# Seanforfun/Distributed-Tensorflow-Framework

Measured on AMD Instinct MI355X. Metric: images/sec (whole node) ResNet-50 sync-SGD at 1/2/4/8 MI355X; scaling efficiency, higher is better.
Workload: dtype bf16; 1 GPU; model=resnet50_v1.5, global_batch=256, per_gpu_batch=256, image_size=224, parallelism=dp1, grad_sync=allreduce, comm_dtype=fp32, optimizer=momentum-sgd (fused), kernels=native, hip_graph=True

## Files before the change

### mdtf/csrc/bn.hip

```cpp
#include "mdtf_common.h"

using namespace mdtf;

namespace {

constexpr int kThreads = 256;

struct Geo {
  int tpr;
  int rg;
  int gy;
  int gx;
};

Geo make_geo(long long M, int C) {
  Geo g;
  int cv = C / 8;
  int t = 1;
  while (t * 2 <= cv && t * 2 <= kThreads) t *= 2;
  g.tpr = t;
  g.rg = kThreads / t;
  g.gy = static_cast<int>(ceil_div(cv, t));
  long long gx = ceil_div(M, (long long)g.rg * 16);
  long long cap = 1024 / g.gy;
// ... 258 lines not shown
    const char* e = getenv("MDTF_BN_NT");
    return !(e && e[0] == '0');
  }();
  return on;
}

template <bool HAS_RES, bool RELU, bool NT = false>
__device__ __forceinline__ void apply8(const uint4& xr, const uint4& rr, const float (&sc)[8], const float (&sh)[8],
                                       bf16_t* __restrict__ y, uint8_t* __restrict__ mask, long long i) {
  float v[8], r[8];
  unpack8(xr, v);
  if (HAS_RES) unpack8(rr, r);
  uint32_t bits = 0;
#pragma unroll
  for (int k = 0; k < 8; ++k) {
    float o = v[k] * sc[k] + sh[k];
    if (HAS_RES) o += r[k];
    if (RELU) {
      o = fmaxf(o, 0.f);
      bits |= (o > 0.f ? 1u : 0u) << k;
    }
    v[k] = o;
  }
  st_bf8<NT>(y + i * 8, v);
  if (RELU && mask) mask[i] = static_cast<uint8_t>(bits);
}

constexpr int kVpt = 4;

template <bool HAS_RES, bool RELU, bool NT = false>
__global__ void __launch_bounds__(kThreads)
    bn_apply_kernel(const bf16_t* __restrict__ x, const bf16_t* __restrict__ res, bf16_t* __restrict__ y,
                    uint8_t* __restrict__ mask, long long n8, int C, const float* __restrict__ scale,
                    const float* __restrict__ shift) {
  const long long base = (long long)blockIdx.x * (kThreads * kVpt) + threadIdx.x;
  const uint4 z4 = make_uint4(0, 0, 0, 0);
  uint4 xr[kVpt], rr[kVpt];
#pragma unroll
  for (int u = 0; u < kVpt; ++u) {
    const long long i = base + u * kThreads;
    xr[u] = i < n8 ? ld16<NT>(x + i * 8) : z4;
    rr[u] = (HAS_RES && i < n8) ? ld16<NT>(res + i * 8) : z4;
  }
  const bool fixed = (kThreads * 8) % C == 0;
  float sc[8], sh[8];
  load_coef8(scale, static_cast<int>((base * 8) % C), sc);
  load_coef8(shift, static_cast<int>((base * 8) % C), sh);
#pragma unroll
  for (int u = 0; u < kVpt; ++u) {
    const long long i = base + u * kThreads;
    if (i >= n8) break;
    if (!fixed) {
      load_coef8(scale, static_cast<int>((i * 8) % C), sc);
      load_coef8(shift, static_cast<int>((i * 8) % C), sh);
    }
    apply8<HAS_RES, RELU, NT>(xr[u], rr[u], sc, sh, y, mask, i);
  }
}

template <bool NT>
__global__ void __launch_bounds__(kThreads)
    bn_apply_dual_kernel(const bf16_t* __restrict__ x, const bf16_t* __restrict__ r, bf16_t* __restrict__ y,
                         uint8_t* __restrict__ mask, long long n8, int C, const float* __restrict__ scale,
                         const float* __restrict__ shift, const float* __restrict__ scale2,
                         const float* __restrict__ shift2) {
  const long long base = (long long)blockIdx.x * (kThreads * kVpt) + threadIdx.x;
  const uint4 z4 = make_uint4(0, 0, 0, 0);
  uint4 xr[kVpt], rr[kVpt];
#pragma unroll
  for (int u = 0; u < kVpt; ++u) {
    const long long i = base + u * kThreads;
    xr[u] = i < n8 ? ld16<NT>(x + i * 8) : z4;
    rr[u] = i < n8 ? ld16<NT>(r + i * 8) : z4;
  }
  const bool fixed = (kThreads * 8) % C == 0;
  float sc[8], sh[8], sc2[8], sh2[8];
  int c0 = static_cast<int>((base * 8) % C);
  load_coef8(scale, c0, sc);
  load_coef8(shift, c0, sh);
  load_coef8(scale2, c0, sc2);
  load_coef8(shift2, c0, sh2);
#pragma unroll
  for (int u = 0; u < kVpt; ++u) {
    const long long i = base + u * kThreads;
    if (i >= n8) break;
    if (!fixed) {
      c0 = static_cast<int>((i * 8) % C);
      load_coef8(scale, c0, sc);
      load_coef8(shift, c0, sh);
      load_coef8(scale2, c0, sc2);
      load_coef8(shift2, c0, sh2);
    }
    float v[8], rv[8];
    unpack8(xr[u], v);
    unpack8(rr[u], rv);
    uint32_t bits = 0;
#pragma unroll
    for (int k = 0; k < 8; ++k) {
      const float o = fmaxf(v[k] * sc[k] + sh[k] + (rv[k] * sc2[k] + sh2[k]), 0.f);
      bits |= (o > 0.f ? 1u : 0u) << k;
      v[k] = o;
    }
    st_bf8<NT>(y + i * 8, v);
    mask[i] = static_cast<uint8_t>(bits);
  }
}

struct FinBwd {
  const float* p0;
  const float* p1;
  int gx;
  const float* gamma;
  const float* mean;
  const float* invstd;
  float* dgamma;
  float* dbeta;
  float* k1;
  float* k2;
  float* k3;
  int zero_after;
};

__device__ __forceinline__ void finalize_bwd(const FinBwd& a, long long M, int C) {
  const int c = blockIdx.x * kFinCh + threadIdx.x % kFinCh;
  const bool own = threadIdx.x < kFinCh && c < C;
  const float mu = own ? a.mean[c] : 0.f, inv = own ? a.invstd[c] : 0.f;
  const float g = own && a.gamma ? a.gamma[c] : 1.f;
  const bool ow = (a.zero_after & 2) != 0;
  const float dg0 = own && a.dgamma && !ow ? a.dgamma[c] : 0.f;
  const float db0 = own && a.dbeta && !ow ? a.dbeta[c] : 0.f;
  double sdz, sdzx;
  if (!sum_partials(a.p0, a.p1, a.gx, C, sdz, sdzx, (a.zero_after & 1) != 0)) return;
  float db = (float)sdz;
  float dg = (float)((sdzx - (double)mu * sdz) * inv);
  if (a.dgamma) a.dgamma[c] = dg0 + dg;
  if (a.dbeta) a.dbeta[c] = db0 + db;
  float ak = g * inv;
  float invM = 1.f / (float)M;
  a.k1[c] = ak;
  a.k2[c] = -ak * inv * dg * invM;
  a.k3[c] = ak * (-db * invM + mu * inv * dg * invM);
}

__global__ void __launch_bounds__(1024)
    bn_finalize_bwd(const float* __restrict__ p0, const float* __restrict__ p1, int gx, long long M, int C,
                    const float* __restrict__ gamma, const float* __restrict__ mean, const float* __restrict__ invstd,
                    float* __restrict__ dgamma, float* __restrict__ dbeta, float* __restrict__ k1,
                    float* __restrict__ k2, float* __restrict__ k3, int zero_after) {
  finalize_bwd(FinBwd{p0, p1, gx, gamma, mean, invstd, dgamma, dbeta, k1, k2, k3, zero_after}, M, C);
}

__global__ void __launch_bounds__(1024) bn_finalize_bwd2(FinBwd a0, FinBwd a1, long long M, int C) {
  finalize_bwd(blockIdx.y ? a1 : a0, M, C);
}

template <bool RELU, bool WRITE_DRES, bool NT = false>
__device__ __forceinline__ void dx8(const uint4& gr, const uint4& xr, uint32_t m8, const uint4& orr,
                                    const float (&A)[8], const float (&B)[8], const float (&E)[8],
                                    bf16_t* __restrict__ dx, bf16_t* __restrict__ dres, long long i, int accum_dres) {
  float g[8], xv[8];
  unpack8(gr, g);
  unpack8(xr, xv);
  if (RELU) {
#pragma unroll
    for (int k = 0; k < 8; ++k) g[k] = ((m8 >> k) & 1u) ? g[k] : 0.f;
  }
  if (WRITE_DRES) {
    if (accum_dres) {
      float o[8];
      unpack8(orr, o);
#pragma unroll
      for (int k = 0; k < 8; ++k) o[k] += g[k];
      st_bf8<NT>(dres + i * 8, o);
    } else {
      st_bf8<NT>(dres + i * 8, g);
    }
  }
  float o[8];
#pragma unroll
  for (int k = 0; k < 8; ++k) o[k] = A[k] * g[k] + B[k] * xv[k] + E[k];
  st_bf8<NT>(dx + i * 8, o);
}

template <bool RELU, bool WRITE_DRES, bool NT = false>
__global__ void __launch_bounds__(kThreads)
    bn_dx_kernel(const bf16_t* __restrict__ dy, const bf16_t* __restrict__ x, const uint8_t* __restrict__ mk,
                 bf16_t* __restrict__ dx, bf16_t* __restrict__ dres, long long n8, int C, const float* __restrict__ k1,
                 const float* __restrict__ k2, const float* __restrict__ k3, int accum_dres,
                 const float* __restrict__ fin_dgdb, float* __restrict__ dgamma, float* __restrict__ dbeta) {
  if (fin_dgdb && blockIdx.x == 0) {
    for (int c = threadIdx.x; c < C; c += kThreads) {
      if (dgamma) dgamma[c] += fin_dgdb[c];
      if (dbeta) dbeta[c] += fin_dgdb[C + c];
    }
  }
  const long long base = (long long)blockIdx.x * (kThreads * kVpt) + threadIdx.x;
  const uint4 z4 = make_uint4(0, 0, 0, 0);
  const bool acc = WRITE_DRES && accum_dres;
  uint4 gr[kVpt], xr[kVpt], orr[kVpt];
  uint32_t m8[kVpt];
#pragma unroll
  for (int u = 0; u < kVpt; ++u) {
    const long long i = base + u * kThreads;
    const bool ok = i < n8;
    gr[u] = ok ? ld16<NT>(dy + i * 8) : z4;
    xr[u] = ok ? ld16<NT>(x + i * 8) : z4;
    m8[u] = (RELU && ok) ? mk[i] : 0xffu;
    orr[u] = (acc && ok) ? ld16<NT>(dres + i * 8) : z4;
  }
  const bool fixed = (kThreads * 8) % C == 0;
  float A[8], B[8], E[8];
  const int c0 = static_cast<int>((base * 8) % C);
  load_coef8(k1, c0, A);
  load_coef8(k2, c0, B);
  load_coef8(k3, c0, E);
#pragma unroll
  for (int u = 0; u < kVpt; ++u) {
    const long long i = base + u * kThreads;
    if (i >= n8) break;
    if (!fixed) {
      const int c = static_cast<int>((i * 8) % C);
      load_coef8(k1, c, A);
      load_coef8(k2, c, B);
      load_coef8(k3, c, E);
    }
    dx8<RELU, WRITE_DRES, NT>(gr[u], xr[u], m8[u], orr[u], A, B, E, dx, dres, i, accum_dres);
  }
}

inline int ew_grid(long long n8);
void launch_dx(const void* dy, const void* x, const void* mask, void* dx, void* dres, long long M, int C,
               const float* k1, const float* k2, const float* k3, int relu, int accum_dres, hipStream_t st,
               const float* fin_dgdb = nullptr, float* dgamma = nullptr, float* dbeta = nullptr);

void launch_apply(const void* x, const void* res, void* y, uint8_t* mask, long long n8, int C, const float* scale,
                  const float* shift, int relu, hipStream_t st) {
  const bf16_t* r = (const bf16_t*)res;
  const bf16_t* xx = (const bf16_t*)x;
  bf16_t* yy = (bf16_t*)y;
  const bool nt = bn_nt();
#define APPLY(R_, L_)                                                                                               \
  hipLaunchKernelGGL((nt ? bn_apply_kernel<R_, L_, true> : bn_apply_kernel<R_, L_, false>), dim3(ew_grid(n8)),     \
                     dim3(kThreads), 0, st, xx, R_ ? r : nullptr, yy, L_ ? mask : nullptr, n8, C, scale, shift)
  if (r && relu)
    APPLY(true, true);
  else if (r)
    APPLY(true, false);
  else if (relu)
    APPLY(false, true);
  else
    APPLY(false, false);
#undef APPLY
}

inline int ew_grid(long long n8) {
  long long b = ceil_div(n8, (long long)kThreads * kVpt);
  return static_cast<int>(b > 0 ? b : 1);
}

}

MDTF_EXPORT long long mdtf_bn_workspace_floats(long long M, int C) {
  Geo g = make_geo(M, C);
  return 2LL * g.gx * C + 4LL * C;
}

MDTF_EXPORT int mdtf_bn_fwd_train(const void* x, const void* res, void* y, uint8_t* mask, long long M, int C,
                                  const float* gamma, const float* beta, float* mmean, float* mvar, float decay,
                                  float eps, int relu, float* mean, float* invstd, float* ws, hipStream_t st) {
  if (C % 8) return MDTF_EINVAL;
  Geo g = make_geo(M, C);
  float* p0 = ws;
  float* p1 = ws + (long long)g.gx * C;
  float* scale = p1 + (long long)g.gx * C;
  float* shift = scale + C;
  size_t lds = 2 * sizeof(float) * g.rg * g.tpr * 8;
  hipLaunchKernelGGL((bn_reduce_kernel<false, false>), dim3(g.gx, g.gy), dim3(kThreads), lds, st,
                     (const bf16_t*)x, nullptr, nullptr, M, C, g.tpr, g.rg, p0, p1);
  hipLaunchKernelGGL(bn_finalize_fwd, dim3(ceil_div(C, kFinCh)), dim3(kFinCh * kFinGroups), 0, st, p0, p1, g.gx, M, C, gamma, beta,
                     mmean, mvar, decay, eps, mean, invstd, scale, shift, 0);
  long long n8 = M * C / 8;
  launch_apply(x, res, y, mask, n8, C, scale, shift, relu, st);
  MDTF_LAUNCH_CHECK();
  return 0;
}

MDTF_EXPORT int mdtf_bn_fwd_stats(const void* x, const void* res, void* y, uint8_t* mask, long long M, int C,
                                  const float* gamma, const float* beta, float* mmean, float* mvar, float decay,
                                  float eps, int relu, float* mean, float* invstd, const float* psum, const float* psq,
                                  int P, float* ws, hipStream_t st) {
  if (C % 8) return MDTF_EINVAL;
  float* scale = ws;
  float* shift = ws + C;
  hipLaunchKernelGGL(bn_finalize_fwd, dim3(ceil_div(C, kFinCh)), dim3(kFinCh * kFinGroups), 0, st, psum, psq, P, M,
                     C, gamma, beta, mmean, mvar, decay, eps, mean, invstd, scale, shift, 1);
  long long n8 = M * C / 8;
  launch_apply(x, res, y, mask, n8, C, scale, shift, relu, st);
  MDTF_LAUNCH_CHECK();
  return 0;
}

MDTF_EXPORT int mdtf_bn_fwd_coeffs(long long M, int C, const float* gamma, const float* beta, float* mmean,
                                   float* mvar, float decay, float eps, float* mean, float* invstd, const float* psum,
                                   const float* psq, int P, float* ws, hipStream_t st) {
  if (C % 8) return MDTF_EINVAL;
  hipLaunchKernelGGL(bn_finalize_fwd, dim3(ceil_div(C, kFinCh)), dim3(kFinCh * kFinGroups), 0, st, psum, psq, P, M,
// ... 630 lines not shown
bool pool_geo_ok(const PoolG& g) {
  return g.C % 8 == 0 && g.KH * g.KW <= 255 && (long long)g.N * g.H * g.W * g.C < (1LL << 31) &&
         g.OH > 0 && g.OW > 0;
}

}

MDTF_EXPORT int mdtf_bn_relu_maxpool_fwd(const void* x, void* y, uint8_t* arg, int N, int H, int W, int C, int OH,
                                         int OW, int KH, int KW, int SH, int SW, int PT, int PL, const float* gamma,
                                         const float* beta, float* mmean, float* mvar, float decay, float eps,
                                         float* mean, float* invstd, const float* psum, const float* psq, int P,
                                         float* ss, hipStream_t st) {
  PoolG g{N, H, W, C, OH, OW, KH, KW, SH, SW, PT, PL};
  if (!pool_geo_ok(g)) return MDTF_EUNSUPPORTED;
  const long long M = (long long)N * H * W;
  hipLaunchKernelGGL(bn_finalize_fwd, dim3(ceil_div(C, kFinCh)), dim3(kFinCh * kFinGroups), 0, st, psum, psq, P, M,
                     C, gamma, beta, mmean, mvar, decay, eps, mean, invstd, ss, ss + C, 1);
  const int total = N * OH * OW * (C / 8);
  hipLaunchKernelGGL(bn_relu_maxpool_fwd, dim3(ceil_div(total, kThreads)), dim3(kThreads), 0, st, (const bf16_t*)x,
                     ss, ss + C, (bf16_t*)y, arg, g, total);
  MDTF_LAUNCH_CHECK();
  return 0;
}

namespace {
int pool_dx_pairs = -1;
}

MDTF_EXPORT void mdtf_bn_pool_dx_pairs(int on) { pool_dx_pairs = on ? 1 : 0; }

MDTF_EXPORT int mdtf_maxpool_bn_bwd(const void* dy, const uint8_t* arg, const void* x, void* dx, int N, int H, int W,
                                    int C, int OH, int OW, int KH, int KW, int SH, int SW, int PT, int PL,
                                    const float* gamma, const float* mean, const float* invstd, float* dgamma,
                                    float* dbeta, const float* ss, float* ws, const void* y, hipStream_t st) {
  PoolG g{N, H, W, C, OH, OW, KH, KW, SH, SW, PT, PL};
  if (!pool_geo_ok(g)) return MDTF_EUNSUPPORTED;
  const long long M = (long long)N * H * W;
  Geo ge = make_geo(M, C);
  float* p0 = ws;
  float* p1 = ws + (long long)ge.gx * C;
  float* k1 = p1 + (long long)ge.gx * C;
  float* k2 = k1 + C;
  float* k3 = k2 + C;
  const int cv = C / 8;
  const bool rows_path = (cv & (cv - 1)) == 0 && cv <= kThreads;
  int parts = ge.gx;
  if (y) {
    const Geo gp = make_geo((long long)N * OH * OW, C);
    parts = gp.gx;
    const size_t lds = 2 * sizeof(float) * gp.rg * gp.tpr * 8;
    hipLaunchKernelGGL(maxpool_bn_bwd_reduce_pooled, dim3(gp.gx, gp.gy), dim3(kThreads), lds, st, (const bf16_t*)dy,
                       (const bf16_t*)y, arg, (const bf16_t*)x, ss, ss + C, invstd, g, gp.tpr, gp.rg, p0, p1);
  } else if (rows_path) {
    int cvs = 0;
    while ((1 << cvs) < cv) ++cvs;
    const int nrows = N * H;
    int gx = ge.gx < nrows ? ge.gx : nrows;
    const int rpb = (nrows + gx - 1) / gx;
    gx = (nrows + rpb - 1) / rpb;
    parts = gx;
    hipLaunchKernelGGL(maxpool_bn_bwd_reduce_rows, dim3(gx), dim3(kThreads), 0, st, (const bf16_t*)dy, arg,
                       (const bf16_t*)x, ss, ss + C, g, cvs, rpb, p0, p1);
  } else {
    const size_t lds = 2 * sizeof(float) * ge.rg * ge.tpr * 8;
    hipLaunchKernelGGL(maxpool_bn_bwd_reduce, dim3(ge.gx, ge.gy), dim3(kThreads), lds, st, (const bf16_t*)dy, arg,
                       (const bf16_t*)x, ss, ss + C, g, ge.tpr, ge.rg, p0, p1);
  }
  hipLaunchKernelGGL(bn_finalize_bwd, dim3(ceil_div(C, kFinCh)), dim3(kFinCh * kFinGroups), 0, st, p0, p1, parts, M,
                     C, gamma, mean, invstd, dgamma, dbeta, k1, k2, k3, 0);
  if (pool_dx_pairs < 0) {
    const char* e = getenv("MDTF_POOL_DX_PAIRS");
    pool_dx_pairs = (e && e[0] == '0') ? 0 : 1;
  }
  const bool pairs_on = pool_dx_pairs != 0;
  const size_t pair_lds = (size_t)2 * OW * cv * (sizeof(uint4) + sizeof(uint2));
  if (rows_path && pairs_on && SH == 2 && SW == 2 && KH <= 4 && KW <= 4 && PT >= 0 && PL >= 0 &&
      2 * W * cv <= kThreads * kPairVec && pair_lds <= 64 * 1024) {
    int cvs = 0;
    while ((1 << cvs) < cv) ++cvs;
    const int kmin = PT >> 1, nk = ((H - 1 + PT) >> 1) - kmin + 1;
    hipLaunchKernelGGL(maxpool_bn_dx_pairs, dim3(N * nk), dim3(kThreads), pair_lds, st, (const bf16_t*)dy, arg,
                       (const bf16_t*)x, ss, ss + C, k1, k2, k3, (bf16_t*)dx, g, cvs, kmin, nk);
  } else if (rows_path) {
    int cvs = 0;
    while ((1 << cvs) < cv) ++cvs;
    hipLaunchKernelGGL(maxpool_bn_dx_rows, dim3(N * H), dim3(kThreads), 0, st, (const bf16_t*)dy, arg,
                       (const bf16_t*)x, ss, ss + C, k1, k2, k3, (bf16_t*)dx, g, cvs);
  } else {
    const int total = (int)(M * cv);
    hipLaunchKernelGGL(maxpool_bn_dx, dim3(ceil_div(total, kThreads)), dim3(kThreads), 0, st, (const bf16_t*)dy, arg,
                       (const bf16_t*)x, ss, ss + C, k1, k2, k3, (bf16_t*)dx, g, total);
  }
  MDTF_LAUNCH_CHECK();
  return 0;
}

namespace {
template <bool NT>
__global__ void __launch_bounds__(kThreads)
    bn_dx_dual_kernel(const bf16_t* __restrict__ dy, const bf16_t* __restrict__ x, const bf16_t* __restrict__ r,
                      const uint8_t* __restrict__ mk, bf16_t* __restrict__ dx, bf16_t* __restrict__ dr, long long n8,
                      int C, const float* __restrict__ k, const float* __restrict__ k2) {
  const long long base = (long long)blockIdx.x * (kThreads * kVpt) + threadIdx.x;
  const uint4 z4 = make_uint4(0, 0, 0, 0);
  uint4 gr[kVpt], xr[kVpt], rr[kVpt];
  uint32_t m8[kVpt];
#pragma unroll
  for (int u = 0; u < kVpt; ++u) {
    const long long i = base + u * kThreads;
    const bool ok = i < n8;
    gr[u] = ok ? ld16<NT>(dy + i * 8) : z4;
    xr[u] = ok ? ld16<NT>(x + i * 8) : z4;
    rr[u] = ok ? ld16<NT>(r + i * 8) : z4;
    m8[u] = ok ? mk[i] : 0u;
  }
  const bool fixed = (kThreads * 8) % C == 0;
  float A[8], B[8], E[8], A2[8], B2[8], E2[8];
  int c0 = static_cast<int>((base * 8) % C);
  load_coef8(k, c0, A);
  load_coef8(k + C, c0, B);
  load_coef8(k + 2 * C, c0, E);
  load_coef8(k2, c0, A2);
  load_coef8(k2 + C, c0, B2);
  load_coef8(k2 + 2 * C, c0, E2);
#pragma unroll
  for (int u = 0; u < kVpt; ++u) {
    const long long i = base + u * kThreads;
    if (i >= n8) break;
    if (!fixed) {
      c0 = static_cast<int>((i * 8) % C);
      load_coef8(k, c0, A);
      load_coef8(k + C, c0, B);
      load_coef8(k + 2 * C, c0, E);
      load_coef8(k2, c0, A2);
      load_coef8(k2 + C, c0, B2);
      load_coef8(k2 + 2 * C, c0, E2);
    }
    float g[8], xv[8], rv[8], o[8], o2[8];
    unpack8(gr[u], g);
    unpack8(xr[u], xv);
    unpack8(rr[u], rv);
#pragma unroll
    for (int e = 0; e < 8; ++e) {
      const float gm = ((m8[u] >> e) & 1u) ? g[e] : 0.f;
      o[e] = A[e] * gm + B[e] * xv[e] + E[e];
      o2[e] = A2[e] * gm + B2[e] * rv[e] + E2[e];
    }
    st_bf8<NT>(dx + i * 8, o);
    st_bf8<NT>(dr + i * 8, o2);
  }
}
}

MDTF_EXPORT int mdtf_bn_bwd_dual(const void* dy, const void* x, const void* r, const uint8_t* mask, void* dx, void* dr,
                                 long long M, int C, const float* gamma, const float* mean, const float* invstd,
                                 float* dgamma, float* dbeta, float* psum, float* psq, int P, const float* gamma2,
                                 const float* mean2, const float* invstd2, float* dgamma2, float* dbeta2, float* ws,
                                 hipStream_t st) {
  if (C % 8 || !mask) return MDTF_EINVAL;
  Geo g = make_geo(M, C);
  const long long half = 2LL * g.gx * C + 4LL * C;
  float* q0 = ws;
  float* q1 = q0 + (long long)g.gx * C;
  float* kk2 = q1 + (long long)g.gx * C;
  float* w2 = ws + half;
  float* p0 = w2;
  float* p1 = p0 + (long long)g.gx * C;
  float* kk = p1 + (long long)g.gx * C;
  const size_t lds = 2 * sizeof(float) * g.rg * g.tpr * 8;
  if (P <= 0) {
    hipLaunchKernelGGL((bn_reduce_kernel<true, true>), dim3(g.gx, g.gy), dim3(kThreads), lds, st, (const bf16_t*)dy,
                       (const bf16_t*)x, mask, M, C, g.tpr, g.rg, p0, p1);
    hipLaunchKernelGGL(bn_finalize_bwd, dim3(ceil_div(C, kFinCh)), dim3(kFinCh * kFinGroups), 0, st, p0, p1, g.gx, M,
                       C, gamma, mean, invstd, dgamma, dbeta, kk, kk + C, kk + 2 * C, 0);
  }
  hipLaunchKernelGGL((bn_reduce_kernel<true, true>), dim3(g.gx, g.gy), dim3(kThreads), lds, st, (const bf16_t*)dy,
                     (const bf16_t*)r, mask, M, C, g.tpr, g.rg, q0, q1);
  const FinBwd sc{q0, q1, g.gx, gamma2, mean2, invstd2, dgamma2, dbeta2, kk2, kk2 + C, kk2 + 2 * C, 0};
  if (P > 0)
    hipLaunchKernelGGL(bn_finalize_bwd2, dim3(ceil_div(C, kFinCh), 2), dim3(kFinCh * kFinGroups), 0, st,
                       FinBwd{psum, psq, P, gamma, mean, invstd, dgamma, dbeta, kk, kk + C, kk + 2 * C, 1}, sc, M, C);
  else
    hipLaunchKernelGGL(bn_finalize_bwd2, dim3(ceil_div(C, kFinCh), 1), dim3(kFinCh * kFinGroups), 0, st, sc, sc, M,
                       C);
  const long long n8 = M * C / 8;
  hipLaunchKernelGGL((bn_nt() ? bn_dx_dual_kernel<true> : bn_dx_dual_kernel<false>), dim3(ew_grid(n8)),
                     dim3(kThreads), 0, st, (const bf16_t*)dy,
                     (const bf16_t*)x, (const bf16_t*)r, mask, (bf16_t*)dx, (bf16_t*)dr, n8, C, kk, kk2);
  MDTF_LAUNCH_CHECK();
  return 0;
}
```

### mdtf/csrc/conv_igemm.hip

```cpp
#include "mdtf_common.h"

#ifndef FD_PF16
#define FD_PF16 1
#endif

using namespace mdtf;

namespace {

typedef __bf16 bf16x8_t __attribute__((ext_vector_type(8)));
typedef short v4s __attribute__((ext_vector_type(4)));
typedef __attribute__((address_space(3))) v4s lds_v4s;

constexpr int BK = 32;
constexpr int PADK = 8;
constexpr int PADN = 16;
constexpr int NT = 256;
constexpr int kStatSlots = 64;

struct ConvArgs {
  const bf16_t* src;
  const bf16_t* wgt;
  const bf16_t* dy;
  bf16_t* out;
  float* dw;
  float* stat_sum;
  float* stat_sq;
  int N, H, W, Cin;
  int OH, OW, Cout;
  int KH, KW, SH, SW, PH, PW, DH, DW;
  long long M;
  int Ncol;
  int K;
  int mtiles, ntiles;
  int ksplit_steps;
  int stat_slots;
  int ld_dy, ld_dw;
  int accumulate;
  const bf16_t* acc_src;
  const uint8_t* acc_mask;
  int cls_h0, cls_w0, cls_q0h, cls_q0w, cls_kh0, cls_kw0, cls_Hc, cls_Wc, cls_th, cls_tw;
  const bf16_t* bx;
  const uint8_t* bmask;
  float* bsum;
  float* bsq;
  int bslots;
  float* dbias;
  float* slab;
  int slab_cap;
  int slab_nt;
  int* cnt;
  int wg_xcd;
  const bf16_t* wseg[4];
  int seg_cols, ld_b;
  const bf16_t* bias;
  bf16_t* pre_out;
  int act;
  unsigned mg_rw, mg_rh;
  int sh_rw, sh_rh;
  long long m_base;
  int fin_blocks, fin_first;
  int co_remap;
  const float* fin_psum;
  const float* fin_psq;
  int fin_P, fin_C;
  long long fin_M;
  const float* fin_gamma;
  const float* fin_mean;
  const float* fin_invstd;
  float* fin_ws;
};

__device__ __noinline__ void fin_bwd_block(float* psum, float* psq, int P, int C, long long M, const float* gamma,
                                           const float* meanp, const float* invstdp, float* ws, int blk, char* smem) {
  const int G = blockDim.x / 32;
  const int lc = threadIdx.x & 31, grp = threadIdx.x >> 5;
  const int c = blk * 32 + lc;
  const bool own = grp == 0 && c < C;
  const float mu = own ? meanp[c] : 0.f, inv = own ? invstdp[c] : 0.f;
  const float gm = own && gamma ? gamma[c] : 1.f;
  float s[4] = {0.f, 0.f, 0.f, 0.f}, q[4] = {0.f, 0.f, 0.f, 0.f};
  if (c < C) {
    int r = grp;
    for (; r + 3 * G < P; r += 4 * G) {
#pragma unroll
      for (int u = 0; u < 4; ++u) {
        s[u] += psum[(long long)(r + u * G) * C + c];
        q[u] += psq[(long long)(r + u * G) * C + c];
      }
    }
    for (; r < P; r += G) {
      s[0] += psum[(long long)r * C + c];
      q[0] += psq[(long long)r * C + c];
    }
    for (r = grp; r < P; r += G) {
      psum[(long long)r * C + c] = 0.f;
      psq[(long long)r * C + c] = 0.f;
    }
  }
  double* L0 = reinterpret_cast<double*>(smem);
  double* L1 = L0 + G * 32;
  L0[grp * 32 + lc] = (double)s[0] + (double)s[1] + (double)s[2] + (double)s[3];
  L1[grp * 32 + lc] = (double)q[0] + (double)q[1] + (double)q[2] + (double)q[3];
  __syncthreads();
  if (!own) return;
  double sdz = 0.0, sdzx = 0.0;
  for (int g = 0; g < G; ++g) {
    sdz += L0[g * 32 + lc];
    sdzx += L1[g * 32 + lc];
  }
  const float db = (float)sdz;
  const float dg = (float)((sdzx - (double)mu * sdz) * inv);
  ws[3 * C + c] = dg;
  ws[4 * C + c] = db;
  const float ak = gm * inv, invM = 1.f / (float)M;
  ws[c] = ak;
  ws[C + c] = -ak * inv * dg * invM;
  ws[2 * C + c] = ak * (-db * invM + mu * inv * dg * invM);
}

inline void magic31(unsigned d, unsigned* m, int* sh) {
  int l = 0;
  while ((1ull << l) < d) ++l;
  *m = static_cast<unsigned>(((1ull << (31 + l)) + d - 1) / d);
  *sh = 31 + l;
}

__device__ __forceinline__ unsigned fdiv31(unsigned n, unsigned m, int sh) {
  return static_cast<unsigned>((static_cast<unsigned long long>(n) * m) >> sh);
}

__device__ __forceinline__ uint4 mask_bf8(const uint4& v, uint32_t m8) {
  const uint32_t w[4] = {v.x, v.y, v.z, v.w};
  uint32_t o[4];
#pragma unroll
  for (int k = 0; k < 4; ++k)
    o[k] = (w[k] & (((m8 >> (2 * k)) & 1u) ? 0x0000ffffu : 0u)) | (w[k] & (((m8 >> (2 * k + 1)) & 1u) ? 0xffff0000u : 0u));
  return make_uint4(o[0], o[1], o[2], o[3]);
}

typedef unsigned v4u __attribute__((ext_vector_type(4)));

__device__ __forceinline__ void unpack8(const uint4& raw, float (&f)[8]) {
  const uint32_t w[4] = {raw.x, raw.y, raw.z, raw.w};
#pragma unroll
  for (int k = 0; k < 4; ++k) {
    f[2 * k] = __uint_as_float(w[k] << 16);
    f[2 * k + 1] = __uint_as_float(w[k] & 0xffff0000u);
  }
}

__device__ __forceinline__ uint4 ld16(const bf16_t* p, bool ok) {
  return ok ? *reinterpret_cast<const uint4*>(p) : make_uint4(0, 0, 0, 0);
}

__device__ __forceinline__ void st16(bf16_t* lds, const uint4& v) { *reinterpret_cast<uint4*>(lds) = v; }

__device__ __forceinline__ bf16x8_t frag_kcontig(const bf16_t* tile, int row0, int lane) {
  const bf16_t* p = tile + (row0 + (lane & 15)) * (BK + PADK) + 8 * (lane >> 4);
  uint4 v = *reinterpret_cast<const uint4*>(p);
  return __builtin_bit_cast(bf16x8_t, v);
}

__device__ __forceinline__ bf16x8_t frag_ncontig(const bf16_t* tile, int ld, int col0, int lane) {
  const int g = lane >> 4, i = lane & 15, q = i >> 2, p = i & 3;
  const int odd = g & 1;
  const int rfirst = 8 * g + (odd ? 4 : 0) + q;
  const int rsecond = 8 * g + (odd ? 0 : 4) + q;
  const bf16_t* a1 = tile + rfirst * ld + col0 + 4 * p;
  const bf16_t* a2 = tile + rsecond * ld + col0 + 4 * p;
  v4s r1 = __builtin_amdgcn_ds_read_tr16_b64_v4i16((lds_v4s*)a1);
  v4s r2 = __builtin_amdgcn_ds_read_tr16_b64_v4i16((lds_v4s*)a2);
  v4s lo = odd ? r2 : r1;
  v4s hi = odd ? r1 : r2;
  short8 f = {lo[0], lo[1], lo[2], lo[3], hi[0], hi[1], hi[2], hi[3]};
  return __builtin_bit_cast(bf16x8_t, f);
}

__device__ __forceinline__ float dense_act(float v, int act) {
  if (act == 1) return fmaxf(v, 0.f);
  if (act == 2) {
    const float u2 = 1.5957691216f * (v + 0.044715f * v * v * v);
    return v * __builtin_amdgcn_rcpf(1.f + __expf(-u2));
  }
  return v;
}

__device__ __forceinline__ float dense_act_grad(float x, int act) {
  if (act == 1) return x > 0.f ? 1.f : 0.f;
  if (act == 2) {
    const float s = __builtin_amdgcn_rcpf(1.f + __expf(-1.5957691216f * (x + 0.044715f * x * x * x)));
    return s + 2.f * x * s * (1.f - s) * 0.7978845608f * (1.f + 0.134145f * x * x);
  }
  return 1.f;
}

__device__ __forceinline__ int trswz(int k) { return 2 * (((k >> 1) & 1) | (((k >> 3) & 1) << 1)); }

__device__ __forceinline__ bf16x8_t frag_tr(const char* img, int col0, int kbase, int lane) {
  const int g = lane >> 4, i = lane & 15, q = i >> 2, p = i & 3;
  const int c = col0 + 4 * p;
  const int k1 = kbase + 8 * g + q, k2 = k1 + 4;
  const char* a1 = img + k1 * 128 + (((c >> 3) ^ trswz(k1)) << 4) + (c & 7) * 2;
  const char* a2 = img + k2 * 128 + (((c >> 3) ^ trswz(k2)) << 4) + (c & 7) * 2;
  v4s lo = __builtin_amdgcn_ds_read_tr16_b64_v4i16((lds_v4s*)a1);
  v4s hi = __builtin_amdgcn_ds_read_tr16_b64_v4i16((lds_v4s*)a2);
  short8 f = {lo[0], lo[1], lo[2], lo[3], hi[0], hi[1], hi[2], hi[3]};
  return __builtin_bit_cast(bf16x8_t, f);
}

__device__ __forceinline__ float4v mfma(const bf16x8_t& a, const bf16x8_t& b, const float4v& c) {
  return __builtin_amdgcn_mfma_f32_16x16x32_bf16(a, b, c, 0, 0, 0);
}

__device__ __forceinline__ int xcd_remap(int bid, int nwg) {
// ... 251 lines not shown
    const int cidx = tid + i * NT;
    a_mrow[i] = cidx / (BM / 8);
    a_rc[i] = cidx % (BM / 8);
    const int r = r0 + a_rc[i] * 8;
    a_rok[i] = r < R;
    const int rr = a_rok[i] ? r : 0;
    a_c[i] = rr % a.Cin;
    const int t = rr / a.Cin;
    a_kw[i] = t % a.KW;
    a_kh[i] = t / a.KW;
  }
  const long long Mpix = a.M;
  const int KT_total = static_cast<int>((Mpix + BK - 1) / BK);
  const int kt_begin = split * a.ksplit_steps;
  const int kt_end = min(KT_total, kt_begin + a.ksplit_steps);
  if (kt_begin >= kt_end) return;

  int p_ow[A_CHUNKS], p_oh[A_CHUNKS], p_n[A_CHUNKS];
#pragma unroll
  for (int i = 0; i < A_CHUNKS; ++i) {
    const long long m = (long long)kt_begin * BK + a_mrow[i];
    p_ow[i] = static_cast<int>(m % a.OW);
    const long long t = m / a.OW;
    p_oh[i] = static_cast<int>(t % a.OH);
    p_n[i] = static_cast<int>(t / a.OH);
  }
  uint4 ra[A_CHUNKS], rb[B_CHUNKS];
  auto load_tiles = [&](int kt) {
#pragma unroll
    for (int i = 0; i < A_CHUNKS; ++i) {
      const long long m = (long long)kt * BK + a_mrow[i];
      const int iy = p_oh[i] * a.SH - a.PH + a_kh[i] * a.DH, ix = p_ow[i] * a.SW - a.PW + a_kw[i] * a.DW;
      const bool ok = a_rok[i] && m < Mpix && iy >= 0 && iy < a.H && ix >= 0 && ix < a.W;
      ra[i] = ld16(a.src + (((long long)p_n[i] * a.H + (ok ? iy : 0)) * a.W + (ok ? ix : 0)) * a.Cin + a_c[i], ok);
      p_ow[i] += BK;
      while (p_ow[i] >= a.OW) { p_ow[i] -= a.OW; if (++p_oh[i] == a.OH) { p_oh[i] = 0; ++p_n[i]; } }
    }
#pragma unroll
    for (int i = 0; i < B_CHUNKS; ++i) {
      const int cidx = tid + i * NT;
      const int mrow = cidx / (BN / 8), c8 = cidx % (BN / 8);
      const long long m = (long long)kt * BK + mrow;
      const int n = n0 + c8 * 8;
      const bool ok = m < Mpix && n < a.Cout;
      rb[i] = ld16(a.dy + (ok ? m : 0) * a.Cout + (ok ? n : 0), ok);
    }
  };
  auto store_tiles = [&](int buf) {
#pragma unroll
    for (int i = 0; i < A_CHUNKS; ++i) st16(As[buf] + a_mrow[i] * LDA + a_rc[i] * 8, ra[i]);
#pragma unroll
    for (int i = 0; i < B_CHUNKS; ++i) {
      const int cidx = tid + i * NT;
      st16(Bs[buf] + (cidx / (BN / 8)) * LDB + (cidx % (BN / 8)) * 8, rb[i]);
    }
  };

  float4v acc[TM][TN];
#pragma unroll
  for (int i = 0; i < TM; ++i)
#pragma unroll
    for (int j = 0; j < TN; ++j) acc[i][j] = float4v{0.f, 0.f, 0.f, 0.f};

  load_tiles(kt_begin);
  store_tiles(0);
  __syncthreads();
  int cur = 0;
  for (int kt = kt_begin; kt < kt_end; ++kt) {
    if (kt + 1 < kt_end) load_tiles(kt + 1);
    bf16x8_t fa[TM], fb[TN];
#pragma unroll
    for (int i = 0; i < TM; ++i) fa[i] = frag_ncontig(As[cur], LDA, wm * (TM * 16) + i * 16, lane);
#pragma unroll
    for (int j = 0; j < TN; ++j) fb[j] = frag_ncontig(Bs[cur], LDB, wn * (TN * 16) + j * 16, lane);
#pragma unroll
    for (int i = 0; i < TM; ++i)
#pragma unroll
      for (int j = 0; j < TN; ++j) acc[i][j] = mfma(fa[i], fb[j], acc[i][j]);
    if (kt + 1 < kt_end) store_tiles(cur ^ 1);
    __syncthreads();
    cur ^= 1;
  }
  const int g = lane >> 4, li = lane & 15;
#pragma unroll
  for (int i = 0; i < TM; ++i)
#pragma unroll
    for (int j = 0; j < TN; ++j) {
      const int co = n0 + wn * (TN * 16) + j * 16 + li;
      if (co >= a.Cout) continue;
#pragma unroll
      for (int rr = 0; rr < 4; ++rr) {
        const int r = r0 + wm * (TM * 16) + i * 16 + 4 * g + rr;
        if (r < R) atomicAdd(a.dw + (long long)r * a.Cout + co, acc[i][j][rr]);
      }
    }
}

template <int BN>
__device__ __forceinline__ void copyout_rc(int idx, int& row, int& c8, bool remap) {
  if (BN == 128 && remap) {
    const int l = idx & 31, hh = (idx >> 5) & 1;
    const bool ga = l < 4 || (l >= 12 && l < 16) || (l >= 20 && l < 28);
    c8 = ga ? (l < 4 ? l : (l < 16 ? l - 8 : l - 12)) : (l < 12 ? l - 4 : (l < 20 ? l - 8 : l - 16));
    row = ((idx >> 6) << 2) + 2 * hh + (ga ? 0 : 1);
  } else {
    row = idx / (BN / 8);
    c8 = idx - row * (BN / 8);
  }
}

template <int BM, int BN, int MODE, bool STATS, int STAGES, int NW>
__global__ void __launch_bounds__(64 * NW) conv_fd_v2(ConvArgs a) {
  constexpr int NT = 64 * NW;
  constexpr int WM = NW == 4 ? 2 : (BM > BN ? 4 : 2), WN = NW / WM;
  constexpr int TM = BM / WM / 16, TN = BN / WN / 16;
  constexpr int RA = BM / (8 * NW), RB = BN / (8 * NW);
  constexpr int ROWB = 128;
  constexpr int STAGE = (BM + BN) * ROWB;
  constexpr int PER_STAGE = RA + RB;
  constexpr unsigned OOB = 0x80000000u;
  constexpr bool SPLIT = STAGES >= 10;
  constexpr int SA = SPLIT ? STAGES / 10 : STAGES, SB = SPLIT ? STAGES % 10 : STAGES;
  static_assert(RA >= 1 && RB >= 1, "tile too small");
  static_assert(STAGES >= 1 && (STAGES < 2 || SPLIT || (STAGES - 2) * PER_STAGE < 64), "pipeline depth");
  static_assert(!SPLIT || (SA > SB && SB >= 2 && (SA - 1) * PER_STAGE < 64), "split ring");
  extern __shared__ __attribute__((aligned(16))) char smem_raw[];

  const int tid = threadIdx.x, lane = tid & 63;
  const int wave = __builtin_amdgcn_readfirstlane(tid >> 6);
  const int wm = wave / WN, wn = wave % WN;
  const int tile = xcd_remap(blockIdx.x, gridDim.x);
  const int mt = tile / a.ntiles, nt = tile % a.ntiles;
  const long long m0 = a.m_base + (long long)mt * BM;
  const int n0 = nt * BN;

  constexpr int AM = MODE == 3 ? 0 : MODE == 4 ? 1 : MODE;
  const int GH = AM == 0 ? a.H : a.OH;
  const int GW = AM == 0 ? a.W : a.OW;
  const int GC = AM == 0 ? a.Cin : a.Cout;
  const int RH = AM == 0 ? a.OH : AM == 1 ? a.H : a.cls_Hc;
  const int RW = AM == 0 ? a.OW : AM == 1 ? a.W : a.cls_Wc;
  const int lrow = lane >> 3;
  const int TKW = MODE == 2 ? a.cls_tw : a.KW;
  const int ntaps = MODE == 2 ? a.cls_th * a.cls_tw : a.KH * a.KW;
  const int DHe = MODE == 2 ? 1 : a.DH, DWe = MODE == 2 ? 1 : a.DW;

  const int bytes_a = (int)((long long)a.N * GH * GW * GC * 2);
  const int bytes_b = MODE == 3 ? (int)((long long)a.K * a.ld_b * 2)
                                : (int)((long long)(MODE == 2 ? a.KH * a.KW * a.Cout : a.K) * a.Ncol * 2);
  const int seg = MODE == 3 ? n0 / a.seg_cols : 0;
  const bf16_t* wbase = MODE == 3 ? a.wseg[seg] : a.wgt;
  const int nl0 = MODE == 3 ? n0 - seg * a.seg_cols : n0;

  unsigned a_off[RA], a_mask[RA];
#pragma unroll
  for (int i = 0; i < RA; ++i) {
    const int row = 8 * (wave + NW * i) + lrow;
    const long long m = m0 + row;
    const bool ok = m < a.M;
    const unsigned mm = ok ? static_cast<unsigned>(m) : 0u;
    const unsigned t = fdiv31(mm, a.mg_rw, a.sh_rw);
    const int ow = static_cast<int>(mm - t * static_cast<unsigned>(RW));
    const unsigned nq = fdiv31(t, a.mg_rh, a.sh_rh);
    const int oh = static_cast<int>(t - nq * static_cast<unsigned>(RH));
    const int n = static_cast<int>(nq);
    const int y0 = AM == 0 ? oh * a.SH - a.PH : AM == 1 ? oh + a.PH : a.cls_q0h + oh;
    const int x0 = AM == 0 ? ow * a.SW - a.PW : AM == 1 ? ow + a.PW : a.cls_q0w + ow;
    const int ch = 8 * ((lane & 7) ^ ((row >> 1) & 7));
    a_off[i] = static_cast<unsigned>(((n * GH + y0) * GW + x0) * GC + ch);
    unsigned mask = 0;
    if (ok) {
      for (int tt = 0; tt < ntaps; ++tt) {
        const int kh = tt / TKW, kw = tt - kh * TKW;
        const int iy = AM == 0 ? y0 + kh * DHe : y0 - kh * DHe;
        const int ix = AM == 0 ? x0 + kw * DWe : x0 - kw * DWe;
        if (iy >= 0 && iy < GH && ix >= 0 && ix < GW) mask |= 1u << tt;
      }
    }
    a_mask[i] = mask;
  }
  unsigned b_off[RB];
#pragma unroll
  for (int i = 0; i < RB; ++i) {
    if (MODE == 3) {
      const int blk = wave + NW * i;
      const int krow = 8 * (blk & 7) + lrow;
      const int col = nl0 + 64 * (blk >> 3) + 8 * ((lane & 7) ^ trswz(krow));
      b_off[i] = (unsigned)(((long long)krow * a.ld_b + col) * 2);
      continue;
    }
    const int row = 8 * (wave + NW * i) + lrow;
    const int n = n0 + row;
    const int ch = 8 * ((lane & 7) ^ ((row >> 1) & 7));
    const long long e = MODE == 0 ? (long long)n * a.K + ch : (long long)n * a.Cout + ch;
    b_off[i] = n < a.Ncol ? (unsigned)(e * 2) : OOB;
  }

  int s_t = 0, s_kh = 0, s_kw = 0, s_c0 = 0, s_k0 = 0;
  auto stage = [&](int buf) {
    const int tap_e = (AM == 0 ? (s_kh * DHe * GW + s_kw * DWe) : -(s_kh * DHe * GW + s_kw * DWe)) * GC + s_c0;
    char* lds = smem_raw + buf * STAGE;
#pragma unroll
    for (int i = 0; i < RA; ++i) {
      const bool ok = (a_mask[i] >> s_t) & 1u;
      const unsigned voff = ok ? (a_off[i] + (unsigned)tap_e) * 2u : OOB;
      dma16(a.src, bytes_a, lds + (wave + NW * i) * 1024, voff, 0);
    }
    char* ldsb = lds + BM * ROWB;
    const int wtap = MODE == 2 ? (a.cls_kh0 + a.SH * s_kh) * a.KW + a.cls_kw0 + a.SW * s_kw : s_t;
    const int sb = MODE == 3 ? s_k0 * a.ld_b * 2 : MODE == 0 ? s_k0 * 2 : (wtap * a.Cin * a.Cout + s_c0) * 2;
#pragma unroll
    for (int i = 0; i < RB; ++i)
      dma16(wbase, bytes_b, ldsb + (wave + NW * i) * 1024, b_off[i], sb);
    s_k0 += 64;
    s_c0 += 64;
    const int wrap = s_c0 == GC ? 1 : 0;
    s_c0 = wrap ? 0 : s_c0;
    s_t += wrap;
    s_kw += wrap;
    const int wrap2 = s_kw == TKW ? 1 : 0;
    s_kw = wrap2 ? 0 : s_kw;
    s_kh += wrap2;
  };

  float4v acc[TM][TN];
#pragma unroll
  for (int i = 0; i < TM; ++i)
#pragma unroll
    for (int j = 0; j < TN; ++j) acc[i][j] = float4v{0.f, 0.f, 0.f, 0.f};

  constexpr int PITER = MODE == 4 ? BM * (BN / 8) / (64 * NW) : 1;
  uint4 prepf[PITER];
  if constexpr (MODE == 4) {
#pragma unroll
    for (int it = 0; it < PITER; ++it) {
      const int idx = tid + it * 64 * NW;
      int row, c8;
      copyout_rc<BN>(idx, row, c8, a.co_remap != 0);
      const long long m = m0 + row;
      const int n = n0 + c8 * 8;
      prepf[it] = (m < a.M && n < a.Ncol) ? *reinterpret_cast<const uint4*>(a.pre_out + m * a.Ncol + n)
                                          : make_uint4(0, 0, 0, 0);
    }
  }

  const int KT = a.K / 64;
  const int fr = lane & 15, fq = lane >> 4;
  if constexpr (SPLIT) {
    struct Walk { int t, kh, kw, c0, k0; };
    Walk wa{0, 0, 0, 0, 0}, wb{0, 0, 0, 0, 0};
    auto advance = [&](Walk& w) {
      w.k0 += 64;
      w.c0 += 64;
      const int wrap = w.c0 == GC ? 1 : 0;
      w.c0 = wrap ? 0 : w.c0;
      w.t += wrap;
      w.kw += wrap;
      const int wrap2 = w.kw == TKW ? 1 : 0;
      w.kw = wrap2 ? 0 : w.kw;
      w.kh += wrap2;
    };
    char* const ringB = smem_raw + SA * BM * ROWB;
    auto stage_a = [&](int buf) {
      const int tap_e = (AM == 0 ? (wa.kh * DHe * GW + wa.kw * DWe) : -(wa.kh * DHe * GW + wa.kw * DWe)) * GC + wa.c0;
      char* lds = smem_raw + buf * (BM * ROWB);
#pragma unroll
      for (int i = 0; i < RA; ++i) {
        const bool ok = (a_mask[i] >> wa.t) & 1u;
        const unsigned voff = ok ? (a_off[i] + (unsigned)tap_e) * 2u : OOB;
        dma16(a.src, bytes_a, lds + (wave + NW * i) * 1024, voff, 0);
      }
      advance(wa);
    };
    auto stage_b = [&](int buf) {
      char* ldsb = ringB + buf * (BN * ROWB);
      const int wtap = MODE == 2 ? (a.cls_kh0 + a.SH * wb.kh) * a.KW + a.cls_kw0 + a.SW * wb.kw : wb.t;
      const int sb = MODE == 3 ? wb.k0 * a.ld_b * 2 : MODE == 0 ? wb.k0 * 2 : (wtap * a.Cin * a.Cout + wb.c0) * 2;
#pragma unroll
      for (int i = 0; i < RB; ++i)
        dma16(wbase, bytes_b, ldsb + (wave + NW * i) * 1024, b_off[i], sb);
      advance(wb);
    };
    auto nb_of = [&](int j) { return (j + SB - 1 < KT ? RB : 0); };
    auto na_of = [&](int j) { return (j + SA - 1 < KT ? RA : 0); };
#pragma unroll
    for (int s = 0; s < SA - 1; ++s) {
      if (s <= SB - 2 && s < KT) stage_b(s);
      if (s < KT) stage_a(s);
    }
    int ca = 0, cb = 0;
    for (int kt = 0; kt < KT; ++kt) {
      int younger = 0;
      if (kt <= SB - 2) {
        for (int s = kt + 1; s <= SA - 2; ++s) younger += (s <= SB - 2 && s < KT ? RB : 0) + (s < KT ? RA : 0);
        for (int j = 0; j < kt; ++j) younger += nb_of(j) + na_of(j);
      } else {
        const int g0 = kt - SB + 1;
        younger = na_of(g0);
        for (int j = g0 + 1; j < kt; ++j) younger += nb_of(j) + na_of(j);
      }
      wait_vmcnt_le<(SA - 1) * PER_STAGE>(younger);
      __builtin_amdgcn_s_barrier();
      if (kt + SB - 1 < KT) stage_b(cb == 0 ? SB - 1 : cb - 1);
      if (kt + SA - 1 < KT) stage_a(ca == 0 ? SA - 1 : ca - 1);
      const char* As = smem_raw + ca * (BM * ROWB);
      const char* Bs = ringB + cb * (BN * ROWB);
      ca = ca + 1 == SA ? 0 : ca + 1;
      cb = cb + 1 == SB ? 0 : cb + 1;
      bf16x8_t fa[2][TM], fb[2][TN];
#pragma unroll
      for (int h = 0; h < 2; ++h) {
#pragma unroll
        for (int i = 0; i < TM; ++i) {
          const int row = wm * (TM * 16) + i * 16 + fr;
          const int pc = (h * 4 + fq) ^ ((row >> 1) & 7);
          fa[h][i] = __builtin_bit_cast(bf16x8_t, *reinterpret_cast<const uint4*>(As + row * ROWB + pc * 16));
        }
#pragma unroll
        for (int j = 0; j < TN; ++j) {
          if (MODE == 3) {
            const int col = wn * (TN * 16) + j * 16;
            fb[h][j] = frag_tr(Bs + (col >> 6) * 8192, col & 63, 32 * h, lane);
            continue;
          }
          const int row = wn * (TN * 16) + j * 16 + fr;
          const int pc = (h * 4 + fq) ^ ((row >> 1) & 7);
          fb[h][j] = __builtin_bit_cast(bf16x8_t, *reinterpret_cast<const uint4*>(Bs + row * ROWB + pc * 16));
        }
      }
#pragma unroll
      for (int h = 0; h < 2; ++h)
#pragma unroll
        for (int i = 0; i < TM; ++i)
#pragma unroll
          for (int j = 0; j < TN; ++j) acc[i][j] = mfma(fb[h][j], fa[h][i], acc[i][j]);
      {
        constexpr int R = TM + TN, MF = TM * TN, PER = MF / R > 0 ? MF / R : 1;
        __builtin_amdgcn_sched_group_barrier(0x100, R, 0);
#pragma unroll
        for (int i = 0; i < R; ++i) {
          __builtin_amdgcn_sched_group_barrier(0x008, PER, 0);
          __builtin_amdgcn_sched_group_barrier(0x100, 1, 0);
        }
        __builtin_amdgcn_sched_group_barrier(0x008, 2 * MF, 0);
      }
    }
  } else {
#pragma unroll
  for (int s = 0; s < (STAGES > 1 ? STAGES - 1 : 1); ++s)
    if (s < KT) stage(s);
  int cur = 0;
  for (int kt = 0; kt < KT; ++kt) {
    if (STAGES >= 2 && kt + STAGES - 2 < KT)
      wait_vmcnt<(STAGES >= 2 ? (STAGES - 2) * PER_STAGE : 0)>();
    else
      wait_vmcnt<0>();
    __builtin_amdgcn_s_barrier();
    if (STAGES >= 2) {
      const int nk = kt + STAGES - 1;
      if (nk < KT) stage(nk % STAGES);
    }
    const char* As = smem_raw + cur * STAGE;
    cur = cur + 1 == STAGES ? 0 : cur + 1;
    const char* Bs = As + BM * ROWB;
    bf16x8_t fa[2][TM], fb[2][TN];
#pragma unroll
    for (int h = 0; h < 2; ++h) {
#pragma unroll
      for (int i = 0; i < TM; ++i) {
        const int row = wm * (TM * 16) + i * 16 + fr;
        const int pc = (h * 4 + fq) ^ ((row >> 1) & 7);
        fa[h][i] = __builtin_bit_cast(bf16x8_t, *reinterpret_cast<const uint4*>(As + row * ROWB + pc * 16));
      }
#pragma unroll
      for (int j = 0; j < TN; ++j) {
        if (MODE == 3) {
          const int col = wn * (TN * 16) + j * 16;
          fb[h][j] = frag_tr(Bs + (col >> 6) * 8192, col & 63, 32 * h, lane);
          continue;
        }
        const int row = wn * (TN * 16) + j * 16 + fr;
        const int pc = (h * 4 + fq) ^ ((row >> 1) & 7);
        fb[h][j] = __builtin_bit_cast(bf16x8_t, *reinterpret_cast<const uint4*>(Bs + row * ROWB + pc * 16));
      }
    }
#pragma unroll
    for (int h = 0; h < 2; ++h)
#pragma unroll
      for (int i = 0; i < TM; ++i)
#pragma unroll
        for (int j = 0; j < TN; ++j) acc[i][j] = mfma(fb[h][j], fa[h][i], acc[i][j]);
    {
      constexpr int R = TM + TN, MF = TM * TN, PER = MF / R > 0 ? MF / R : 1;
      __builtin_amdgcn_sched_group_barrier(0x100, R, 0);
#pragma unroll
      for (int i = 0; i < R; ++i) {
        __builtin_amdgcn_sched_group_barrier(0x008, PER, 0);
        __builtin_amdgcn_sched_group_barrier(0x100, 1, 0);
      }
      __builtin_amdgcn_sched_group_barrier(0x008, 2 * MF, 0);
    }
  }
  }

  constexpr int LDC = BN * 2 + 16;
  const int g = lane >> 4, li = lane & 15;
  __syncthreads();
#pragma unroll
  for (int i = 0; i < TM; ++i) {
    const int pl = wm * (TM * 16) + i * 16 + li;
#pragma unroll
    for (int j = 0; j < TN; ++j) {
      const int cl = wn * (TN * 16) + j * 16 + 4 * g;
      float4v v = acc[i][j];
      if (MODE == 3 && a.bias) {
        const uint2 b4 = *reinterpret_cast<const uint2*>(a.bias + n0 + cl);
        v[0] += __uint_as_float(b4.x << 16);
        v[1] += __uint_as_float(b4.x & 0xffff0000u);
        v[2] += __uint_as_float(b4.y << 16);
        v[3] += __uint_as_float(b4.y & 0xffff0000u);
      }
      uint32_t lo = (uint32_t)f2bf(v[0]) | ((uint32_t)f2bf(v[1]) << 16);
      uint32_t hi = (uint32_t)f2bf(v[2]) | ((uint32_t)f2bf(v[3]) << 16);
      *reinterpret_cast<uint2*>(smem_raw + pl * LDC + ((cl * 2) ^ (((pl >> 3) & 1) << 3))) = make_uint2(lo, hi);
    }
  }
  __syncthreads();
  const bool bstat = (MODE == 1 || MODE == 2) && a.bsum != nullptr;
  float bs0[8], bs1[8];
#pragma unroll
  for (int k = 0; k < 8; ++k) bs0[k] = bs1[k] = 0.f;
  constexpr int ITER = BM * (BN / 8) / NT;
  static_assert(ITER * NT == BM * (BN / 8), "copy-out rows per thread");
  constexpr int PF = (FD_PF16 && (MODE == 1 || MODE == 2) && ITER <= 16) ? ITER
                                                                        : (ITER < 4 ? ITER : (ITER % 4 == 0 ? 4 : 2));
  static_assert(ITER % PF == 0, "prefetch groups");
#pragma unroll
  for (int g0 = 0; g0 < ITER; g0 += PF) {
  long long off[PF];
  uint4 old4[PF], x4[PF];
  uint32_t mb[PF];
#pragma unroll
  for (int it = 0; it < PF; ++it) {
    const int idx = tid + (g0 + it) * NT;
    int row, c8;
    copyout_rc<BN>(idx, row, c8, a.co_remap != 0);
    const long long m = m0 + row;
    const int n = n0 + c8 * 8;
    off[it] = -1;
    if (m < a.M && n < a.Ncol) {
      long long pix = m;
      if (MODE == 2) {
        const unsigned mu = static_cast<unsigned>(m);
        const unsigned t = fdiv31(mu, a.mg_rw, a.sh_rw);
        const int j = static_cast<int>(mu - t * static_cast<unsigned>(a.cls_Wc));
        const unsigned nb = fdiv31(t, a.mg_rh, a.sh_rh);
        const int i = static_cast<int>(t - nb * static_cast<unsigned>(a.cls_Hc));
        pix = (static_cast<long long>(nb) * a.H + a.cls_h0 + a.SH * i) * a.W + a.cls_w0 + a.SW * j;
      }
      off[it] = pix * a.Ncol + n;
      if (a.accumulate) {
        old4[it] = *reinterpret_cast<const uint4*>((a.acc_src ? a.acc_src : a.out) + off[it]);
        if (a.acc_mask) old4[it] = mask_bf8(old4[it], a.acc_mask[off[it] >> 3]);
      }
      if (bstat) {
        x4[it] = *reinterpret_cast<const uint4*>(a.bx + off[it]);
        mb[it] = a.bmask ? a.bmask[off[it] >> 3] : 0xffu;
      }
    }
  }
#pragma unroll
  for (int it = 0; it < PF; ++it) {
    if (off[it] < 0) continue;
    const int idx = tid + (g0 + it) * NT;
    int row, c8;
    copyout_rc<BN>(idx, row, c8, a.co_remap != 0);
    uint4 v = *reinterpret_cast<const uint4*>(smem_raw + row * LDC + c8 * 16);
    if ((row >> 3) & 1) v = make_uint4(v.z, v.w, v.x, v.y);
    bf16_t* dst = a.out + off[it];
    if (MODE == 3 && a.act) {
      if (a.pre_out) *reinterpret_cast<uint4*>(a.pre_out + off[it]) = v;
      float c[8];
      const uint32_t w4[4] = {v.x, v.y, v.z, v.w};
#pragma unroll
      for (int k = 0; k < 4; ++k) {
        c[2 * k] = dense_act(__uint_as_float(w4[k] << 16), a.act);
        c[2 * k + 1] = dense_act(__uint_as_float(w4[k] & 0xffff0000u), a.act);
      }
      store_bf8(dst, c);
    } else if (MODE == 4) {
      float c[8];
      const uint32_t w4[4] = {v.x, v.y, v.z, v.w};
      const uint4 pv = prepf[(g0 + it) % PITER];
      const uint32_t p4[4] = {pv.x, pv.y, pv.z, pv.w};
#pragma unroll
      for (int k = 0; k < 4; ++k) {
        c[2 * k] = __uint_as_float(w4[k] << 16) * dense_act_grad(__uint_as_float(p4[k] << 16), a.act);
        c[2 * k + 1] = __uint_as_float(w4[k] & 0xffff0000u) * dense_act_grad(__uint_as_float(p4[k] & 0xffff0000u), a.act);
      }
      store_bf8(dst, c);
    } else if (a.accumulate || bstat) {
      float c[8];
      const uint32_t w4[4] = {v.x, v.y, v.z, v.w};
#pragma unroll
      for (int k = 0; k < 4; ++k) {
        c[2 * k] = __uint_as_float(w4[k] << 16);
        c[2 * k + 1] = __uint_as_float(w4[k] & 0xffff0000u);
      }
      if (a.accumulate) {
        const uint32_t o4[4] = {old4[it].x, old4[it].y, old4[it].z, old4[it].w};
#pragma unroll
        for (int k = 0; k < 4; ++k) {
          const float lo = __uint_as_float(o4[k] << 16) + c[2 * k];
          const float hi = __uint_as_float(o4[k] & 0xffff0000u) + c[2 * k + 1];
          c[2 * k] = __uint_as_float((uint32_t)f2bf(lo) << 16);
          c[2 * k + 1] = __uint_as_float((uint32_t)f2bf(hi) << 16);
        }
        store_bf8(dst, c);
      } else {
        *reinterpret_cast<uint4*>(dst) = v;
      }
      if (bstat) {
        const uint32_t xw[4] = {x4[it].x, x4[it].y, x4[it].z, x4[it].w};
#pragma unroll
        for (int k = 0; k < 8; ++k) {
          const float xk = (k & 1) ? __uint_as_float(xw[k >> 1] & 0xffff0000u) : __uint_as_float(xw[k >> 1] << 16);
          const float gk = ((mb[it] >> k) & 1u) ? c[k] : 0.f;
          bs0[k] += gk;
          bs1[k] += gk * xk;
        }
      }
    } else {
      *reinterpret_cast<uint4*>(dst) = v;
    }
  }
  }
  if (bstat) {
    static_assert(NT % (BN / 8) == 0, "one channel chunk per thread");
    __syncthreads();
    constexpr int LDR = NT + 4;
    float* red = reinterpret_cast<float*>(smem_raw);
    int slot = tid;
    if (BN == 128 && a.co_remap) {
      int r0_, c0_;
      copyout_rc<BN>(tid, r0_, c0_, true);
      slot = (tid & ~63) | ((r0_ & 3) << 4) | c0_;
    }
#pragma unroll
    for (int k = 0; k < 8; ++k) {
      red[k * LDR + slot] = bs0[k];
      red[(8 + k) * LDR + slot] = bs1[k];
    }
    __syncthreads();
    for (int nl = tid; nl < BN; nl += NT) {
      const int n = n0 + nl, c8 = nl >> 3, k = nl & 7;
      if (n < a.Ncol) {
        float sv = 0.f, q = 0.f;
        for (int t2 = c8; t2 < NT; t2 += BN / 8) {
          sv += red[k * LDR + t2];
          q += red[(8 + k) * LDR + t2];
        }
        const long long slot = (long long)(mt % a.bslots) * a.Ncol + n;
        atomicAdd(a.bsum + slot, sv);
        atomicAdd(a.bsq + slot, q);
      }
    }
  }
  if (STATS) {
    float ssum[TN][4], ssq[TN][4];
#pragma unroll
    for (int j = 0; j < TN; ++j)
#pragma unroll
      for (int r = 0; r < 4; ++r) ssum[j][r] = ssq[j][r] = 0.f;
#pragma unroll
    for (int i = 0; i < TM; ++i) {
      const bool mok = m0 + wm * (TM * 16) + i * 16 + li < a.M;
#pragma unroll
      for (int j = 0; j < TN; ++j)
        if (mok) {
#pragma unroll
          for (int r = 0; r < 4; ++r) {
            ssum[j][r] += acc[i][j][r];
            ssq[j][r] += acc[i][j][r] * acc[i][j][r];
          }
        }
    }
#pragma unroll
    for (int j = 0; j < TN; ++j)
#pragma unroll
      for (int r = 0; r < 4; ++r) {
#pragma unroll
        for (int o = 1; o < 16; o <<= 1) {
          ssum[j][r] += __shfl_xor(ssum[j][r], o, 64);
          ssq[j][r] += __shfl_xor(ssq[j][r], o, 64);
        }
      }
    __syncthreads();
    float* red = reinterpret_cast<float*>(smem_raw);
    if (li == 0) {
#pragma unroll
      for (int j = 0; j < TN; ++j)
#pragma unroll
        for (int r = 0; r < 4; ++r) {
          const int nl = wn * (TN * 16) + j * 16 + 4 * g + r;
          red[wm * BN + nl] = ssum[j][r];
          red[WM * BN + wm * BN + nl] = ssq[j][r];
        }
    }
    __syncthreads();
    for (int nl = tid; nl < BN; nl += NT) {
      const int n = n0 + nl;
      if (n < a.Ncol) {
        float sv = 0.f, q = 0.f;
#pragma unroll
        for (int w = 0; w < WM; ++w) {
          sv += red[w * BN + nl];
          q += red[WM * BN + w * BN + nl];
        }
        const long long slot = (long long)(mt % a.stat_slots) * a.Ncol + n;
        atomicAdd(a.stat_sum + slot, sv);
        atomicAdd(a.stat_sq + slot, q);
      }
    }
  }
}

template <int BM, int BN, int MODE, bool STATS, int STAGES, int NW, bool HEAVY>
__global__ void __launch_bounds__(64 * NW) conv_fd_p(ConvArgs a) {
  constexpr int NT = 64 * NW;
  constexpr int WM = NW == 4 ? 2 : (BM > BN ? 4 : 2), WN = NW / WM;
  constexpr int TM = BM / WM / 16, TN = BN / WN / 16;
  constexpr int RA = BM / (8 * NW), RB = BN / (8 * NW);
  constexpr int ROWB = 128;
  constexpr int PER_STAGE = RA + RB;
  constexpr unsigned OOB = 0x80000000u;
  constexpr bool SPLIT = STAGES >= 10;
  constexpr int SA = SPLIT ? STAGES / 10 : STAGES, SB = SPLIT ? STAGES % 10 : STAGES;
  constexpr int RING = (SA * BM + SB * BN) * ROWB;
  static_assert(MODE <= 2 && TN % 2 == 0 && RA >= 1 && RB >= 1, "persistent tile");
  constexpr int EMAX = TM * (TN / 2);
  static_assert(SA >= SB && SB >= 2 && (SA - 1) * PER_STAGE + EMAX < 64, "persistent ring");
  extern __shared__ __attribute__((aligned(16))) char smem_raw[];
  float* red = reinterpret_cast<float*>(smem_raw + RING);

  const int tid = threadIdx.x, lane = tid & 63;
  const int wave = __builtin_amdgcn_readfirstlane(tid >> 6);
  const int wm = wave / WN, wn = wave % WN;
  const int total = a.mtiles * a.ntiles;
  const int GH = MODE == 0 ? a.H : a.OH;
  const int GW = MODE == 0 ? a.W : a.OW;
  const int GC = MODE == 0 ? a.Cin : a.Cout;
  const int RH = MODE == 0 ? a.OH : MODE == 1 ? a.H : a.cls_Hc;
  const int RW = MODE == 0 ? a.OW : MODE == 1 ? a.W : a.cls_Wc;
  const int lrow = lane >> 3;
  const int TKW = MODE == 2 ? a.cls_tw : a.KW;
  const int ntaps = MODE == 2 ? a.cls_th * a.cls_tw : a.KH * a.KW;
  const int DHe = MODE == 2 ? 1 : a.DH, DWe = MODE == 2 ? 1 : a.DW;
  const int bytes_a = (int)((long long)a.N * GH * GW * GC * 2);
  const int bytes_b = (int)((long long)(MODE == 2 ? a.KH * a.KW * a.Cout : a.K) * a.Ncol * 2);
  const int bytes_o = (int)((long long)a.N * (MODE == 0 ? a.OH * a.OW : a.H * a.W) * a.Ncol * 2);
  const __amdgpu_buffer_rsrc_t rs_out = __builtin_amdgcn_make_buffer_rsrc(a.out, (short)0, bytes_o, 0x00020000);
  constexpr bool heavy = HEAVY && (MODE == 1 || MODE == 2);
  const bool bstat = heavy && a.bsum != nullptr;
  const int KT = a.K / 64;

  int mt = 0, nt = 0;
  long long m0 = 0;
  int n0 = 0;
  unsigned a_off[RA], a_mask[RA], b_off[RB];
  auto setup = [&](int w) {
    const int tile = xcd_remap(w, total);
    mt = tile / a.ntiles;
    nt = tile - mt * a.ntiles;
    m0 = a.m_base + (long long)mt * BM;
    n0 = nt * BN;
#pragma unroll
    for (int i = 0; i < RA; ++i) {
      const int row = 8 * (wave + NW * i) + lrow;
      const long long m = m0 + row;
      const bool ok = m < a.M;
      const unsigned mm = ok ? static_cast<unsigned>(m) : 0u;
      const unsigned t = fdiv31(mm, a.mg_rw, a.sh_rw);
      const int ow = static_cast<int>(mm - t * static_cast<unsigned>(RW));
      const unsigned nq = fdiv31(t, a.mg_rh, a.sh_rh);
      const int oh = static_cast<int>(t - nq * static_cast<unsigned>(RH));
      const int n = static_cast<int>(nq);
      const int y0 = MODE == 0 ? oh * a.SH - a.PH : MODE == 1 ? oh + a.PH : a.cls_q0h + oh;
      const int x0 = MODE == 0 ? ow * a.SW - a.PW : MODE == 1 ? ow + a.PW : a.cls_q0w + ow;
      const int ch = 8 * ((lane & 7) ^ ((row >> 1) & 7));
      a_off[i] = static_cast<unsigned>(((n * GH + y0) * GW + x0) * GC + ch);
      unsigned mask = 0;
      if (ok) {
        for (int tt = 0; tt < ntaps; ++tt) {
          const int kh = tt / TKW, kw = tt - kh * TKW;
          const int iy = MODE == 0 ? y0 + kh * DHe : y0 - kh * DHe;
          const int ix = MODE == 0 ? x0 + kw * DWe : x0 - kw * DWe;
          if (iy >= 0 && iy < GH && ix >= 0 && ix < GW) mask |= 1u << tt;
        }
      }
      a_mask[i] = mask;
    }
#pragma unroll
    for (int i = 0; i < RB; ++i) {
      const int row = 8 * (wave + NW * i) + lrow;
      const int n = n0 + row;
      const int ch = 8 * ((lane & 7) ^ ((row >> 1) & 7));
      const int e = MODE == 0 ? n * a.K + ch : n * a.Cout + ch;
      b_off[i] = n < a.Ncol ? static_cast<unsigned>(e * 2) : OOB;
    }
  };

  struct Walk { int t, kh, kw, c0, k0; };
  Walk wa{0, 0, 0, 0, 0}, wb{0, 0, 0, 0, 0};
  auto advance = [&](Walk& w) {
    w.k0 += 64;
    w.c0 += 64;
    const int wrap = w.c0 == GC ? 1 : 0;
// ... 236 lines not shown
#pragma unroll
        for (int r = 0; r < 4; ++r)
#pragma unroll
          for (int o2 = 1; o2 < 16; o2 <<= 1) {
            ssum[j][r] += __shfl_xor(ssum[j][r], o2, 64);
            ssq[j][r] += __shfl_xor(ssq[j][r], o2, 64);
          }
      if (li == 0) {
#pragma unroll
        for (int j = 0; j < TN; ++j)
#pragma unroll
          for (int r = 0; r < 4; ++r) {
            const int nl = wn * (TN * 16) + j * 16 + 4 * g + r;
            red[wm * BN + nl] = ssum[j][r];
            red[WM * BN + wm * BN + nl] = ssq[j][r];
          }
      }
      __syncthreads();
      for (int nl = tid; nl < BN; nl += NT) {
        const int n = cur_n0 + nl;
        if (n < a.Ncol) {
          float sv = 0.f, q = 0.f;
#pragma unroll
          for (int w2 = 0; w2 < WM; ++w2) {
            sv += red[w2 * BN + nl];
            q += red[WM * BN + w2 * BN + nl];
          }
          const long long slot = (long long)(cur_mt % a.stat_slots) * a.Ncol + n;
          atomicAdd(a.stat_sum + slot, sv);
          atomicAdd(a.stat_sq + slot, q);
        }
      }
    }
    if (!more) break;
    if (heavy) {
      __syncthreads();
      setup(w_next);
      prologue();
      E = 0;
    } else {
      E = issued;
    }
    w = w_next;
  }
}

int conv_persist_mode() {
  static const int m = [] {
    const char* e = getenv("MDTF_CONV_PERSIST");
    return e ? atoi(e) : 0;
  }();
  return m;
}

int num_cus() {
  static const int n = [] {
    int dev = 0, v = 0;
    if (hipGetDevice(&dev) != hipSuccess ||
        hipDeviceGetAttribute(&v, hipDeviceAttributeMultiprocessorCount, dev) != hipSuccess || v <= 0)
      return 256;
    return v;
  }();
  return n;
}

template <int BM, int BN, int MODE, bool STATS, int STAGES, int NW>
int launch_fd_p(ConvArgs& a, hipStream_t st) {
  constexpr int NT = 64 * NW;
  constexpr int WM = NW == 4 ? 2 : (BM > BN ? 4 : 2), WN = NW / WM;
  constexpr int TM = BM / WM / 16, TN = BN / WN / 16;
  constexpr int SA = STAGES >= 10 ? STAGES / 10 : STAGES, SB = STAGES >= 10 ? STAGES % 10 : STAGES;
  const bool heavy = (MODE == 1 || MODE == 2) && (a.accumulate || a.bsum != nullptr);
  if (conv_persist_mode() == 2 && !(MODE == 0 && NW == 8 && BM == 256 && BN == 256)) return MDTF_EUNSUPPORTED;
  if constexpr (MODE > 2 || TN % 2 != 0 || SB < 2) {
    return MDTF_EUNSUPPORTED;
  } else {
    if (heavy && TM > 4) return MDTF_EUNSUPPORTED;
    const size_t ring = ((size_t)SA * BM + (size_t)SB * BN) * 128;
    const size_t lds = ring + (STATS ? (size_t)2 * WM * BN * sizeof(float) : 0);
    if (lds > 160 * 1024) return MDTF_EUNSUPPORTED;
    auto kern = heavy ? conv_fd_p<BM, BN, MODE, STATS, STAGES, NW, (MODE != 0 && TM <= 4)>
                      : conv_fd_p<BM, BN, MODE, STATS, STAGES, NW, false>;
    static int occ[2] = {0, 0};
    if (occ[heavy] == 0) {
      int o = 0;
      if (hipOccupancyMaxActiveBlocksPerMultiprocessor(&o, kern, NT, lds) != hipSuccess || o < 1) o = 1;
      occ[heavy] = o;
    }
    const long long total = (long long)a.mtiles * a.ntiles;
    const long long cap = (long long)num_cus() * occ[heavy];
    const unsigned grid = (unsigned)(total < cap ? total : cap);
    hipLaunchKernelGGL(kern, dim3(grid), dim3(NT), lds, st, a);
    MDTF_LAUNCH_CHECK();
    return 0;
  }
}

int conv_tail_mode() {
  static const int m = [] {
    const char* e = getenv("MDTF_CONV_TAIL");
    return e ? atoi(e) : 0;
  }();
  return m;
}

extern "C" int mdtf_get_deterministic();

template <int BM, int BN, int MODE, bool STATS, int STAGES, int NW = 4>
int launch_fd_v2(ConvArgs& a, hipStream_t st);

template <int BM, int BN, int MODE, bool STATS, int STAGES, int NW>
int launch_fd_tail_split(ConvArgs& a, hipStream_t st, int* rc) {
  if constexpr (NW == 8 && BM == 256 && (MODE == 0 || MODE == 1)) {
    if (!conv_tail_mode() || a.m_base != 0 || mdtf_get_deterministic()) return 0;
    const long long mtiles = ceil_div(a.M, BM), ntiles = ceil_div(a.Ncol, BN);
    const long long cus = num_cus(), total = mtiles * ntiles;
    const long long rounds = total / cus, rem = total - rounds * cus;
    if (rounds < 1 || rem == 0 || (conv_tail_mode() == 1 && rem * 4 > cus) || (rounds * cus) % ntiles) return 0;
    const long long m1 = rounds * cus / ntiles * BM;
    if (m1 >= a.M) return 0;
    const long long M = a.M;
    ConvArgs tail = a;
    tail.m_base = m1;
    a.M = m1;
    *rc = launch_fd_v2<BM, BN, MODE, STATS, STAGES, NW>(a, st);
    a.M = M;
    if (*rc == 0) *rc = launch_fd_v2<128, 128, MODE, STATS, 2, 4>(tail, st);
    a.mtiles = static_cast<int>(mtiles);
    a.ntiles = static_cast<int>(ntiles);
    return 1;
  } else {
    (void)a;
    (void)st;
    (void)rc;
    return 0;
  }
}

template <int BM, int BN, int MODE, bool STATS, int STAGES, int NW>
int launch_fd_v2(ConvArgs& a, hipStream_t st) {
  constexpr int NT = 64 * NW;
  {
    int rc = 0;
    if (launch_fd_tail_split<BM, BN, MODE, STATS, STAGES, NW>(a, st, &rc)) return rc;
  }
  a.mtiles = static_cast<int>(ceil_div(a.M - a.m_base, BM));
  a.ntiles = static_cast<int>(ceil_div(a.Ncol, BN));
  const long long nblk = (long long)a.mtiles * a.ntiles;
  if (nblk > 0x7fffffff) return MDTF_EUNSUPPORTED;
  const size_t stage_bytes = STAGES >= 10 ? ((size_t)(STAGES / 10) * BM + (size_t)(STAGES % 10) * BN) * 128
                                          : STAGES * (size_t)(BM + BN) * 128;
  const size_t ctile = (size_t)BM * (BN * 2 + 16);
  size_t lds = stage_bytes > ctile ? stage_bytes : ctile;
  if (lds < (size_t)(NT + 8) * 16 * sizeof(float)) lds = (size_t)(NT + 8) * 16 * sizeof(float);
  if (STAGES == 1 && a.K > 64) return MDTF_EINVAL;
  if (lds > 160 * 1024) return MDTF_EUNSUPPORTED;
  if (a.M >= (1LL << 31)) return MDTF_EUNSUPPORTED;
  {
    constexpr int AM = MODE == 3 ? 0 : MODE == 4 ? 1 : MODE;
    const int RH = AM == 0 ? a.OH : AM == 1 ? a.H : a.cls_Hc;
    const int RW = AM == 0 ? a.OW : AM == 1 ? a.W : a.cls_Wc;
    if (RH < 1 || RW < 1) return MDTF_EINVAL;
    magic31(static_cast<unsigned>(RW), &a.mg_rw, &a.sh_rw);
    magic31(static_cast<unsigned>(RH), &a.mg_rh, &a.sh_rh);
  }
  if (MODE <= 2 && STAGES >= 2 && conv_persist_mode() && a.K >= 64) {
    const int rc = launch_fd_p<BM, BN, MODE, STATS, STAGES, NW>(a, st);
    if (rc != MDTF_EUNSUPPORTED) return rc;
  }
  {
    static const int remap = [] {
      const char* e = getenv("MDTF_FD_COREMAP");
      return (e && e[0] == '1') ? 1 : 0;
    }();
    a.co_remap = remap;
  }
  hipLaunchKernelGGL((conv_fd_v2<BM, BN, MODE, STATS, STAGES, NW>), dim3((unsigned)nblk), dim3(NT), lds, st, a);
  MDTF_LAUNCH_CHECK();
  return 0;
}

template <int MODE, bool STATS, int STAGES>
int dispatch_fd_v2s(ConvArgs& a, int bm, int bn, hipStream_t st) {
  if (bm == 128 && bn == 128) return launch_fd_v2<128, 128, MODE, STATS, STAGES>(a, st);
  if (bm == 128 && bn == 64) return launch_fd_v2<128, 64, MODE, STATS, STAGES>(a, st);
  if (bm == 256 && bn == 128) return launch_fd_v2<256, 128, MODE, STATS, STAGES>(a, st);
  if (bm == 256 && bn == 64) return launch_fd_v2<256, 64, MODE, STATS, STAGES>(a, st);
  if (bm == 64 && bn == 128) return launch_fd_v2<64, 128, MODE, STATS, STAGES>(a, st);
  if (bm == 64 && bn == 64) return launch_fd_v2<64, 64, MODE, STATS, STAGES>(a, st);
  return MDTF_EUNSUPPORTED;
}

template <int MODE, bool STATS>
int dispatch_fd_v2w8(ConvArgs& a, int bm, int bn, int stages, hipStream_t st) {
#define FD8(BM_, BN_, S_) \
  if (bm == BM_ && bn == BN_ && stages == S_) return launch_fd_v2<BM_, BN_, MODE, STATS, S_, 8>(a, st);
  FD8(256, 256, 1) FD8(256, 256, 2) FD8(256, 128, 1) FD8(256, 128, 2) FD8(256, 128, 3) FD8(256, 64, 2)
  FD8(256, 64, 3) FD8(256, 64, 4) FD8(128, 256, 2) FD8(128, 256, 3)
  FD8(256, 256, 32) FD8(256, 128, 32) FD8(256, 128, 42) FD8(128, 256, 32) FD8(128, 256, 42)
  if constexpr (MODE != 4) {
    FD8(448, 128, 1) FD8(448, 128, 2)
  }
#undef FD8
  return MDTF_EUNSUPPORTED;
}

template <int MODE, bool STATS>
int dispatch_fd_v2(ConvArgs& a, int bm, int bn, int stages, hipStream_t st) {
  if (bm >= 10000) return dispatch_fd_v2w8<MODE, STATS>(a, bm % 10000, bn, stages, st);
  if (stages == 32) {
    if (bm == 128 && bn == 128) return launch_fd_v2<128, 128, MODE, STATS, 32>(a, st);
    if (bm == 64 && bn == 128) return launch_fd_v2<64, 128, MODE, STATS, 32>(a, st);
    return MDTF_EUNSUPPORTED;
  }
  if (stages == 42) {
    if (bm == 64 && bn == 128) return launch_fd_v2<64, 128, MODE, STATS, 42>(a, st);
    return MDTF_EUNSUPPORTED;
  }
  if (stages == 1) return dispatch_fd_v2s<MODE, STATS, 1>(a, bm, bn, st);
  if (stages == 2) return dispatch_fd_v2s<MODE, STATS, 2>(a, bm, bn, st);
  if (stages == 3) return dispatch_fd_v2s<MODE, STATS, 3>(a, bm, bn, st);
  if (stages == 4) return dispatch_fd_v2s<MODE, STATS, 4>(a, bm, bn, st);
  return MDTF_EUNSUPPORTED;
}


template <int BM, int BN, int STAGES, int NW>
constexpr int wgrad_min_waves() {
  constexpr int blocks = (160 * 1024) / (STAGES * (BM + BN) * 128);
  constexpr int w = blocks * NW / 4;
  return w < 1 ? 1 : (w > 8 ? 8 : w);
}

template <int BM, int BN, int STAGES, int NW, bool PIPE>
__global__ void __launch_bounds__(64 * NW, (wgrad_min_waves<BM, BN, STAGES, NW>()))
    conv_wgrad_v2(ConvArgs a) {
  constexpr int WM = NW == 4 ? 2 : (BM > BN ? 4 : 2), WN = NW / WM;
  constexpr int U = 8 / NW;
  constexpr int TM = BM / WM / 16, TN = BN / WN / 16;
  constexpr int HA = BM / 64, HB = BN / 64;
  constexpr int IA = HA * U, IB = HB * U;
  constexpr int STAGE = (BM + BN) * 128;
  constexpr int PER_STAGE = IA + IB;
  constexpr unsigned OOB = 0x80000000u;
  static_assert(HA >= 1 && HB >= 1, "tile too small");
  static_assert(STAGES >= 2 && (STAGES - 2) * PER_STAGE < 64, "pipeline depth");
  extern __shared__ __attribute__((aligned(16))) char smem_raw[];

  const int tid = threadIdx.x, lane = tid & 63;
  const int wave = __builtin_amdgcn_readfirstlane(tid >> 6);
  const int wm = wave / WN, wn = wave % WN;
  const int tiles_mn = a.mtiles * a.ntiles;
  const int nwg = static_cast<int>(gridDim.x) - a.fin_blocks;
  const int fb = a.fin_first ? static_cast<int>(blockIdx.x) : static_cast<int>(blockIdx.x) - nwg;
  if (fb >= 0 && fb < a.fin_blocks) {
    fin_bwd_block(const_cast<float*>(a.fin_psum), const_cast<float*>(a.fin_psq), a.fin_P, a.fin_C, a.fin_M,
                  a.fin_gamma, a.fin_mean, a.fin_invstd, a.fin_ws, fb, smem_raw);
    return;
  }
  const int gb = a.fin_first ? static_cast<int>(blockIdx.x) - a.fin_blocks : static_cast<int>(blockIdx.x);
  const int lb = a.wg_xcd ? xcd_remap(gb, nwg) : gb;
  const int tile = lb % tiles_mn;
  const int split = lb / tiles_mn;
  const int mt = tile / a.ntiles, nt = tile % a.ntiles;
  const int r0 = mt * BM, n0 = nt * BN;
  const int R = a.KH * a.KW * a.Cin;
  const long long Mpix = a.M;
  const int KT_total = static_cast<int>((Mpix + 63) / 64);
  const int kt_begin = split * a.ksplit_steps;
  const int kt_end = min(KT_total, kt_begin + a.ksplit_steps);
  if (kt_begin >= kt_end) return;

  const int bytes_x = (int)((long long)a.N * a.H * a.W * a.Cin * 2);
  const int bytes_dy = (int)((Mpix - 1) * a.ld_dy * 2 + a.Cout * 2);
  const i32x4_t rsrc_x = buffer_rsrc(a.src, bytes_x), rsrc_dy = buffer_rsrc(a.dy, bytes_dy);

  int h_dy[HA], h_dx[HA], h_c[HA];
  bool h_ok[HA];
#pragma unroll
  for (int h = 0; h < HA; ++h) {
    const int r = r0 + 64 * h;
    h_ok[h] = r < R;
    const int rr = h_ok[h] ? r : 0;
    const int t = rr / a.Cin;
    h_c[h] = rr - t * a.Cin;
    const int kh = t / a.KW, kw = t - kh * a.KW;
    h_dy[h] = kh * a.DH - a.PH;
    h_dx[h] = kw * a.DW - a.PW;
  }
  const int krow0 = 8 * wave + (lane >> 3);
  int gch[U];
#pragma unroll
  for (int u = 0; u < U; ++u) gch[u] = ((lane & 7) ^ trswz(krow0 + 8 * NW * u)) * 8;
  int p_ow[U], p_oh[U], p_n[U];
  long long p_m[U];
#pragma unroll
  for (int u = 0; u < U; ++u) {
    const long long m = (long long)kt_begin * 64 + krow0 + 8 * NW * u;
    p_m[u] = m;
    p_ow[u] = static_cast<int>(m % a.OW);
    const long long t = m / a.OW;
    p_oh[u] = static_cast<int>(t % a.OH);
    p_n[u] = static_cast<int>(t / a.OH);
  }
  const int d_ow = 64 % a.OW, d_oh = (64 / a.OW) % a.OH, d_n = 64 / (a.OW * a.OH);

  auto stage = [&](int buf) {
    char* lds = smem_raw + buf * STAGE;
#pragma unroll
    for (int u = 0; u < U; ++u) {
      const bool mok = p_m[u] < Mpix;
      const int iy0 = p_oh[u] * a.SH, ix0 = p_ow[u] * a.SW;
#pragma unroll
      for (int h = 0; h < HA; ++h) {
        const int iy = iy0 + h_dy[h], ix = ix0 + h_dx[h];
        const bool ok = mok && h_ok[h] && iy >= 0 && iy < a.H && ix >= 0 && ix < a.W;
        const unsigned voff =
            ok ? (unsigned)((((p_n[u] * a.H + iy) * a.W + ix) * a.Cin + h_c[h] + gch[u]) * 2) : OOB;
        if constexpr (PIPE)
          dma16_asm(rsrc_x, lds + h * 8192 + (wave + NW * u) * 1024, voff);
        else
          dma16(a.src, bytes_x, lds + h * 8192 + (wave + NW * u) * 1024, voff, 0);
      }
      char* ldsb = lds + BM * 128;
#pragma unroll
      for (int h = 0; h < HB; ++h) {
        const int co = n0 + 64 * h;
        const unsigned voff = (mok && co < a.Cout) ? (unsigned)((p_m[u] * a.ld_dy + co + gch[u]) * 2) : OOB;
// ... 390 lines not shown
  if (a.slab && (splits < 2 || splits > a.slab_cap || (a.ld_dw % 4) || (a.Cout % 4))) b.slab = nullptr;
  b.cnt = nullptr;
  if (b.slab && g_wg_cnt && g_wg_cnt_n >= (long long)a.mtiles * a.ntiles && 256 % BM == 0 && 256 % BN == 0 &&
      (long long)splits * BM * BN * a.mtiles * a.ntiles * 4 < (1ll << 31) &&
      (long long)a.mtiles * BM <= ceil_div(R, 256) * 256 && (long long)a.ntiles * BN <= ceil_div(a.Cout, 256) * 256)
    b.cnt = g_wg_cnt;
  {
    static const int nt = [] {
      const char* e = getenv("MDTF_SLAB_NT");
      return (e && e[0] == '0') ? 0 : 1;
    }();
    b.slab_nt = nt;
  }
  const int store = g_wg_store;
  if (g_wg_fin.C > 0) {
    b.fin_blocks = static_cast<int>(ceil_div(g_wg_fin.C, 32));
    b.fin_psum = g_wg_fin.psum;
    b.fin_psq = g_wg_fin.psq;
    b.fin_P = g_wg_fin.P;
    b.fin_C = g_wg_fin.C;
    b.fin_M = g_wg_fin.M;
    b.fin_gamma = g_wg_fin.gamma;
    b.fin_mean = g_wg_fin.mean;
    b.fin_invstd = g_wg_fin.invstd;
    b.fin_ws = g_wg_fin.ws;
    static const int first = [] {
      const char* e = getenv("MDTF_BN_WG_FIN_FIRST");
      return (e && e[0] == '1') ? 1 : 0;
    }();
    b.fin_first = first;
    g_wg_fin = FinReq{};
  } else {
    b.fin_blocks = 0;
    b.fin_first = 0;
  }
  if (store && !(b.slab && !b.cnt)) {
    if (hipMemset2DAsync(a.dw, (size_t)a.ld_dw * 4, 0, (size_t)a.Cout * 4, (size_t)R, st) != hipSuccess)
      return MDTF_EUNSUPPORTED;
  }
  hipLaunchKernelGGL((conv_wgrad_v2<BM, BN, STAGES, NW, PIPE>), dim3(a.mtiles * a.ntiles * splits + b.fin_blocks),
                     dim3(64 * NW), lds, st, b);
  MDTF_LAUNCH_CHECK();
  if (b.slab && !b.cnt) {
    if (g_slab_stream && g_slab_stream != st) {
      hipEvent_t ev = slab_event();
      if (!ev || hipEventRecord(ev, st) != hipSuccess || hipStreamWaitEvent(g_slab_stream, ev, 0) != hipSuccess)
        return MDTF_EUNSUPPORTED;
      st = g_slab_stream;
    }
    const long long RC = (long long)R * a.Cout;
    static const int gmax = [] {
      const char* e = getenv("MDTF_SLAB_G");
      return e ? atoi(e) : 16;
    }();
    const long long q4 = RC / 4;
    int G = 1;
    while (G < gmax && G < 16 && q4 * G < 256LL * 256 && splits >= 8 * G) G *= 4;
    if (G == 16)
      hipLaunchKernelGGL((b.slab_nt ? wgrad_slab_reduce_g<true, 16> : wgrad_slab_reduce_g<false, 16>),
                         dim3((unsigned)ceil_div(q4, 16)), dim3(256), 0, st, b.slab, splits, RC, a.Cout,
                         (long long)a.ld_dw, a.dw, store);
    else if (G == 4)
      hipLaunchKernelGGL((b.slab_nt ? wgrad_slab_reduce_g<true, 4> : wgrad_slab_reduce_g<false, 4>),
                         dim3((unsigned)ceil_div(q4, 64)), dim3(256), 0, st, b.slab, splits, RC, a.Cout,
                         (long long)a.ld_dw, a.dw, store);
    else
      hipLaunchKernelGGL((b.slab_nt ? wgrad_slab_reduce<true> : wgrad_slab_reduce<false>),
                         dim3((unsigned)ceil_div(RC / 4, 256)), dim3(256), 0, st, b.slab, splits, RC, a.Cout,
                         (long long)a.ld_dw, a.dw, store);
    MDTF_LAUNCH_CHECK();
  }
  return 0;
}

template <int BM, int BN, int MODE, bool STATS>
size_t fd_lds() {
  const size_t a = (size_t)BM * (BK + PADK);
  const size_t b = MODE == 0 ? (size_t)BK * (BN + PADN) : (size_t)BN * (BK + PADK);
  size_t bytes = 2 * (a + b) * sizeof(bf16_t);
  const size_t red = 2 * 2 * BN * sizeof(float);
  return bytes > red ? bytes : red;
}

template <int BM, int BN, int MODE, bool STATS>
int launch_fd(ConvArgs& a, hipStream_t st) {
  a.mtiles = static_cast<int>(ceil_div(a.M, BM));
  a.ntiles = static_cast<int>(ceil_div(a.Ncol, BN));
  const long long nblk = (long long)a.mtiles * a.ntiles;
  if (nblk > 0x7fffffff) return MDTF_EUNSUPPORTED;
  const size_t lds = fd_lds<BM, BN, MODE, STATS>();
  hipLaunchKernelGGL((conv_fd_kernel<BM, BN, MODE, STATS>), dim3((unsigned)nblk), dim3(NT), lds, st, a);
  MDTF_LAUNCH_CHECK();
  return 0;
}

template <int MODE, bool STATS>
int dispatch_fd(ConvArgs& a, int bm, int bn, hipStream_t st) {
  if (bm == 128 && bn == 128) return launch_fd<128, 128, MODE, STATS>(a, st);
  if (bm == 128 && bn == 64) return launch_fd<128, 64, MODE, STATS>(a, st);
  if (bm == 64 && bn == 64) return launch_fd<64, 64, MODE, STATS>(a, st);
  if (bm == 256 && bn == 64) return launch_fd<256, 64, MODE, STATS>(a, st);
  return MDTF_EUNSUPPORTED;
}

template <int BM, int BN>
int launch_wgrad(ConvArgs& a, int splits, hipStream_t st) {
  const int R = a.KH * a.KW * a.Cin;
  a.mtiles = static_cast<int>(ceil_div(R, BM));
  a.ntiles = static_cast<int>(ceil_div(a.Cout, BN));
  const int kt_total = static_cast<int>(ceil_div(a.M, BK));
  if (splits < 1) {
    const int tiles = a.mtiles * a.ntiles;
    splits = (1024 + tiles - 1) / tiles;
  }
  if (splits > kt_total) splits = kt_total;
  a.ksplit_steps = (kt_total + splits - 1) / splits;
  splits = (kt_total + a.ksplit_steps - 1) / a.ksplit_steps;
  const size_t lds = 2 * ((size_t)BK * (BM + PADN) + (size_t)BK * (BN + PADN)) * sizeof(bf16_t);
  hipLaunchKernelGGL((conv_wgrad_kernel<BM, BN>), dim3(a.mtiles * a.ntiles * splits), dim3(NT), lds, st, a);
  MDTF_LAUNCH_CHECK();
  return 0;
}

int dispatch_wgrad_v2(ConvArgs& a, int bm, int bn, int stages, int w8, int splits, hipStream_t st) {
  static const bool pipe = [] {
    const char* e = getenv("MDTF_WGRAD_PIPE");
    return !(e && e[0] == '0');
  }();
  static const int xcd = [] {
    const char* e = getenv("MDTF_WGRAD_XCD");
    return (e && e[0] == '0') ? 0 : 1;
  }();
  a.wg_xcd = xcd;
#define WG2(BM_, BN_, S_, NW_) \
  if (bm == BM_ && bn == BN_ && stages == S_ && (NW_ == 8) == (w8 != 0)) \
    return pipe ? launch_wgrad_v2<BM_, BN_, S_, NW_, true>(a, splits, st) \
                : launch_wgrad_v2<BM_, BN_, S_, NW_, false>(a, splits, st);
  WG2(128, 128, 2, 4) WG2(128, 128, 3, 4) WG2(128, 64, 2, 4) WG2(128, 64, 3, 4) WG2(64, 128, 2, 4)
  WG2(64, 128, 3, 4) WG2(64, 64, 2, 4) WG2(64, 64, 3, 4) WG2(64, 64, 4, 4)
  WG2(256, 256, 2, 8) WG2(256, 128, 2, 8) WG2(256, 128, 3, 8) WG2(128, 256, 2, 8) WG2(128, 256, 3, 8)
  WG2(128, 128, 2, 8) WG2(128, 128, 3, 8) WG2(128, 128, 4, 8)
  WG2(128, 128, 5, 8) WG2(128, 128, 4, 4) WG2(128, 128, 5, 4) WG2(64, 128, 4, 4) WG2(64, 128, 6, 4)
  WG2(64, 256, 3, 8) WG2(64, 256, 4, 8) WG2(256, 64, 3, 8) WG2(256, 64, 4, 8)
#undef WG2
  return MDTF_EUNSUPPORTED;
}

template <bool BSTAT>
__global__ void __launch_bounds__(256) dgrad_zero_classes(ConvArgs a, int C8) {
  const int tid = threadIdx.x;
  const int ppb = 256 / C8;
  const int c8 = tid % C8, pl = tid / C8;
  const unsigned P = (unsigned)a.N * a.H * a.W;
  float s0[8], s1[8];
#pragma unroll
  for (int k = 0; k < 8; ++k) s0[k] = s1[k] = 0.f;
  for (unsigned p = blockIdx.x * (unsigned)ppb + pl; p < P; p += gridDim.x * (unsigned)ppb) {
    const unsigned q = fdiv31(p, a.mg_rw, a.sh_rw);
    const int w = static_cast<int>(p - q * (unsigned)a.W);
    const int h = static_cast<int>(q - fdiv31(q, a.mg_rh, a.sh_rh) * (unsigned)a.H);
    const int rh = (h + a.PH) % a.SH, rw = (w + a.PW) % a.SW;
    if (rh < a.KH && rw < a.KW) continue;
    const long long off = (long long)p * a.Ncol + c8 * 8;
    uint4 v = make_uint4(0, 0, 0, 0);
    if (a.accumulate) {
      v = *reinterpret_cast<const uint4*>((a.acc_src ? a.acc_src : a.out) + off);
      if (a.acc_mask) v = mask_bf8(v, a.acc_mask[off >> 3]);
    }
    if (a.acc_src || !a.accumulate) *reinterpret_cast<uint4*>(a.out + off) = v;
    if constexpr (BSTAT) {
      const uint4 x4 = *reinterpret_cast<const uint4*>(a.bx + off);
      const uint32_t mb = a.bmask ? a.bmask[off >> 3] : 0xffu;
      const uint32_t vw[4] = {v.x, v.y, v.z, v.w}, xw[4] = {x4.x, x4.y, x4.z, x4.w};
#pragma unroll
      for (int k = 0; k < 8; ++k) {
        const float g = (k & 1) ? __uint_as_float(vw[k >> 1] & 0xffff0000u) : __uint_as_float(vw[k >> 1] << 16);
        const float xk = (k & 1) ? __uint_as_float(xw[k >> 1] & 0xffff0000u) : __uint_as_float(xw[k >> 1] << 16);
        const float gm = ((mb >> k) & 1u) ? g : 0.f;
        s0[k] += gm;
        s1[k] += gm * xk;
      }
    }
  }
  if constexpr (BSTAT) {
    __shared__ float red[2][8][260];
#pragma unroll
    for (int k = 0; k < 8; ++k) {
      red[0][k][tid] = s0[k];
      red[1][k][tid] = s1[k];
    }
    __syncthreads();
    const long long slot = (long long)(blockIdx.x % a.bslots) * a.Ncol;
    for (int ch = tid; ch < a.Ncol; ch += 256) {
      const int cc = ch >> 3, k = ch & 7;
      float sv = 0.f, q = 0.f;
      for (int t = cc; t < 256; t += C8) {
        sv += red[0][k][t];
        q += red[1][k][t];
      }
      atomicAdd(a.bsum + slot + ch, sv);
      atomicAdd(a.bsq + slot + ch, q);
    }
  }
}

bool zero_class_gemm() {
  static const bool g = [] {
    const char* e = getenv("MDTF_ZERO_CLASS");
    return e && e[0] == 'g';
  }();
  return g;
}

void decode_tile(int* bm, int* stages) {
  const int c = *bm;
  if (c >= 100000) {
    *stages = (c % 100000) / 1000;
    *bm = (c / 100000 - 1) * 10000 + c % 1000;
    return;
  }
  *stages = (c % 10000) / 1000 ? (c % 10000) / 1000 : 2;
  *bm = (c / 10000) * 10000 + c % 1000;
}

ConvArgs make_args(int N, int H, int W, int Cin, int OH, int OW, int Cout, int KH, int KW, int SH, int SW, int PH,
                   int PW, int DH, int DW) {
  ConvArgs a{};
  a.N = N;
  a.H = H;
  a.W = W;
  a.Cin = Cin;
  a.OH = OH;
  a.OW = OW;
  a.Cout = Cout;
  a.KH = KH;
  a.KW = KW;
  a.SH = SH;
  a.SW = SW;
  a.PH = PH;
  a.PW = PW;
  a.DH = DH;
  a.DW = DW;
  return a;
}

}

MDTF_EXPORT int mdtf_conv_fwd(const void* x, const void* w, void* y, float* stat_sum, float* stat_sq, int stat_slots,
                              int N, int H, int W, int Cin, int OH, int OW, int Cout, int KH, int KW, int SH, int SW,
                              int PH, int PW, int DH, int DW, int bm, int bn, int* mtiles_out, hipStream_t st) {
  if (Cin % 8 || Cout % 8) return MDTF_EINVAL;
  ConvArgs a = make_args(N, H, W, Cin, OH, OW, Cout, KH, KW, SH, SW, PH, PW, DH, DW);
  a.src = (const bf16_t*)x;
  a.wgt = (const bf16_t*)w;
  a.out = (bf16_t*)y;
  a.stat_sum = stat_sum;
  a.stat_sq = stat_sq;
  a.stat_slots = stat_slots > 0 ? stat_slots : kStatSlots;
  a.M = (long long)N * OH * OW;
  a.Ncol = Cout;
  a.K = KH * KW * Cin;
  int rc = stat_sum ? dispatch_fd<0, true>(a, bm, bn, st) : dispatch_fd<0, false>(a, bm, bn, st);
  if (mtiles_out) *mtiles_out = a.mtiles;
  return rc;
}

MDTF_EXPORT int mdtf_conv_dgrad(const void* dy, const void* w, void* dx, int N, int H, int W, int Cin, int OH, int OW,
                                int Cout, int KH, int KW, int SH, int SW, int PH, int PW, int DH, int DW, int bm, int bn,
                                hipStream_t st) {
  if (Cin % 8 || Cout % 8) return MDTF_EINVAL;
  ConvArgs a = make_args(N, H, W, Cin, OH, OW, Cout, KH, KW, SH, SW, PH, PW, DH, DW);
  a.src = (const bf16_t*)dy;
  a.wgt = (const bf16_t*)w;
  a.out = (bf16_t*)dx;
  a.M = (long long)N * H * W;
  a.Ncol = Cin;
  a.K = KH * KW * Cout;
  return dispatch_fd<1, false>(a, bm, bn, st);
}

MDTF_EXPORT int mdtf_conv_wgrad(const void* x, const void* dy, float* dw, int N, int H, int W, int Cin, int OH, int OW,
                                int Cout, int KH, int KW, int SH, int SW, int PH, int PW, int DH, int DW, int bm, int bn,
                                int splits, hipStream_t st) {
  if (Cin % 8 || Cout % 8) return MDTF_EINVAL;
  ConvArgs a = make_args(N, H, W, Cin, OH, OW, Cout, KH, KW, SH, SW, PH, PW, DH, DW);
  a.src = (const bf16_t*)x;
  a.dy = (const bf16_t*)dy;
  a.dw = dw;
  a.M = (long long)N * OH * OW;
  a.Ncol = Cout;
  if (bm == 128 && bn == 128) return launch_wgrad<128, 128>(a, splits, st);
  if (bm == 64 && bn == 64) return launch_wgrad<64, 64>(a, splits, st);
  if (bm == 128 && bn == 64) return launch_wgrad<128, 64>(a, splits, st);
  if (bm == 64 && bn == 128) return launch_wgrad<64, 128>(a, splits, st);
  return MDTF_EUNSUPPORTED;
}

MDTF_EXPORT int mdtf_conv_fwd_v2(const void* x, const void* wt, void* y, float* stat_sum, float* stat_sq,
                                 int stat_slots, int N, int H, int W, int Cin, int OH, int OW, int Cout, int KH, int KW,
                                 int SH, int SW, int PH, int PW, int DH, int DW, int bm, int bn, int* mtiles_out,
                                 hipStream_t st) {
  if (Cin % 64 || Cout % 8) return MDTF_EINVAL;
  if (KH * KW > 32 || (long long)N * H * W * Cin * 2 > 0x7fffffffLL) return MDTF_EUNSUPPORTED;
  ConvArgs a = make_args(N, H, W, Cin, OH, OW, Cout, KH, KW, SH, SW, PH, PW, DH, DW);
  a.src = (const bf16_t*)x;
  a.wgt = (const bf16_t*)wt;
  a.out = (bf16_t*)y;
  a.stat_sum = stat_sum;
  a.stat_sq = stat_sq;
  a.stat_slots = stat_slots > 0 ? stat_slots : kStatSlots;
  a.M = (long long)N * OH * OW;
  a.Ncol = Cout;
  a.K = KH * KW * Cin;
  int stages;
  decode_tile(&bm, &stages);
  int rc = stat_sum ? dispatch_fd_v2<0, true>(a, bm, bn, stages, st) : dispatch_fd_v2<0, false>(a, bm, bn, stages, st);
  if (mtiles_out) *mtiles_out = a.mtiles;
  return rc;
}

MDTF_EXPORT int mdtf_conv_dgrad_v2(const void* dy, const void* w, void* dx, int N, int H, int W, int Cin, int OH,
                                   int OW, int Cout, int KH, int KW, int SH, int SW, int PH, int PW, int DH, int DW,
                                   int bm, int bn, int accumulate, const void* bx, const void* bmask,
                                   float* bsum, float* bsq, int bslots, const void* acc_src, const void* acc_mask,
                                   hipStream_t st) {
  if (Cout % 64 || Cin % 8) return MDTF_EINVAL;
  if ((acc_src || acc_mask) && !accumulate) return MDTF_EINVAL;
  if ((long long)N * OH * OW * Cout * 2 > 0x7fffffffLL) return MDTF_EUNSUPPORTED;
  if ((SH != 1 || SW != 1) && (DH != 1 || DW != 1)) return MDTF_EUNSUPPORTED;
  if (ceil_div(KH, SH) * ceil_div(KW, SW) > 32) return MDTF_EUNSUPPORTED;
  ConvArgs a = make_args(N, H, W, Cin, OH, OW, Cout, KH, KW, SH, SW, PH, PW, DH, DW);
  a.src = (const bf16_t*)dy;
  a.wgt = (const bf16_t*)w;
  a.out = (bf16_t*)dx;
  a.accumulate = accumulate;
  a.acc_src = (const bf16_t*)acc_src;
  a.acc_mask = (const uint8_t*)acc_mask;
  a.bx = (const bf16_t*)bx;
  a.bmask = (const uint8_t*)bmask;
  a.bsum = bsum;
  a.bsq = bsq;
  a.bslots = bslots > 0 ? bslots : 1;
  a.Ncol = Cin;
  int stages;
  decode_tile(&bm, &stages);
  if (SH == 1 && SW == 1) {
    a.M = (long long)N * H * W;
    a.K = KH * KW * Cout;
    return dispatch_fd_v2<1, false>(a, bm, bn, stages, st);
  }
  const int C8 = Cin / 8;
  const bool zero_stream = C8 <= 256 && 256 % C8 == 0 && !zero_class_gemm();
  bool zero_pending = false;
  for (int rh = 0; rh < SH; ++rh)
    for (int rw = 0; rw < SW; ++rw) {
      ConvArgs c = a;
      c.cls_h0 = ((rh - PH) % SH + SH) % SH;
      c.cls_w0 = ((rw - PW) % SW + SW) % SW;
      c.cls_Hc = c.cls_h0 < H ? (H - c.cls_h0 + SH - 1) / SH : 0;
      c.cls_Wc = c.cls_w0 < W ? (W - c.cls_w0 + SW - 1) / SW : 0;
      c.cls_kh0 = rh;
      c.cls_kw0 = rw;
      c.cls_th = rh < KH ? (KH - rh + SH - 1) / SH : 0;
      c.cls_tw = rw < KW ? (KW - rw + SW - 1) / SW : 0;
      c.cls_q0h = (c.cls_h0 + PH - rh) / SH;
      c.cls_q0w = (c.cls_w0 + PW - rw) / SW;
      c.M = (long long)N * c.cls_Hc * c.cls_Wc;
      c.K = c.cls_th * c.cls_tw * Cout;
      if (c.M == 0 || (c.K == 0 && accumulate && !bsum && !acc_src)) continue;
      if (c.K == 0 && zero_stream) {
        zero_pending = true;
        continue;
      }
      const int cs = c.K > 64 && stages == 1 ? 2 : stages;
      const int rc = dispatch_fd_v2<2, false>(c, bm, bn, cs, st);
      if (rc) return rc;
    }
  if (zero_pending) {
    if ((long long)N * H * W >= (1LL << 31)) return MDTF_EUNSUPPORTED;
    magic31(static_cast<unsigned>(W), &a.mg_rw, &a.sh_rw);
    magic31(static_cast<unsigned>(H), &a.mg_rh, &a.sh_rh);
    const long long chunks = (long long)N * H * W * C8;
    const int blocks = static_cast<int>(ceil_div(chunks, 256) < 4096 ? ceil_div(chunks, 256) : 4096);
    if (bsum)
      hipLaunchKernelGGL(dgrad_zero_classes<true>, dim3(blocks), dim3(256), 0, st, a, C8);
    else
      hipLaunchKernelGGL(dgrad_zero_classes<false>, dim3(blocks), dim3(256), 0, st, a, C8);
    MDTF_LAUNCH_CHECK();
  }
  return 0;
}

MDTF_EXPORT int mdtf_set_wgrad_fin(const float* psum, const float* psq, int P, const float* gamma, const float* mean,
                                   const float* invstd, float* ws, long long M, int C) {
  if (C < 0 || (C > 0 && (!psum || !psq || !mean || !invstd || !ws || P <= 0 || M <= 0))) return MDTF_EINVAL;
  g_wg_fin = FinReq{psum, psq, gamma, mean, invstd, ws, P, C, M};
  return 0;
}

MDTF_EXPORT int mdtf_set_wgrad_store(int on) {
  g_wg_store = on ? 1 : 0;
  return 0;
}

MDTF_EXPORT int mdtf_set_wgrad_tickets(int* cnt, long long n) {
  g_wg_cnt = cnt;
  g_wg_cnt_n = cnt ? n : 0;
  return 0;
}

MDTF_EXPORT int mdtf_set_slab_stream(hipStream_t s) {
  g_slab_stream = s;
  return 0;
}

MDTF_EXPORT int mdtf_conv_wgrad_v2(const void* x, const void* dy, float* dw, int N, int H, int W, int Cin, int OH,
                                   int OW, int Cout, int KH, int KW, int SH, int SW, int PH, int PW, int DH, int DW,
                                   int bm, int bn, int splits, float* slab, int slab_cap, hipStream_t st) {
  if (Cin % 64 || Cout % 64) return MDTF_EINVAL;
  if ((long long)N * H * W * Cin * 2 > 0x7fffffffLL || (long long)N * OH * OW * Cout * 2 > 0x7fffffffLL)
    return MDTF_EUNSUPPORTED;
  ConvArgs a = make_args(N, H, W, Cin, OH, OW, Cout, KH, KW, SH, SW, PH, PW, DH, DW);
  a.src = (const bf16_t*)x;
  a.dy = (const bf16_t*)dy;
  a.dw = dw;
  a.ld_dy = a.ld_dw = Cout;
  a.M = (long long)N * OH * OW;
  a.Ncol = Cout;
  a.slab = slab;
  a.slab_cap = slab_cap;
  const int w8 = bm / 10000, stages = (bm % 10000) / 1000 ? (bm % 10000) / 1000 : 2;
  bm %= 1000;
  return dispatch_wgrad_v2(a, bm, bn, stages, w8, splits, st);
}

MDTF_EXPORT int mdtf_gemm_wgrad(const void* x, const void* dy, float* dw, long long M, int K, int N, int ld_dy,
                                int ld_dw, int bm, int bn, int stages, int splits, float* slab, int slab_cap,
                                float* dbias, hipStream_t st) {
  if (dbias && bm >= 10000) return MDTF_EUNSUPPORTED;
  if (K % 64 || N % 64 || ld_dy % 8 || M > 0x7fffffff) return MDTF_EINVAL;
  if (M * K * 2 > 0x7fffffffLL || M * (long long)ld_dy * 2 > 0x7fffffffLL) return MDTF_EUNSUPPORTED;
  ConvArgs a = make_args((int)M, 1, 1, K, 1, 1, N, 1, 1, 1, 1, 0, 0, 1, 1);
  a.src = (const bf16_t*)x;
  a.dy = (const bf16_t*)dy;
  a.dw = dw;
  a.ld_dy = ld_dy;
  a.ld_dw = ld_dw;
  a.M = M;
  a.Ncol = N;
  a.slab = slab;
  a.slab_cap = slab_cap;
  a.dbias = dbias;
  return dispatch_wgrad_v2(a, bm % 10000, bn, stages, bm / 10000, splits, st);
}

MDTF_EXPORT int mdtf_gemm_fwd(const void* x, const void* w0, const void* w1, const void* w2, const void* w3, int nseg,
                              int seg_cols, const void* bias, void* y, void* pre, int act, long long M, int K, int bm,
                              int bn, hipStream_t st) {
  if (nseg < 1 || nseg > 4 || K % 64 || bn <= 0 || seg_cols % bn || seg_cols % 64 || M <= 0 || act < 0 || act > 2)
    return MDTF_EINVAL;
  if (M > 0x7fffffff || M * K * 2 > 0x7fffffffLL || (long long)K * seg_cols * 2 > 0x7fffffffLL)
    return MDTF_EUNSUPPORTED;
  ConvArgs a = make_args((int)M, 1, 1, K, 1, 1, nseg * seg_cols, 1, 1, 1, 1, 0, 0, 1, 1);
  a.src = (const bf16_t*)x;
  const void* ws[4] = {w0, w1, w2, w3};
  for (int s = 0; s < 4; ++s) {
    if (s < nseg && !ws[s]) return MDTF_EINVAL;
    a.wseg[s] = (const bf16_t*)(s < nseg ? ws[s] : w0);
  }
  a.seg_cols = seg_cols;
  a.ld_b = seg_cols;
  a.bias = (const bf16_t*)bias;
  a.pre_out = (bf16_t*)pre;
  a.act = act;
  a.out = (bf16_t*)y;
  a.M = M;
  a.Ncol = nseg * seg_cols;
  a.K = K;
  const int w8 = bm / 10000, stages = (bm % 10000) / 1000 ? (bm % 10000) / 1000 : 2;
  bm = w8 * 10000 + bm % 1000;
  return dispatch_fd_v2<3, false>(a, bm, bn, stages, st);
}

MDTF_EXPORT int mdtf_gemm_dgrad_act(const void* dy, const void* w, void* dx, const void* pre, int act, long long M,
                                    int K, int N, int bm, int bn, hipStream_t st) {
  if (N % 64 || K % 8 || M <= 0 || !pre || act < 1 || act > 2) return MDTF_EINVAL;
  if (M > 0x7fffffff || M * N * 2 > 0x7fffffffLL || M * K * 2 > 0x7fffffffLL) return MDTF_EUNSUPPORTED;
  ConvArgs a = make_args((int)M, 1, 1, K, 1, 1, N, 1, 1, 1, 1, 0, 0, 1, 1);
  a.src = (const bf16_t*)dy;
  a.wgt = (const bf16_t*)w;
  a.out = (bf16_t*)dx;
  a.pre_out = (bf16_t*)pre;
  a.act = act;
  a.Ncol = K;
  a.M = M;
  a.K = N;
  const int w8 = bm / 10000, stages = (bm % 10000) / 1000 ? (bm % 10000) / 1000 : 2;
  bm = w8 * 10000 + bm % 1000;
  return dispatch_fd_v2<4, false>(a, bm, bn, stages, st);
}
```

### mdtf/ops/bn.py

```python
import os

import torch

from . import _native as N
from ..train import variables as V

N.register("mdtf_bn_workspace_floats", [N.L, N.I], N.L)
N.register("mdtf_bn_fwd_train", [N.P, N.P, N.P, N.P, N.L, N.I, N.P, N.P, N.P, N.P, N.F, N.F, N.I, N.P, N.P, N.P, N.P])
N.register("mdtf_bn_fwd_eval", [N.P, N.P, N.P, N.L, N.I, N.P, N.P, N.P, N.P, N.F, N.I, N.P, N.P])
N.register("mdtf_bn_bwd", [N.P, N.P, N.P, N.P, N.P, N.L, N.I, N.P, N.P, N.P, N.P, N.P, N.I, N.P, N.I, N.P])
N.register("mdtf_bn_bwd_stats", [N.P, N.P, N.P, N.P, N.P, N.L, N.I, N.P, N.P, N.P, N.P, N.P, N.I, N.P, N.P, N.I,
                                 N.P, N.I, N.P])
N.register("mdtf_bn_fwd_dual", [N.P, N.P, N.P, N.P, N.L, N.I] + [N.P] * 6 + [N.I, N.P, N.P] + [N.P] * 6 + [N.I, N.P, N.P]
           + [N.F, N.F, N.P, N.P])
N.register("mdtf_bn_fwd_stats", [N.P, N.P, N.P, N.P, N.L, N.I, N.P, N.P, N.P, N.P, N.F, N.F, N.I, N.P, N.P, N.P, N.P,
                                 N.I, N.P, N.P])
N.register("mdtf_bn_relu_maxpool_fwd", [N.P, N.P, N.P] + [N.I] * 12 + [N.P] * 4 + [N.F, N.F] + [N.P] * 4 + [N.I]
           + [N.P, N.P])
N.register("mdtf_maxpool_bn_bwd", [N.P] * 4 + [N.I] * 12 + [N.P] * 8 + [N.P])
N.register("mdtf_bn_bwd_dual", [N.P] * 6 + [N.L, N.I] + [N.P] * 7 + [N.I] + [N.P] * 6 + [N.P])
N.register("mdtf_bn_bwd_finalize_ws", [N.L, N.I, N.P, N.P, N.P, N.P, N.P, N.I, N.P, N.P])
N.register("mdtf_bn_dx_ws", [N.P, N.P, N.P, N.P, N.P, N.L, N.I, N.P, N.P, N.P, N.I, N.I, N.P])
N.register("mdtf_bn_fwd_coeffs", [N.L, N.I, N.P, N.P, N.P, N.P, N.F, N.F, N.P, N.P, N.P, N.P, N.I, N.P, N.P])
N.register("mdtf_bn_apply_ss", [N.P, N.P, N.P, N.L, N.I, N.P, N.I, N.P])


FUSED_BWD = [0]
EARLY_FIN = os.environ.get("MDTF_BN_EARLY_FIN", "0") == "1"
WG_FIN = os.environ.get("MDTF_BN_WG_FIN", "1") == "1"
WG_FIN_USED = [0]
EARLY_USED = [0]
_FIN_SIDE = {}


def _early_finalize(sbuf, g, mean, invstd, M, C):
    dev = sbuf.device
    main = torch.cuda.current_stream(dev)
    side = _FIN_SIDE.get(dev)
    if side is None:
        side = _FIN_SIDE[dev] = torch.cuda.Stream(device=dev)
    side.wait_stream(main)
    with torch.cuda.stream(side):
        ws = torch.empty(5 * C, dtype=torch.float32, device=dev)
        N.check(N.fn("mdtf_bn_bwd_finalize_ws")(M, C, N.ptr(g), N.ptr(mean), N.ptr(invstd), N.ptr(sbuf[0]),
                                                N.ptr(sbuf[1]), int(sbuf.shape[1]), N.ptr(ws), N.stream_ptr()),
                "bn_bwd_finalize_ws")
        ev = torch.cuda.Event()
        ev.record(side)
    ws.record_stream(main)
    for t in (sbuf, g, mean, invstd):
        if t is not None:
            t.record_stream(side)
    return ws, ev
DEFER_SHORTCUT = os.environ.get("MDTF_DEFER_SHORTCUT_BN", "1") != "0"
ON_CONSUMER = os.environ.get("MDTF_BN_ON_CONSUMER", "0") == "1"
_PENDING = {}
ON_CONSUMER_USED = [0]


def take_pending(y):
    if not _PENDING:
        return None
    ent = _PENDING.get(y.data_ptr())
    if ent is None or ent[0].shape != y.shape or ent[0].dtype != y.dtype:
        return None
    del _PENDING[y.data_ptr()]
    return ent


def apply_pending(ent):
    y, x, ss, mask = ent
    C = x.shape[-1]
    N.check(N.fn("mdtf_bn_apply_ss")(N.ptr(x), N.ptr(y), N.ptr(mask), x.numel() // C, C, N.ptr(ss), 1,
                                     N.stream_ptr()), "bn_apply_ss")


def materialize(y):
    ent = take_pending(y)
    if ent is not None:
        apply_pending(ent)
    return y


def _check(x):
    if x.dtype != torch.bfloat16:
        raise TypeError("mdtf BN kernel expects bf16 NHWC activations, got %s" % x.dtype)
    if x.shape[-1] % 8:
        raise ValueError("mdtf BN kernel needs C % 8 == 0 (C=%d)" % x.shape[-1])


def _f32(t):
    return None if t is None else t.detach().float().contiguous()


BWD_TRACE = [] if os.environ.get("MDTF_BN_TRACE") == "1" else None
DUAL_DZ = os.environ.get("MDTF_DUAL_DZ", "0") == "1"
DUAL_FUSED = os.environ.get("MDTF_DUAL_BWD_FUSED", "1") != "0"
DUAL_BWD = [0]


class _BNTrain(torch.autograd.Function):
    @staticmethod
    def forward(ctx, x, gamma, beta, residual, mm, mv, decay, eps, relu, stats, on_consumer=False):
        from . import actsink
        ctx.set_materialize_grads(False)
        ctx.res_sink = actsink.sink_of(residual)
        if ctx.res_sink is not None:
            ctx.res_sink.register()
        x = x.contiguous()
        C = x.shape[-1]
        M = x.numel() // C
        y = torch.empty_like(x)
        mean = torch.empty(C, dtype=torch.float32, device=x.device)
        invstd = torch.empty_like(mean)
        mask = torch.empty(M * C // 8, dtype=torch.uint8, device=x.device) if relu else None
        g, b = _f32(gamma), _f32(beta)
        res = residual.contiguous() if residual is not None else None
        if stats is not None and on_consumer and relu and res is None:
            psum, psq, P = stats
            ws = torch.empty(2 * C, dtype=torch.float32, device=x.device)
            N.check(N.fn("mdtf_bn_fwd_coeffs")(M, C, N.ptr(g), N.ptr(b), N.ptr(mm), N.ptr(mv), float(decay),
                                               float(eps), N.ptr(mean), N.ptr(invstd), N.ptr(psum), N.ptr(psq),
                                               int(P), N.ptr(ws), N.stream_ptr()), "bn_fwd_coeffs")
            from . import conv as _conv
            _conv.stats_consumed(x.device)
            _PENDING[y.data_ptr()] = (y, x, ws, mask)
        elif stats is not None:
            psum, psq, P = stats
            ws = torch.empty(2 * C, dtype=torch.float32, device=x.device)
            N.check(N.fn("mdtf_bn_fwd_stats")(N.ptr(x), N.ptr(res), N.ptr(y), N.ptr(mask), M, C, N.ptr(g), N.ptr(b),
                                              N.ptr(mm), N.ptr(mv), float(decay), float(eps), int(relu), N.ptr(mean),
                                              N.ptr(invstd), N.ptr(psum), N.ptr(psq), int(P), N.ptr(ws),
                                              N.stream_ptr()), "bn_fwd_stats")
            from . import conv as _conv
            _conv.stats_consumed(x.device)
        else:
            ws = torch.empty(int(N.fn("mdtf_bn_workspace_floats")(M, C)), dtype=torch.float32, device=x.device)
            N.check(N.fn("mdtf_bn_fwd_train")(N.ptr(x), N.ptr(res), N.ptr(y), N.ptr(mask), M, C, N.ptr(g), N.ptr(b),
                                              N.ptr(mm), N.ptr(mv), float(decay), float(eps), int(relu), N.ptr(mean),
                                              N.ptr(invstd), N.ptr(ws), N.stream_ptr()), "bn_fwd_train")
        ctx.save_for_backward(x, mask if mask is not None else y.new_empty(0), g, mean, invstd)
        ctx.has_res = residual is not None
        ctx.relu = relu
        ctx.has_gamma = gamma is not None
        ctx.has_beta = beta is not None
        ctx.sinks = (V.grad_sink(gamma) if gamma is not None else None,
                     V.grad_sink(beta) if beta is not None else None)
        ctx.like = (gamma, beta)
        ctx.out_sink = actsink.attach(y)
        if ctx.out_sink is not None:
            fin = None
            if EARLY_FIN and x.is_cuda and not N.deterministic():
                def fin(sbuf, g=g, mean=mean, invstd=invstd, M=M, C=C):
                    return _early_finalize(sbuf, g, mean, invstd, M, C)
            wgf = (g, mean, invstd, M, C) if (WG_FIN and x.is_cuda and not N.deterministic()) else None
            ctx.out_sink.stat_req = (x, mask, fin, wgf)
        return y

    @staticmethod
    def backward(ctx, dy):
        x, mask, g, mean, invstd = ctx.saved_tensors
        pstats = None
        early = None
        why = "no_sink"
        if ctx.out_sink is not None:
            pstats = ctx.out_sink.take_stats()
            early = ctx.out_sink.take_early()
            why = "no_epilogue_stats" if pstats is None else "fused"
            if early is not None and (pstats is None or dy is not None):
                if early[1] is not None:
                    torch.cuda.current_stream(x.device).wait_event(early[1])
                early = None
            if pstats is not None and dy is not None:
                from . import conv as _conv
                _conv.bwd_stats_release(pstats, False)
                pstats = None
                why = "autograd_part"
            dy = ctx.out_sink.take(dy)
            ctx.out_sink.stat_req = None
        if BWD_TRACE is not None:
            BWD_TRACE.append((tuple(x.shape), ctx.has_res, why))
        if dy is None:
            if early is not None and early[1] is not None:
                torch.cuda.current_stream(x.device).wait_event(early[1])
            return (None,) * 11
        dy = dy.contiguous()
        C = x.shape[-1]
        M = x.numel() // C
        dx = torch.empty_like(x)
        dres, accum = None, 0
        rs = ctx.res_sink if ctx.needs_input_grad[3] else None
        pending = False
        if ctx.has_res:
            from . import actsink
            if (rs is not None and ctx.relu and actsink.MASKED_RESIDUAL and rs.idle()
                    and not rs.completing()):
                pending = True
            else:
                if rs is not None:
                    dres, acc = rs.target()
                    accum = int(acc)
                if dres is None:
                    dres = torch.empty_like(x)
        sg, sb = ctx.sinks
        dgamma = sg.grad if sg is not None else torch.zeros(C, dtype=torch.float32, device=x.device)
        dbeta = sb.grad if sb is not None else torch.zeros(C, dtype=torch.float32, device=x.device)
        if pstats is not None and early is not None:
            from . import conv as _conv
            ws, ev = early
            if ev is not None:
                torch.cuda.current_stream(x.device).wait_event(ev)
                EARLY_USED[0] += 1
            else:
                WG_FIN_USED[0] += 1
            N.check(N.fn("mdtf_bn_dx_ws")(N.ptr(dy), N.ptr(x), N.ptr(mask if ctx.relu else None), N.ptr(dx),
                                          N.ptr(dres), M, C, N.ptr(ws), N.ptr(dgamma), N.ptr(dbeta), int(ctx.relu),
                                          accum, N.stream_ptr()), "bn_dx_ws")
            _conv.bwd_stats_release(pstats, True)
            FUSED_BWD[0] += 1
        elif pstats is not None:
            from . import conv as _conv
            ws = torch.empty(3 * C, dtype=torch.float32, device=x.device)
            N.check(N.fn("mdtf_bn_bwd_stats")(N.ptr(dy), N.ptr(x), N.ptr(mask if ctx.relu else None), N.ptr(dx),
                                              N.ptr(dres), M, C, N.ptr(g), N.ptr(mean), N.ptr(invstd), N.ptr(dgamma),
                                              N.ptr(dbeta), int(ctx.relu), N.ptr(pstats[0]), N.ptr(pstats[1]),
                                              int(pstats.shape[1]), N.ptr(ws), accum, N.stream_ptr()), "bn_bwd_stats")
            _conv.bwd_stats_release(pstats, True)
            FUSED_BWD[0] += 1
        else:
            ws = torch.empty(int(N.fn("mdtf_bn_workspace_floats")(M, C)), dtype=torch.float32, device=x.device)
            N.check(N.fn("mdtf_bn_bwd")(N.ptr(dy), N.ptr(x), N.ptr(mask if ctx.relu else None), N.ptr(dx), N.ptr(dres), M,
                                        C, N.ptr(g),
                                        N.ptr(mean), N.ptr(invstd), N.ptr(dgamma), N.ptr(dbeta), int(ctx.relu),
                                        N.ptr(ws), accum, N.stream_ptr()), "bn_bwd")
        if pending:
            rs.defer_masked(dy, mask)
        elif rs is not None and dres is not None:
            rs.written(dres)
            dres = None
        gamma, beta = ctx.like
        rg = (V.grad_marker(gamma) if sg is not None else dgamma) if ctx.has_gamma else None
        rb = (V.grad_marker(beta) if sb is not None else dbeta) if ctx.has_beta else None
        return (dx, rg, rb, dres, None, None, None, None, None, None, None)


class DeferredBN(object):

    def __init__(self, x, gamma, beta, moving_mean, moving_var, decay, epsilon, stats):
        self.x, self.gamma, self.beta = x, gamma, beta
        self.moving_mean, self.moving_var = moving_mean, moving_var
        self.decay, self.epsilon, self.stats = decay, epsilon, stats
        self.shape = x.shape
        self.dtype = x.dtype

    def materialize(self):
        return _BNTrain.apply(self.x, self.gamma, self.beta, None, self.moving_mean, self.moving_var, self.decay,
                              self.epsilon, False, self.stats)


class _BNTrainDual(torch.autograd.Function):

    @staticmethod
    def forward(ctx, x, gamma, beta, mm, mv, r, gamma2, beta2, mm2, mv2, decay, eps, stats, stats2):
        from . import actsink
        ctx.set_materialize_grads(False)
        x = x.contiguous()
        r = r.contiguous()
        C = x.shape[-1]
        M = x.numel() // C
        y = torch.empty_like(x)
        mean, invstd = (torch.empty(C, dtype=torch.float32, device=x.device) for _ in range(2))
        mean2, invstd2 = (torch.empty(C, dtype=torch.float32, device=x.device) for _ in range(2))
        mask = torch.empty(M * C // 8, dtype=torch.uint8, device=x.device)
        g, b, g2, b2 = _f32(gamma), _f32(beta), _f32(gamma2), _f32(beta2)
        ws = torch.empty(4 * C, dtype=torch.float32, device=x.device)
        (ps, pq, P), (ps2, pq2, P2) = stats, stats2
        N.check(N.fn("mdtf_bn_fwd_dual")(N.ptr(x), N.ptr(r), N.ptr(y), N.ptr(mask), M, C, N.ptr(g), N.ptr(b),
                                         N.ptr(mm), N.ptr(mv), N.ptr(ps), N.ptr(pq), int(P), N.ptr(mean),
                                         N.ptr(invstd), N.ptr(g2), N.ptr(b2), N.ptr(mm2), N.ptr(mv2), N.ptr(ps2),
                                         N.ptr(pq2), int(P2), N.ptr(mean2), N.ptr(invstd2), float(decay), float(eps),
                                         N.ptr(ws), N.stream_ptr()), "bn_fwd_dual")
        from . import conv as _conv
        _conv.stats_consumed(x.device)
        ctx.save_for_backward(x, mask, g, mean, invstd, r, g2, mean2, invstd2)
        ctx.sinks = tuple(V.grad_sink(t) for t in (gamma, beta, gamma2, beta2))
        ctx.like = (gamma, beta, gamma2, beta2)
        ctx.out_sink = actsink.attach(y)
        if ctx.out_sink is not None:
            ctx.out_sink.stat_req = (x, mask)
        return y

    @staticmethod
    def backward(ctx, dy):
        x, mask, g, mean, invstd, r, g2, mean2, invstd2 = ctx.saved_tensors
        pstats = None
        if ctx.out_sink is not None:
            pstats = ctx.out_sink.take_stats()
            if pstats is not None and dy is not None:
                from . import conv as _conv
                _conv.bwd_stats_release(pstats, False)
                pstats = None
            dy = ctx.out_sink.take(dy)
            ctx.out_sink.stat_req = None
        if dy is None:
            return (None,) * 14
        dy = dy.contiguous()
        C = x.shape[-1]
        M = x.numel() // C
        dx = torch.empty_like(x)
        if DUAL_FUSED and not DUAL_DZ:
            grads = [sk.grad if sk is not None else torch.zeros(C, dtype=torch.float32, device=x.device)
                     for sk in ctx.sinks]
            dr = torch.empty_like(r)
            ws = torch.empty(2 * int(N.fn("mdtf_bn_workspace_floats")(M, C)), dtype=torch.float32, device=x.device)
            ps, pq, P = (pstats[0], pstats[1], int(pstats.shape[1])) if pstats is not None else (None, None, 0)
            N.check(N.fn("mdtf_bn_bwd_dual")(N.ptr(dy), N.ptr(x), N.ptr(r), N.ptr(mask), N.ptr(dx), N.ptr(dr), M, C,
                                             N.ptr(g), N.ptr(mean), N.ptr(invstd), N.ptr(grads[0]), N.ptr(grads[1]),
                                             N.ptr(ps), N.ptr(pq), P, N.ptr(g2), N.ptr(mean2), N.ptr(invstd2),
                                             N.ptr(grads[2]), N.ptr(grads[3]), N.ptr(ws), N.stream_ptr()),
                    "bn_bwd_dual")
            DUAL_BWD[0] += 1
            if pstats is not None:
                from . import conv as _conv
                _conv.bwd_stats_release(pstats, True)
                FUSED_BWD[0] += 1
            out = [V.grad_marker(t) if sk is not None else gr for t, sk, gr in zip(ctx.like, ctx.sinks, grads)]
            return (dx, out[0], out[1], None, None, dr, out[2], out[3], None, None, None, None, None, None)
        dz = torch.empty_like(x) if DUAL_DZ else None
        grads = [sk.grad if sk is not None else torch.zeros(C, dtype=torch.float32, device=x.device)
                 for sk in ctx.sinks]
        if pstats is not None:
            from . import conv as _conv
            ws = torch.empty(3 * C, dtype=torch.float32, device=x.device)
            N.check(N.fn("mdtf_bn_bwd_stats")(N.ptr(dy), N.ptr(x), N.ptr(mask), N.ptr(dx), N.ptr(dz), M, C, N.ptr(g),
                                              N.ptr(mean), N.ptr(invstd), N.ptr(grads[0]), N.ptr(grads[1]), 1,
                                              N.ptr(pstats[0]), N.ptr(pstats[1]), int(pstats.shape[1]), N.ptr(ws), 0,
                                              N.stream_ptr()), "bn_bwd_stats")
            _conv.bwd_stats_release(pstats, True)
            FUSED_BWD[0] += 1
        else:
            ws = torch.empty(int(N.fn("mdtf_bn_workspace_floats")(M, C)), dtype=torch.float32, device=x.device)
            N.check(N.fn("mdtf_bn_bwd")(N.ptr(dy), N.ptr(x), N.ptr(mask), N.ptr(dx), N.ptr(dz), M, C, N.ptr(g),
                                        N.ptr(mean), N.ptr(invstd), N.ptr(grads[0]), N.ptr(grads[1]), 1, N.ptr(ws), 0,
                                        N.stream_ptr()), "bn_bwd")
        dr = torch.empty_like(r)
        ws2 = torch.empty(int(N.fn("mdtf_bn_workspace_floats")(M, C)), dtype=torch.float32, device=x.device)
        N.check(N.fn("mdtf_bn_bwd")(N.ptr(dz if dz is not None else dy), N.ptr(r),
                                    N.ptr(mask) if dz is None else None, N.ptr(dr), None, M, C, N.ptr(g2),
                                    N.ptr(mean2), N.ptr(invstd2), N.ptr(grads[2]), N.ptr(grads[3]), int(dz is None),
                                    N.ptr(ws2), 0, N.stream_ptr()), "bn_bwd")
        out = []
        for t, sk, gr in zip(ctx.like, ctx.sinks, grads):
            out.append(V.grad_marker(t) if sk is not None else gr)
        return (dx, out[0], out[1], None, None, dr, out[2], out[3], None, None, None, None, None, None)


FUSED_STEM = os.environ.get("MDTF_FUSED_STEM", "1") != "0"
STEM_POOLED_STATS = os.environ.get("MDTF_STEM_POOLED_STATS", "1") != "0"


class _BNReluMaxPool(torch.autograd.Function):

    @staticmethod
    def forward(ctx, x, gamma, beta, mm, mv, decay, eps, stats, geo):
        from . import actsink
        ctx.set_materialize_grads(False)
        x = x.contiguous()
        n, h, w, c = x.shape
        oh, ow, kh, kw, sh, sw, pt, pl = geo
        y = torch.empty((n, oh, ow, c), dtype=x.dtype, device=x.device)
        arg = torch.empty((n, oh, ow, c), dtype=torch.uint8, device=x.device)
        mean, invstd = (torch.empty(c, dtype=torch.float32, device=x.device) for _ in range(2))
        ss = torch.empty(2 * c, dtype=torch.float32, device=x.device)
        psum, psq, P = stats
        g, b = _f32(gamma), _f32(beta)
        N.check(N.fn("mdtf_bn_relu_maxpool_fwd")(N.ptr(x), N.ptr(y), N.ptr(arg), n, h, w, c, oh, ow, kh, kw, sh, sw,
                                                 pt, pl, N.ptr(g), N.ptr(b), N.ptr(mm), N.ptr(mv), float(decay),
                                                 float(eps), N.ptr(mean), N.ptr(invstd), N.ptr(psum), N.ptr(psq),
                                                 int(P), N.ptr(ss), N.stream_ptr()), "bn_relu_maxpool_fwd")
        from . import conv as _conv
        _conv.stats_consumed(x.device)
        ctx.save_for_backward(x, arg, g, mean, invstd, ss, y if STEM_POOLED_STATS else None)
        ctx.geo = geo
        ctx.sinks = (V.grad_sink(gamma) if gamma is not None else None,
                     V.grad_sink(beta) if beta is not None else None)
        ctx.like = (gamma, beta)
        ctx.out_sink = actsink.attach(y)
        return y

    @staticmethod
    def backward(ctx, dy):
        if ctx.out_sink is not None:
            dy = ctx.out_sink.take(dy)
        if dy is None:
            return (None,) * 9
        x, arg, g, mean, invstd, ss, yp = ctx.saved_tensors
        dy = dy.contiguous()
        n, h, w, c = x.shape
        oh, ow, kh, kw, sh, sw, pt, pl = ctx.geo
        dx = torch.empty_like(x)
        sg, sb = ctx.sinks
        dgamma = sg.grad if sg is not None else torch.zeros(c, dtype=torch.float32, device=x.device)
        dbeta = sb.grad if sb is not None else torch.zeros(c, dtype=torch.float32, device=x.device)
        ws = torch.empty(int(N.fn("mdtf_bn_workspace_floats")(n * h * w, c)), dtype=torch.float32, device=x.device)
        N.check(N.fn("mdtf_maxpool_bn_bwd")(N.ptr(dy), N.ptr(arg), N.ptr(x), N.ptr(dx), n, h, w, c, oh, ow, kh, kw,
                                            sh, sw, pt, pl, N.ptr(g), N.ptr(mean), N.ptr(invstd), N.ptr(dgamma),
                                            N.ptr(dbeta), N.ptr(ss), N.ptr(ws), N.ptr(yp), N.stream_ptr()),
                "maxpool_bn_bwd")
        gamma, beta = ctx.like
        rg = (V.grad_marker(gamma) if sg is not None else dgamma) if gamma is not None else None
        rb = (V.grad_marker(beta) if sb is not None else dbeta) if beta is not None else None
        return (dx, rg, rb, None, None, None, None, None, None)


def bn_relu_maxpool_nhwc(x, gamma, beta, moving_mean, moving_var, decay, epsilon, stats, geo):
    _check(x)
    return _BNReluMaxPool.apply(x, gamma, beta, moving_mean, moving_var, decay, epsilon, stats, geo)


def batch_norm_nhwc(x, gamma, beta, moving_mean, moving_var, training, decay, epsilon, relu, residual, stats=None,
                    on_consumer=False):
    _check(x)
    if isinstance(residual, DeferredBN):
        d = residual
        if training and relu and stats is not None and d.stats is not None and d.x.shape == x.shape:
            return _BNTrainDual.apply(x, gamma, beta, moving_mean, moving_var, d.x, d.gamma, d.beta, d.moving_mean,
                                      d.moving_var, decay, epsilon, stats, d.stats)
        residual = d.materialize()
    if residual is not None and residual.dtype != x.dtype:
        residual = residual.to(x.dtype)
    if training:
        oc = bool(on_consumer and ON_CONSUMER and relu and residual is None and stats is not None
                  and not N.deterministic())
        return _BNTrain.apply(x, gamma, beta, residual, moving_mean, moving_var, decay, epsilon, bool(relu), stats,
                              oc)
    x = x.contiguous()
    C = x.shape[-1]
    M = x.numel() // C
    y = torch.empty_like(x)
    ws = torch.empty(2 * C, dtype=torch.float32, device=x.device)
    res = residual.contiguous() if residual is not None else None
    N.check(N.fn("mdtf_bn_fwd_eval")(N.ptr(x), N.ptr(res), N.ptr(y), M, C, N.ptr(_f32(gamma)), N.ptr(_f32(beta)),
                                     N.ptr(moving_mean), N.ptr(moving_var), float(epsilon), int(bool(relu)),
                                     N.ptr(ws), N.stream_ptr()), "bn_fwd_eval")
    return y
```

### mdtf/ops/conv.py

```python
import collections
import ctypes
import json
import os

import torch
import torch.nn.functional as F

from . import _native as N
from . import winograd
from ..train import variables as V

N.register("mdtf_conv_fwd", [N.P, N.P, N.P, N.P, N.P] + [N.I] * 18 + [N.P, N.P])
N.register("mdtf_conv_dgrad", [N.P, N.P, N.P] + [N.I] * 17 + [N.P])
N.register("mdtf_conv_wgrad", [N.P, N.P, N.P] + [N.I] * 18 + [N.P])
N.register("mdtf_conv_fwd_v2", [N.P, N.P, N.P, N.P, N.P] + [N.I] * 18 + [N.P, N.P])
N.register("mdtf_conv_dgrad_v2", [N.P, N.P, N.P] + [N.I] * 18 + [N.P, N.P, N.P, N.P, N.I, N.P, N.P, N.P])
N.register("mdtf_conv_wgrad_v2", [N.P, N.P, N.P] + [N.I] * 18 + [N.P, N.I, N.P])
N.register("mdtf_set_slab_stream", [N.P])
N.register("mdtf_set_wgrad_store", [N.I])
N.register("mdtf_set_wgrad_fin", [N.P, N.P, N.I, N.P, N.P, N.P, N.P, N.L, N.I])

_SLAB_MODE = os.environ.get("MDTF_WGRAD_SLAB", "dense")
WGRAD_SLAB = _SLAB_MODE not in ("0", "", "false", "dense")
DENSE_WGRAD_SLAB = _SLAB_MODE not in ("0", "", "false")


def wgrad_splits(M, R, Cout, bm, bn, ver, splits):
    kt_total = -(-M // 64)
    tiles = -(-R // bm) * -(-Cout // bn)
    if splits < 1:
        splits = -(-(512 if ver == 3 else 1024) // tiles)
    splits = max(1, min(splits, kt_total))
    ks = -(-kt_total // splits)
    return -(-kt_total // ks)


def wgrad_slab(M, R, Cout, bm, bn, ver, splits, device, dense=False, force=None):
    on = (DENSE_WGRAD_SLAB if dense else WGRAD_SLAB) if force is None else force
    if not on or N.deterministic():
        return None, 0
    sp = wgrad_splits(M, R, Cout, bm, bn, ver, splits)
    if sp < 2:
        return None, 0
    if WGRAD_INK:
        return torch.empty(sp * (-(-R // 256) * 256) * (-(-Cout // 256) * 256), dtype=torch.float32,
                           device=device), sp
    return torch.empty(sp * R * Cout, dtype=torch.float32, device=device), sp


WGRAD_INK = os.environ.get("MDTF_WGRAD_INK", "0") == "1"
N.register("mdtf_set_wgrad_tickets", [N.P, N.L])


class wgrad_tickets:

    def __init__(self, slab):
        self.on = WGRAD_INK and slab is not None and slab.is_cuda
        self.device = slab.device if self.on else None

    def __enter__(self):
        if self.on:
            from . import mm
            t = mm._tickets(self.device, 4096)
            N.fn("mdtf_set_wgrad_tickets")(N.ptr(t), t.numel())
        return self

    def __exit__(self, *exc):
        if self.on:
            N.fn("mdtf_set_wgrad_tickets")(None, 0)
        return False

_HERE = os.path.dirname(os.path.abspath(__file__))
TUNED_BATCH = 256
TABLE_PATH = os.environ.get("MDTF_CONV_TABLE") or os.path.join(_HERE, "conv_table.json")
_TABLE = None


def table():
    global _TABLE
    if _TABLE is None:
        _TABLE = {}
        if os.path.exists(TABLE_PATH):
            with open(TABLE_PATH) as f:
                _TABLE = json.load(f)
    return _TABLE


def shape_key(pass_, x_shape, w_shape, stride, pads, dil):
    n, h, w, c = x_shape
    kh, kw, ci, co = w_shape
    return "%s:%d,%d,%d,%d:%d,%d,%d:%d,%d:%d,%d,%d,%d:%d,%d" % (
        pass_, n, h, w, c, kh, kw, co, stride[0], stride[1], pads[0], pads[1], pads[2], pads[3], dil[0], dil[1])


def _default_tile(ncol):
    return (128, 128) if ncol % 128 == 0 else (128, 64)


def v2_ok(pass_, c, co, stride=(1, 1), taps=1, dil=(1, 1)):
    if taps > 32:
        return False
    if pass_ == "fwd":
        return c % 64 == 0 and co % 8 == 0
    if pass_ == "dgrad":
        return co % 64 == 0 and c % 8 == 0 and (tuple(stride) == (1, 1) or tuple(dil) == (1, 1))
    if pass_ == "wgrad":
        return c % 64 == 0 and co % 64 == 0
    return False


def _default_wgrad_tile(r, co):
    return (128 if r >= 128 else 64, 128 if co % 128 == 0 else 64)


class Mdtf(collections.namedtuple("Mdtf", "backend bm bn splits ver stages")):
    v2 = sink_aware = property(lambda self: self.ver in (2, 3))
    stat_rows = property(lambda self: self.bm)


class Ws(collections.namedtuple("Ws", "backend tile")):
    stat_rows, sink_aware = None, True


class Pp(collections.namedtuple("Pp", "backend tile")):
    rows = stat_rows = property(lambda self: PP_TILES[self.tile][0])
    sink_aware = True


class Lib(collections.namedtuple("Lib", "backend")):
    stat_rows, sink_aware = None, False


def _mdtf(tile, splits=0, ver=1, stages=2):
    return Mdtf("mdtf", tile[0], tile[1], splits, ver, stages)


def choose(pass_, x_shape, w_shape, stride, pads, dil):
    n, h, w, c = x_shape
    kh, kw, ci, co = w_shape
    forced = os.environ.get("MDTF_CONV", "auto")
    native_ok = c % 8 == 0 and co % 8 == 0
    if pass_ in ("fwd", "wgrad") and not native_ok and stem_ok(x_shape, w_shape, dil):
        if pass_ == "fwd" or (co == 64 and kh <= 8 and not N.deterministic()):
            return Lib("stem")
    if not native_ok or forced == "miopen":
        return Lib("miopen")
    if pass_ in ("fwd", "dgrad") and winograd.enabled() and winograd.eligible(w_shape, stride, pads, dil, c, co):
        return Lib("winograd")
    ent = table().get(shape_key(pass_, x_shape, w_shape, stride, pads, dil))
    if ent is None and n != TUNED_BATCH:
        ent = table().get(shape_key(pass_, (TUNED_BATCH, h, w, c), w_shape, stride, pads, dil))
    if N.deterministic() and pass_ == "wgrad":
        ver = 2 if v2_ok(pass_, c, co, stride, kh * kw, dil) else 1
        return _mdtf(_default_wgrad_tile(kh * kw * ci, co), 1, ver)
    if forced == "auto" and ent is not None:
        if ent["backend"] in ("miopen", "winograd"):
            return Lib(ent["backend"])
        if ent.get("ver") == 5:
            if pp_ok(pass_, c, co, stride, kh, kw, ent["tile"]):
                return Pp("pp", ent["tile"])
            ent = ent.get("prev")
            if ent is None:
                return _mdtf(_default_tile(co if pass_ == "fwd" else ci), 0, 2)
            if ent["backend"] in ("miopen", "winograd"):
                return Lib(ent["backend"])
        if ent.get("ver") == 4:
            if N.deterministic():
                return _mdtf(_default_tile(co if pass_ == "fwd" else c), 0, 2)
            return Ws("ws", tuple(ent["ws"]))
        return Mdtf("mdtf", ent["bm"], ent["bn"], ent.get("splits", 0), ent.get("ver", 1), ent.get("stages", 2))
    ver = 2 if (forced in ("auto", "mdtf2") and v2_ok(pass_, c, co, stride, kh * kw, dil)) else 1
    if pass_ == "wgrad":
        return _mdtf(_default_wgrad_tile(kh * kw * ci, co), 0, ver)
    return _mdtf(_default_tile(co if pass_ == "fwd" else ci), 0, ver, 3 if ver == 2 else 2)


def _nchw(x):
    return x.permute(0, 3, 1, 2)


def _w_oihw(w):
    return w.permute(3, 2, 0, 1).contiguous(memory_format=torch.channels_last)


def _sym(pads):
    pt, pb, pl, pr = pads
    return pt == pb and pl == pr


def miopen_fwd(x, w, stride, pads, dil):
    pt, pb, pl, pr = pads
    xc = _nchw(x)
    if not _sym(pads):
        xc = F.pad(xc, (pl, pr, pt, pb))
        pt = pl = 0
    y = F.conv2d(xc, _w_oihw(w).to(x.dtype), None, stride, (pt, pl), dil)
    return y.permute(0, 2, 3, 1).contiguous()


def miopen_bwd(x, w, dy, stride, pads, dil, need_dx, need_dw):
    pt, pb, pl, pr = pads
    xc = _nchw(x)
    if not _sym(pads):
        xc = F.pad(xc, (pl, pr, pt, pb))
        ph, pw = 0, 0
    else:
        ph, pw = pt, pl
    wt = _w_oihw(w).to(x.dtype)
    dyc = _nchw(dy)
    dx_c, dw_c, _ = torch.ops.aten.convolution_backward(
        dyc, xc, wt, None, list(stride), [ph, pw], list(dil), False, [0, 0], 1, [need_dx, need_dw, False])
    dx = dw = None
    if need_dx:
        if not _sym(pads):
            dx_c = dx_c[:, :, pt:pt + x.shape[1], pl:pl + x.shape[2]]
        dx = dx_c.permute(0, 2, 3, 1).contiguous()
    if need_dw:
        dw = dw_c.permute(2, 3, 1, 0).contiguous()
    return dx, dw


def _geo(x_shape, w_shape, out_hw, stride, pads, dil):
    n, h, wd, c = x_shape
    kh, kw, ci, co = w_shape
    return [n, h, wd, c, out_hw[0], out_hw[1], co, kh, kw, stride[0], stride[1], pads[0], pads[2], dil[0], dil[1]]


def _stat_args(stats):
    s_sum, s_sq = stats if stats is not None else (None, None)
    return s_sum, s_sq, s_sum.shape[0] if s_sum is not None else 0


def _bn_args(bn_stats):
    return bn_stats if bn_stats is not None else (None, None, None, None, 0)


def _acc_args(acc_src):
    return acc_src if acc_src is not None else (None, None)


def transpose_filter(w):
    cached = _WT.get(w)
    if cached is not None:
        return cached
    from . import kernels
    kh, kw, ci, co = w.shape
    return kernels.transpose_brs(w.reshape(1, kh * kw * ci, co), 1, kh * kw * ci, co).view(co, kh * kw * ci)


N.register("mdtf_transpose_multi", [N.P, N.I, N.I, N.P])


class _FilterTransposes(object):

    def __init__(self):
        self.entries = {}
        self.order = []
        self.desc = None
        self.tiles = 0
        self.active = False
        self.fresh = False

    def clear(self):
        self.entries.clear()
        del self.order[:]
        self.desc = None
        self.tiles = 0
        self.fresh = False

    def step_begin(self):
        self.active = os.environ.get("MDTF_FILTER_CACHE", "1") != "0"
        self.fresh = False

    def step_end(self):
        self.active = False
        self.fresh = False

    def _rebuild(self):
        import struct
        recs, tile = [], 0
        for key in self.order:
            w, wt = self.entries[key]
            r = w.numel() // w.shape[-1]
            sdim = w.shape[-1]
            ts = -(-sdim // 64)
            recs.append(struct.pack("<qqqii", w.data_ptr(), wt.data_ptr(), r | (sdim << 32), tile, ts))
            tile += ts * -(-r // 64)
        raw = torch.frombuffer(bytearray(b"".join(recs)), dtype=torch.uint8)
        self.desc = raw.to(self.order and self.entries[self.order[0]][0].device)
        self.tiles = tile

    @staticmethod
    def _is_shadow(w):
        flat = getattr(V.get_store(), "flat", None)
        if flat is None:
            return False
        sp = w.untyped_storage().data_ptr()
        return any(g.shadow is not None and g.shadow.untyped_storage().data_ptr() == sp for g in flat.groups)

    def get(self, w):
        if not self.active or not w.is_cuda or w.dtype != torch.bfloat16 or not w.is_contiguous():
            return None
        key = (w.data_ptr(), tuple(w.shape))
        ent = self.entries.get(key)
        if ent is None:
            if torch.cuda.is_current_stream_capturing() or not self._is_shadow(w):
                return None
            from . import kernels
            kh, kw, ci, co = w.shape
            wt = torch.empty((co, kh * kw * ci), dtype=w.dtype, device=w.device)
            self.entries[key] = (w, wt)
            self.order.append(key)
            self.desc = None
            wt.copy_(kernels.transpose_brs(w.reshape(1, kh * kw * ci, co), 1, kh * kw * ci, co).view(co, -1))
            return wt
        if not self.fresh:
            if self.desc is None:
                if torch.cuda.is_current_stream_capturing():
                    return None
                self._rebuild()
            N.check(N.fn("mdtf_transpose_multi")(N.ptr(self.desc), len(self.order), self.tiles, N.stream_ptr()),
                    "transpose_multi")
            self.fresh = True
        return ent[1]


_WT = _FilterTransposes()


def _v2_code(bm, stages, ver):
    if stages >= 10:
        return bm + 1000 * stages + 100000 * (2 if ver == 3 else 1)
    return bm + 1000 * stages + (10000 if ver == 3 else 0)


def mdtf_fwd(x, w, out_hw, stride, pads, dil, bm, bn, stats=None, ver=1, stages=2):
    n = x.shape[0]
    co = w.shape[3]
    y = torch.empty((n, out_hw[0], out_hw[1], co), dtype=x.dtype, device=x.device)
    mt = N.I(0)
    s_sum, s_sq, slots = _stat_args(stats)
    geo = _geo(x.shape, w.shape, out_hw, stride, pads, dil)
    if ver in (2, 3):
        wt = transpose_filter(w)
        N.check(N.fn("mdtf_conv_fwd_v2")(N.ptr(x), N.ptr(wt), N.ptr(y), N.ptr(s_sum), N.ptr(s_sq), slots, *geo,
                                         _v2_code(bm, stages, ver), bn, ctypes.byref(mt), N.stream_ptr()),
                "conv_fwd_v2")
        return y
    N.check(N.fn("mdtf_conv_fwd")(N.ptr(x), N.ptr(w), N.ptr(y), N.ptr(s_sum), N.ptr(s_sq), slots, *geo, bm, bn,
                                  ctypes.byref(mt), N.stream_ptr()), "conv_fwd")
    return y


def mdtf_dgrad(dy, w, x_shape, stride, pads, dil, bm, bn, ver=1, stages=2, out=None, accumulate=False,
               bn_stats=None, acc_src=None):
    dx = out if out is not None else torch.empty(x_shape, dtype=dy.dtype, device=dy.device)
    geo = _geo(x_shape, w.shape, dy.shape[1:3], stride, pads, dil)
    if ver in (2, 3):
        bx, bmask, bsum, bsq, bslots = _bn_args(bn_stats)
        ag, am = _acc_args(acc_src)
        N.check(N.fn("mdtf_conv_dgrad_v2")(N.ptr(dy), N.ptr(w), N.ptr(dx), *geo, _v2_code(bm, stages, ver), bn,
                                           int(bool(accumulate) or acc_src is not None), N.ptr(bx), N.ptr(bmask),
                                           N.ptr(bsum), N.ptr(bsq), int(bslots), N.ptr(ag), N.ptr(am),
                                           N.stream_ptr()), "conv_dgrad_v2")
        return dx
    if acc_src is not None:
        raise ValueError("a masked accumulate source needs the v2 kernel")
    if bn_stats is not None:
        raise ValueError("BN statistics in the dgrad epilogue need the v2 kernel")
    if accumulate:
        raise ValueError("accumulating dgrad needs the v2 kernel")
    N.check(N.fn("mdtf_conv_dgrad")(N.ptr(dy), N.ptr(w), N.ptr(dx), *geo, bm, bn, N.stream_ptr()), "conv_dgrad")
    return dx


N.register("mdtf_conv_ws", [N.P, N.P, N.P] + [N.I] * 16 + [N.I, N.I] +
           [N.P, N.P, N.I, N.P, N.P, N.P, N.P, N.I, N.I, N.P, N.P, N.P])


def ws_ok(pass_, c, co, stride, kh, kw, dil=(1, 1)):
    if pass_ == "fwd":
        red, ncol = c, co
    elif pass_ == "dgrad":
        if tuple(stride) != (1, 1):
            return False
        red, ncol = co, c
    else:
        return False
    return (red % 32 == 0 and ncol % 64 == 0 and kh * kw <= 32 and kh * kw * red >= 64
            and 64 * kh * kw * red * 2 <= 160 * 1024)


N.register("mdtf_stem_pack4", [N.P, N.P] + [N.I] * 8 + [N.P, N.P] + [N.I] * 4 + [N.P])
N.register("mdtf_conv_ws_stem", [N.P, N.P, N.P] + [N.I] * 10 + [N.P, N.P, N.I, N.P])
N.register("mdtf_stem_conv_rows", [N.P, N.P, N.P] + [N.I] * 10 + [N.P, N.P, N.I, N.P])
N.register("mdtf_stem_wgrad", [N.P, N.P, N.P] + [N.I] * 11 + [N.P])
STEM = os.environ.get("MDTF_STEM", "mdtf")
STEM_KERNEL = os.environ.get("MDTF_STEM_KERNEL", "rows")
_STEM_PACK_W = os.environ.get("MDTF_STEM_PACK_W", "1") != "0"
STEM_TILE = (4, 4, 1, 4)


def stem_ok(x_shape, w_shape, dil):
    kh, kw, ci, co = w_shape
    return (STEM != "miopen" and ci <= 4 and kw <= 8 and co % 64 == 0 and tuple(dil) == (1, 1)
            and x_shape[2] * ci <= 16384
            and os.environ.get("MDTF_CONV", "auto") != "miopen")


STEM_WG_BLOCKS = int(os.environ.get("MDTF_STEM_WG_BLOCKS", "768"))


def stem_wgrad(x4, dy, w_shape, stride, out=None, blocks=0):
    kh, kw, ci, co = w_shape
    dw = out if out is not None else torch.zeros(w_shape, dtype=torch.float32, device=dy.device)
    n, h4, w4, _ = x4.shape
    N.check(N.fn("mdtf_stem_wgrad")(N.ptr(x4), N.ptr(dy), N.ptr(dw), n, h4, w4, dy.shape[1], dy.shape[2],
                                    stride[0], stride[1], kh, kw, ci, int(blocks or STEM_WG_BLOCKS),
                                    N.stream_ptr()), "stem_wgrad")
    return dw


def stem_fwd(x, w, out_hw, stride, pads, stats=None, tile=None, keep_x4=None):
    n, h, wd, c = x.shape
    kh, kw, ci, co = w.shape
    pt, pb, pl, pr = pads
    khp = -(-kh // 4) * 4
    h4 = max(h + pt + pb, (out_hw[0] - 1) * stride[0] + khp)
    w4 = max(wd + pl + pr, (out_hw[1] - 1) * stride[1] + 8)
    w4 += w4 & 1
    x4 = torch.empty((n, h4, w4, 4), dtype=x.dtype, device=x.device)
    assert ci == c, "stem filter channels %d != input channels %d" % (ci, c)
    w = w.to(x.dtype).contiguous()
    if _STEM_PACK_W:
        wt = torch.empty((co, khp * 32), dtype=x.dtype, device=x.device)
    else:
        wp = torch.zeros((khp, 8, 4, co), dtype=x.dtype, device=x.device)
        wp[:kh, :kw, :ci].copy_(w)
        wt = wp.view(khp * 32, co).t().contiguous()
    N.check(N.fn("mdtf_stem_pack4")(N.ptr(x), N.ptr(x4), n, h, wd, c, pt, pl, h4, w4,
                                    N.ptr(w if _STEM_PACK_W else None), N.ptr(wt), kh, kw, co, khp,
                                    N.stream_ptr()), "stem_pack4")
    y = torch.empty((n, out_hw[0], out_hw[1], co), dtype=x.dtype, device=x.device)
    s_sum, s_sq, slots = _stat_args(stats)
    if STEM_KERNEL == "rows" and tile is None and out_hw[1] <= 128:
        N.check(N.fn("mdtf_stem_conv_rows")(N.ptr(x4), N.ptr(wt), N.ptr(y), n, h4, w4, out_hw[0], out_hw[1], co, kh,
                                            khp, stride[0], stride[1], N.ptr(s_sum), N.ptr(s_sq), slots,
                                            N.stream_ptr()), "stem_conv_rows")
    else:
        N.check(N.fn("mdtf_conv_ws_stem")(N.ptr(x4), N.ptr(wt), N.ptr(y), n, h4, w4, out_hw[0], out_hw[1], co, khp,
                                          stride[0], stride[1], _ws_code(*(tile or STEM_TILE)), N.ptr(s_sum),
                                          N.ptr(s_sq), slots, N.stream_ptr()), "conv_ws_stem")
    if keep_x4 is not None:
        keep_x4.append(x4)
    return y


def ws_depth_ok(k_total, d):
    ks = k_total // 32
    if ks == 2:
        return d in (2, 4)
    if ks == 3:
        return d == 3
    if ks == 4:
        return d == 4
    return ks > 4 and d in (3, 4, 6) and ks % d == 0


N.register("mdtf_conv3_rows", [N.P, N.P, N.P] + [N.I] * 4 + [N.P, N.P, N.I, N.P, N.P, N.P])
CONV_ROWS = os.environ.get("MDTF_CONV_ROWS", "1") != "0"
DUAL_FUSED = [0]


def rows_ok(h_w, c, co, kh, kw, stride, pads, dil):
    return (CONV_ROWS and c == 64 and co == 64 and kh == 3 and kw == 3 and tuple(stride) == (1, 1)
            and tuple(pads) == (1, 1, 1, 1) and tuple(dil) == (1, 1) and h_w[1] == 56)


def _ws_code(tp, nw, cg, d=4):
    return tp + 10 * nw + 100 * cg + 1000 * d


def ws_fwd(x, wt, kh, kw, out_hw, stride, pads, dil, tile, stats=None, grid_cap=0, out=None):
    n, h, wd, c = x.shape
    co = wt.shape[0]
    y = out if out is not None else torch.empty((n, out_hw[0], out_hw[1], co), dtype=x.dtype, device=x.device)
    s_sum, s_sq, slots = _stat_args(stats)
    if rows_ok((h, wd), c, co, kh, kw, stride, pads, dil) and tuple(out_hw) == (h, wd):
        N.check(N.fn("mdtf_conv3_rows")(N.ptr(x), N.ptr(wt), N.ptr(y), n, h, wd, 0, N.ptr(s_sum), N.ptr(s_sq), slots,
                                        N.ptr(None), N.ptr(None), N.stream_ptr()), "conv3_rows_fwd")
        return y
    N.check(N.fn("mdtf_conv_ws")(N.ptr(x), N.ptr(wt), N.ptr(y), n, h, wd, c, out_hw[0], out_hw[1], co, kh, kw,
                                 stride[0], stride[1], pads[0], pads[2], dil[0], dil[1], 0, _ws_code(*tile),
                                 int(grid_cap), N.ptr(s_sum), N.ptr(s_sq), slots, N.ptr(None), N.ptr(None),
                                 N.ptr(None), N.ptr(None), 0, 0, N.ptr(None), N.ptr(None), N.stream_ptr()),
            "conv_ws_fwd")
    return y


N.register("mdtf_conv_ws_bna", [N.P, N.P, N.P] + [N.I] * 7 + [N.P, N.P, N.I, N.P, N.P, N.P, N.P])


def bna_ok(ch, x_shape, w_shape, stride, pads, dil):
    kh, kw, ci, co = w_shape
    return (ch.backend == "ws" and kh == 1 and kw == 1 and tuple(stride) == (1, 1) and tuple(pads) == (0, 0, 0, 0)
            and tuple(dil) == (1, 1) and ci in (64, 96, 128) and ws_depth_ok(ci, ch.tile[3] if len(ch.tile) > 3 else 4))


def ws_fwd_bna(x, wt, tile, stats, pend):
    a, xin, ss, mask = pend
    n, h, wd, c = xin.shape
    co = wt.shape[0]
    y = torch.empty((n, h, wd, co), dtype=xin.dtype, device=xin.device)
    s_sum, s_sq = stats
    N.check(N.fn("mdtf_conv_ws_bna")(N.ptr(xin), N.ptr(wt), N.ptr(y), n, h, wd, c, co, _ws_code(*tile), 0,
                                     N.ptr(s_sum), N.ptr(s_sq), s_sum.shape[0], N.ptr(ss), N.ptr(a), N.ptr(mask),
                                     N.stream_ptr()), "conv_ws_bna")
    return y


def _ws_stats_tile(tile, bn_stats):
    return tile if bn_stats is None else (2,) + tuple(tile[1:])


def ws_dgrad(dy, w, x_shape, pads, dil, tile, out=None, accumulate=False, bn_stats=None, grid_cap=0, acc_src=None):
    n, h, wd, ci = x_shape
    kh, kw, _, co = w.shape
    dx = out if out is not None else torch.empty(x_shape, dtype=dy.dtype, device=dy.device)
    ph = (kh - 1) * dil[0] - pads[0]
    pw = (kw - 1) * dil[1] - pads[2]
    bx, bmask, bsum, bsq, bslots = _bn_args(bn_stats)
    ag, am = _acc_args(acc_src)
    if (not accumulate and acc_src is None and rows_ok((h, wd), co, ci, kh, kw, (1, 1), pads, dil)
            and tuple(dy.shape[1:3]) == (h, wd)):
        N.check(N.fn("mdtf_conv3_rows")(N.ptr(dy), N.ptr(w), N.ptr(dx), n, h, wd, 1, N.ptr(bsum), N.ptr(bsq),
                                        int(bslots), N.ptr(bx), N.ptr(bmask), N.stream_ptr()), "conv3_rows_dgrad")
        return dx
    N.check(N.fn("mdtf_conv_ws")(N.ptr(dy), N.ptr(w), N.ptr(dx), n, dy.shape[1], dy.shape[2], co, h, wd, ci, kh, kw,
                                 1, 1, ph, pw, dil[0], dil[1], 1, _ws_code(*tile), int(grid_cap), N.ptr(None),
                                 N.ptr(None), 0, N.ptr(bx), N.ptr(bmask), N.ptr(bsum), N.ptr(bsq), int(bslots),
                                 int(bool(accumulate) or acc_src is not None), N.ptr(ag), N.ptr(am),
                                 N.stream_ptr()), "conv_ws_dgrad")
    return dx


N.register("mdtf_conv_ws_dual", [N.P] * 5 + [N.I] * 10 + [N.P, N.P, N.P, N.P, N.I, N.P])
DUAL_DGRAD = os.environ.get("MDTF_DUAL_DGRAD", "1") != "0"
DUAL_TILE = tuple(int(v) for v in os.environ.get("MDTF_DUAL_TILE", "2,8,1").split(","))


def proj_deferrable(w_shape, stride, pads, dil):
    return (DUAL_DGRAD and w_shape[0] == 1 and w_shape[1] == 1 and tuple(stride)[0] == tuple(stride)[1] > 1
            and tuple(pads) == (0, 0, 0, 0) and tuple(dil) == (1, 1) and w_shape[3] % 32 == 0)


def dual_ok(x_shape, w_shape, stride, pads, dil, pconv):
    if pconv is None or not (w_shape[0] == 1 and w_shape[1] == 1 and tuple(stride) == (1, 1)
                             and tuple(pads) == (0, 0, 0, 0) and tuple(dil) == (1, 1)):
        return False
    dy2, w2, s2 = pconv[:3]
    n, h, wd, c = x_shape
    c1, c2 = w_shape[3], w2.shape[3]
    return (c % 64 == 0 and c1 % 128 == 0 and c2 % 128 == 0 and 128 * (c1 + c2) <= 160 * 1024 and h > 1 and wd > 1
            and w2.shape[2] == c and tuple(s2) == (2, 2) and tuple(dy2.shape) == (n, -(-h // 2), -(-wd // 2), c2))


def ws_dual(dy, w, pconv, x_shape, tile=None, bn_stats=None):
    n, h, wd, c = x_shape
    dy2, w2, s2 = pconv[:3]
    dx = torch.empty(x_shape, dtype=dy.dtype, device=dy.device)
    bx, bmask, bsum, bsq, bslots = _bn_args(bn_stats)
    tp, nw, cg = _ws_stats_tile(tile or DUAL_TILE, bn_stats)
    N.check(N.fn("mdtf_conv_ws_dual")(N.ptr(dy), N.ptr(w), N.ptr(dy2), N.ptr(w2), N.ptr(dx), n, h, wd, c,
                                      w.shape[3], dy2.shape[1], dy2.shape[2], dy2.shape[3], s2[0],
                                      _ws_code(tp, nw, cg), N.ptr(bx), N.ptr(bmask), N.ptr(bsum), N.ptr(bsq),
                                      int(bslots), N.stream_ptr()), "conv_ws_dual")
    return dx


N.register("mdtf_conv_pp", [N.I, N.P, N.P, N.P] + [N.I] * 15 + [N.I, N.P, N.P, N.I, N.I] + [N.P] * 6 + [N.I, N.P])
PP_TILES = {0: (256, 256), 1: (256, 128), 2: (128, 256), 3: (128, 128), 4: (256, 192), 5: (128, 192)}


def pp_ok(pass_, c, co, stride, kh, kw, tile=None):
    g = c if pass_ == "fwd" else co
    if pass_ not in ("fwd", "dgrad") or g < 64 or g & (g - 1) or kh * kw > 32:
        return False
    if pass_ == "fwd":
        return co % 8 == 0
    return tuple(stride) == (1, 1) and (tile is None or c % PP_TILES[tile][1] == 0)


def pp_fwd(x, w, out_hw, stride, pads, dil, tile, stats=None, out=None):
    n = x.shape[0]
    co = w.shape[3]
    y = out if out is not None else torch.empty((n, out_hw[0], out_hw[1], co), dtype=x.dtype, device=x.device)
    s_sum, s_sq, slots = _stat_args(stats)
    N.check(N.fn("mdtf_conv_pp")(1, N.ptr(x), N.ptr(transpose_filter(w)), N.ptr(y),
                                 *_geo(x.shape, w.shape, out_hw, stride, pads, dil), int(tile), N.ptr(s_sum),
                                 N.ptr(s_sq), slots, 0, None, None, None, None, None, None, 0, N.stream_ptr()),
            "conv_pp_fwd")
    return y


def pp_dgrad(dy, w, x_shape, pads, dil, tile, out=None, accumulate=False, bn_stats=None, acc_src=None):
    dx = out if out is not None else torch.empty(x_shape, dtype=dy.dtype, device=dy.device)
    geo = _geo(x_shape, w.shape, dy.shape[1:3], (1, 1), pads, dil)
    bx, bmask, bsum, bsq, bslots = _bn_args(bn_stats)
    ag, am = _acc_args(acc_src)
    N.check(N.fn("mdtf_conv_pp")(2, N.ptr(dy), N.ptr(w), N.ptr(dx), *geo, int(tile), None, None, 0,
                                 int(bool(accumulate) or acc_src is not None), N.ptr(ag), N.ptr(am), N.ptr(bx),
                                 N.ptr(bmask), N.ptr(bsum), N.ptr(bsq), int(bslots), N.stream_ptr()), "conv_pp_dgrad")
    return dx


def mdtf_wgrad(x, dy, w_shape, stride, pads, dil, bm, bn, splits, out=None, ver=1, stages=2, store=False, fin=None):
    dw = torch.zeros(w_shape, dtype=torch.float32, device=x.device) if out is None else out
    n, h, wd, c = x.shape
    kh, kw, ci, co = w_shape
    if ver in (2, 3):
        force = None
        if _SLAB_MODE not in ("0", "1"):
            ent = table().get(shape_key("wgrad", tuple(x.shape), tuple(w_shape), stride, pads, dil))
            if ent is not None and "slab" in ent:
                force = bool(ent["slab"])
        slab, cap = wgrad_slab(n * dy.shape[1] * dy.shape[2], kh * kw * ci, co, bm, bn, ver, int(splits), x.device,
                               force=force)
        if store is not False and store is not True:
            var = store
            store = slab is not None and not WGRAD_INK and V.claim_store(var)
            if not store:
                V.note_accumulate(var)
        if store:
            N.fn("mdtf_set_wgrad_store")(1)
        if fin is not None:
            xs, sbuf, g, mean, invstd, M, C = fin
            fws = torch.empty(5 * C, dtype=torch.float32, device=x.device)
            N.check(N.fn("mdtf_set_wgrad_fin")(N.ptr(sbuf[0]), N.ptr(sbuf[1]), int(sbuf.shape[1]), N.ptr(g),
                                               N.ptr(mean), N.ptr(invstd), N.ptr(fws), int(M), int(C)), "wgrad_fin")
        try:
            with slab_side(slab if out is not None else None), wgrad_tickets(slab):
                N.check(N.fn("mdtf_conv_wgrad_v2")(N.ptr(x), N.ptr(dy), N.ptr(dw), n, h, wd, c, dy.shape[1],
                                                   dy.shape[2], co, kh, kw, stride[0], stride[1], pads[0], pads[2],
                                                   dil[0], dil[1], _v2_code(bm, stages, ver), bn, int(splits),
                                                   N.ptr(slab), cap, N.stream_ptr()), "conv_wgrad_v2")
        finally:
            if store:
                N.fn("mdtf_set_wgrad_store")(0)
            if fin is not None:
                N.fn("mdtf_set_wgrad_fin")(None, None, 0, None, None, None, None, 0, 0)
        if fin is not None:
            xs.early = (fws, None)
        return dw
    N.check(N.fn("mdtf_conv_wgrad")(N.ptr(x), N.ptr(dy), N.ptr(dw), n, h, wd, c, dy.shape[1], dy.shape[2], co, kh,
                                    kw, stride[0], stride[1], pads[0], pads[2], dil[0], dil[1], bm, bn, int(splits),
                                    N.stream_ptr()), "conv_wgrad")
    return dw


BWD_STATS = os.environ.get("MDTF_BN_BWD_STATS", "1") != "0"
STAT_SLOTS = 64
MAX_STAT_SLOTS = int(os.environ.get("MDTF_BN_MAX_SLOTS", "128"))
_STATS = {}


def _stats_buffer(co, device, slots=STAT_SLOTS):
    ent = _STATS.get(device)
    need = 2 * slots * co
    if ent is None or ent[0].numel() < need:
        ent = [torch.zeros(max(need, 2 * STAT_SLOTS * 2048), dtype=torch.float32, device=device), False]
        _STATS[device] = ent
    if ent[1]:
        ent[0].zero_()
    ent[1] = True
    return ent[0][:need].view(2, slots, co)


def stats_consumed(device):
    ent = _STATS.get(device)
    if ent is not None:
        ent[1] = False


def stat_slots(mtiles):
    if N.deterministic():
        return mtiles
    slots = STAT_SLOTS
    while slots < MAX_STAT_SLOTS and slots * 8 < mtiles:
        slots *= 2
    return slots


WGRAD_STREAM = os.environ.get("MDTF_WGRAD_STREAM", "0") == "1"
_SIDE = {}
_PENDING = set()


def _side_stream(device):
    s = _SIDE.get(device)
    if s is None:
        s = torch.cuda.Stream(device=device)
        _SIDE[device] = s
    return s


SLAB_SIDE = os.environ.get("MDTF_SLAB_SIDE", "0") == "1"


class slab_side:

    def __init__(self, slab, setter="mdtf_set_slab_stream"):
        self.slab = slab if (SLAB_SIDE and slab is not None and slab.is_cuda) else None
        self.setter = setter

    def __enter__(self):
        if self.slab is not None:
            self.side = _side_stream(self.slab.device)
            N.fn(self.setter)(ctypes.c_void_p(self.side.cuda_stream))
        return self

    def __exit__(self, *exc):
        if self.slab is not None:
            N.fn(self.setter)(None)
            self.slab.record_stream(self.side)
            _PENDING.add(self.slab.device)
        return False


def join_side_streams():
    for dev in list(_PENDING):
        torch.cuda.current_stream(dev).wait_stream(_SIDE[dev])
    _PENDING.clear()


_BSTATS = {}


def bwd_stats_acquire(device, C, slots):
    pool = _BSTATS.setdefault((device, C, slots), [])
    return pool.pop() if pool else torch.zeros((2, slots, C), dtype=torch.float32, device=device)


def _early_finalize(xs, sbuf):
    req = xs.stat_req
    if req is not None and len(req) > 2 and req[2] is not None:
        xs.early = req[2](sbuf)
        return None
    if req is not None and len(req) > 3 and req[3] is not None:
        return (xs, sbuf) + tuple(req[3])
    return None


def bwd_stats_release(buf, zeroed):
    if not zeroed:
        buf.zero_()
    _BSTATS.setdefault((buf.device, buf.shape[2], buf.shape[1]), []).append(buf)


def _fwd_stats(ch, want_stats, rows, co, device):
    if not want_stats or ch.backend in ("winograd", "miopen"):
        return None
    slots = STAT_SLOTS if ch.stat_rows is None else stat_slots(-(-rows // ch.stat_rows))
    buf = (torch.zeros((2, slots, co), dtype=torch.float32, device=device) if want_stats == 2
           else _stats_buffer(co, device, slots))
    return buf[0], buf[1]


def _bwd_stats(xs, stat_rows, x):
    if xs.stat_req is None or not xs.completing() or not BWD_STATS or N.deterministic():
        return None, None
    bx, bmask = xs.stat_req[:2]
    slots = STAT_SLOTS if stat_rows is None else stat_slots(-(-(x.numel() // x.shape[3]) // stat_rows))
    sbuf = bwd_stats_acquire(x.device, x.shape[3], slots)
    return (bx, bmask, sbuf[0], sbuf[1], sbuf.shape[1]), sbuf


def _launch_fwd(ch, x, w, out_hw, stride, pads, dil, stats, pend, keep_x4=None):
    if ch.backend == "mdtf":
        return mdtf_fwd(x, w, out_hw, stride, pads, dil, ch.bm, ch.bn, stats, ch.ver, ch.stages)
    if ch.backend == "pp":
        return pp_fwd(x, w, out_hw, stride, pads, dil, ch.tile, stats)
    if ch.backend == "stem":
        return stem_fwd(x, w, out_hw, stride, pads, stats, keep_x4=keep_x4)
    if ch.backend == "ws":
        if pend is not None:
            from . import bn as _bn
            _bn.ON_CONSUMER_USED[0] += 1
            return ws_fwd_bna(x, transpose_filter(w), ch.tile, stats, pend)
        return ws_fwd(x, transpose_filter(w), w.shape[0], w.shape[1], out_hw, stride, pads, dil, ch.tile, stats)
    if ch.backend == "winograd":
        return winograd.winograd_fwd(x, w, out_hw, pads)
    return miopen_fwd(x, w, stride, pads, dil)


def _launch_dgrad(cd, dy, w, x_shape, stride, pads, dil, out=None, accumulate=False, bn_stats=None, acc_src=None):
    sink = dict(out=out, accumulate=accumulate, bn_stats=bn_stats, acc_src=acc_src)
    if cd.backend == "mdtf":
        return mdtf_dgrad(dy, w, x_shape, stride, pads, dil, cd.bm, cd.bn, cd.ver, cd.stages, **sink)
    if cd.backend == "pp":
        return pp_dgrad(dy, w, x_shape, pads, dil, cd.tile, **sink)
    if cd.backend == "ws":
        return ws_dgrad(dy, w, x_shape, pads, dil, _ws_stats_tile(cd.tile, bn_stats), **sink)
    assert cd.backend == "winograd" and out is None and bn_stats is None and acc_src is None, cd
    return winograd.winograd_dgrad(dy, w, x_shape, pads)


def _dgrad_into_sink(xs, cd, dy, w, x, stride, pads, dil, pconv=None):
    if pconv is None:
        buf, acc, pend = xs.target_ex()
        bst, sbuf = _bwd_stats(xs, cd.stat_rows, x)
        dx = _launch_dgrad(cd, dy, w, x.shape, stride, pads, dil, out=buf, accumulate=acc, bn_stats=bst,
                           acc_src=pend)
    else:
        bst, sbuf = _bwd_stats(xs, None, x)
        dx = ws_dual(dy, w, pconv, x.shape, bn_stats=bst)
    xs.written(dx)
    if bst is None:
        return None
    xs.stats = sbuf
    return _early_finalize(xs, sbuf)


def _launch_wgrad(cw, x, dy, w_shape, stride, pads, dil, **kw):
    return mdtf_wgrad(x, dy, w_shape, stride, pads, dil, cw.bm, cw.bn, cw.splits, ver=cw.ver, stages=cw.stages, **kw)


class _Conv(torch.autograd.Function):
    @staticmethod
    def forward(ctx, x, w, stride, pads, dil, out_hw, want_stats):
        from . import actsink
        ctx.set_materialize_grads(False)
        ctx.x_sink = actsink.sink_of(x)
        if ctx.x_sink is not None:
            ctx.x_sink.register()
        from . import bn as _bn
        pend = _bn.take_pending(x)
        x = x.contiguous()
        w = w.contiguous()
        ch = choose("fwd", x.shape, w.shape, stride, pads, dil)
        if pend is not None and not (want_stats and bna_ok(ch, x.shape, w.shape, stride, pads, dil)):
            _bn.apply_pending(pend)
            pend = None
        stats = _fwd_stats(ch, want_stats, x.shape[0] * out_hw[0] * out_hw[1], w.shape[3], x.device)
        keep = []
        y = _launch_fwd(ch, x, w, out_hw, stride, pads, dil, stats, pend, keep_x4=keep)
        ctx.stem_x4 = keep[0] if keep else None
        ctx.save_for_backward(x, w)
        ctx.args = (stride, pads, dil)
        ctx.w_dtype = w.dtype
        ctx.sink = V.grad_sink(w)
        if not want_stats:
            return y
        psum, psq = stats if stats is not None else (torch.empty(0, device=x.device),) * 2
        ctx.mark_non_differentiable(psum, psq)
        return y, psum, psq

    @staticmethod
    def backward(ctx, dy, *unused):
        x, w = ctx.saved_tensors
        if dy is None:
            return None, None, None, None, None, None, None
        stride, pads, dil = ctx.args
        dy = dy.contiguous()
        need_dx, need_dw = ctx.needs_input_grad[0], ctx.needs_input_grad[1]
        fin_job = None
        dx = dw = None
        cd = choose("dgrad", x.shape, w.shape, stride, pads, dil) if need_dx else None
        cw = choose("wgrad", x.shape, w.shape, stride, pads, dil) if need_dw else None
        if need_dw and cw.backend == "stem" and ctx.stem_x4 is None:
            cw = Lib("miopen")
        lib_dx = need_dx and cd.backend == "miopen"
        lib_dw = need_dw and cw.backend == "miopen"
        sink = ctx.sink
        if lib_dx or lib_dw:
            dx, dw = miopen_bwd(x, w, dy, stride, pads, dil, lib_dx, lib_dw)
            if lib_dw and sink is not None:
                sink.grad.add_(dw)
                dw = V.grad_marker(w)
        xs = ctx.x_sink if need_dx else None
        if xs is not None and not lib_dx:
            if (xs.idle() and not xs.completing() and proj_deferrable(w.shape, stride, pads, dil)
                    and cd.backend in ("mdtf", "pp") and cd.sink_aware):
                xs.defer_conv(dy, w, tuple(stride), lambda out, acc, xshape=tuple(x.shape): _launch_dgrad(
                    cd, dy, w, xshape, stride, pads, dil, out=out, accumulate=acc))
                need_dx = False
            elif dual_ok(x.shape, w.shape, stride, pads, dil, xs.pconv) and xs.buf is None and xs.pend is None:
                fin_job = _dgrad_into_sink(xs, cd, dy, w, x, stride, pads, dil, pconv=xs.take_conv())
                DUAL_FUSED[0] += 1
                need_dx = False
            elif cd.sink_aware:
                fin_job = _dgrad_into_sink(xs, cd, dy, w, x, stride, pads, dil)
                need_dx = False
        if need_dx and not lib_dx:
            dx = _launch_dgrad(cd, dy, w, x.shape, stride, pads, dil)
        if xs is not None and dx is not None:
            xs.adopt_or_add(dx)
            dx = None
        if need_dw and not lib_dw:
            if cw.backend == "stem":
                dw = stem_wgrad(ctx.stem_x4, dy, w.shape, stride, out=sink.grad if sink is not None else None)
                ctx.stem_x4 = None
            elif sink is not None:
                if WGRAD_STREAM and x.is_cuda:
                    V.note_accumulate(sink)
                    side = _side_stream(x.device)
                    side.wait_stream(torch.cuda.current_stream(x.device))
                    with torch.cuda.stream(side):
                        mdtf_wgrad(x, dy, w.shape, stride, pads, dil, cw.bm, cw.bn, cw.splits, out=sink.grad,
                                   ver=cw.ver, stages=cw.stages)
                    x.record_stream(side)
                    dy.record_stream(side)
                    _PENDING.add(x.device)
                else:
                    if not cw.v2:
                        V.note_accumulate(sink)
                    _launch_wgrad(cw, x, dy, w.shape, stride, pads, dil, out=sink.grad,
                                  store=sink if cw.v2 else False, fin=fin_job if cw.v2 else None)
                    fin_job = None
            else:
                dw = _launch_wgrad(cw, x, dy, w.shape, stride, pads, dil)
            dw = V.grad_marker(w) if sink is not None else dw.to(ctx.w_dtype)
        return dx, dw, None, None, None, None, None


def _out_hw(x, w, stride, pads, dil):
    n, h, wd, c = x.shape
    kh, kw, _, co = w.shape
    oh = (h + pads[0] + pads[1] - ((kh - 1) * dil[0] + 1)) // stride[0] + 1
    ow = (wd + pads[2] + pads[3] - ((kw - 1) * dil[1] + 1)) // stride[1] + 1
    return oh, ow


def _apply(x, w, stride, pads, dil, want_stats):
    if x.dtype != torch.bfloat16:
        raise TypeError("mdtf conv kernels take bf16 activations, got %s" % x.dtype)
    if w.dtype != x.dtype:
        w = w.to(x.dtype)
    return _Conv.apply(x, w, tuple(stride), tuple(pads), tuple(dil), _out_hw(x, w, stride, pads, dil), want_stats)


def conv2d_nhwc(x, w, stride, pads, dil, bias=None, act=None):
    y = _apply(x, w, stride, pads, dil, False)
    if bias is not None or act is not None:
        from . import kernels
        y = kernels.bias_act(y, bias, act)
    return y


def conv2d_stats_nhwc(x, w, stride, pads, dil, private=False):
    y, psum, psq = _apply(x, w, stride, pads, dil, 2 if private else True)
    if psum.numel() == 0:
        return y, None
    return y, (psum, psq, psum.shape[0])


def conv2d_dgrad_nhwc(x, w, out_shape, stride, pads):
    n, oh, ow, co = out_shape
    kh, kw, wco, wci = w.shape
    wb = w.to(x.dtype).contiguous()
    ch = choose("dgrad", (n, oh, ow, co), (kh, kw, co, wci), stride, pads, (1, 1))
    if ch.backend == "mdtf":
        return _ConvT.apply(x, wb, tuple(stride), tuple(pads), (n, oh, ow, co), ch.bm, ch.bn, ch.ver, ch.stages)
    xc = x.permute(0, 3, 1, 2)
# ... 32 lines not shown
```

Baseline: 13030 images/sec.

## Fuse second BN reduction into dgrad epilogue and prefetch epilogue operands early

For the dual-BN backward (main branch plus shortcut), the dgrad conv epilogue now also accumulates sum(dy*r) for the shortcut input into a third stats row. The dual BN backward can then skip its separate reduction kernel over dy and r and finalize both BNs in one shared kernel. Separately, the dgrad kernel loads its epilogue operands (old accumulator, x, mask, r) before the main K loop when K is small, hiding that latency. The cost is higher register and LDS use in the epilogue, more atomics, and a fallback to the non-persistent path when bx2 is set.

```diff
diff --git a/mdtf/csrc/bn.hip b/mdtf/csrc/bn.hip
--- a/mdtf/csrc/bn.hip
+++ b/mdtf/csrc/bn.hip
@@ -434,6 +434,20 @@
 
 __global__ void __launch_bounds__(1024) bn_finalize_bwd2(FinBwd a0, FinBwd a1, long long M, int C) {
   finalize_bwd(blockIdx.y ? a1 : a0, M, C);
+}
+
+__global__ void __launch_bounds__(1024) bn_finalize_bwd_shared(FinBwd a0, FinBwd a1, long long M, int C) {
+  finalize_bwd(a0, M, C);
+  __syncthreads();
+  finalize_bwd(a1, M, C);
+  const int c = blockIdx.x * kFinCh + threadIdx.x % kFinCh, grp = threadIdx.x / kFinCh;
+  if (c < C) {
+    for (int r = grp; r < a0.gx; r += kFinGroups) {
+      const_cast<float*>(a0.p0)[(long long)r * C + c] = 0.f;
+      const_cast<float*>(a0.p1)[(long long)r * C + c] = 0.f;
+      const_cast<float*>(a1.p1)[(long long)r * C + c] = 0.f;
+    }
+  }
 }
 
 template <bool RELU, bool WRITE_DRES, bool NT = false>
@@ -1370,12 +1384,13 @@
 }
 }
 
-MDTF_EXPORT int mdtf_bn_bwd_dual(const void* dy, const void* x, const void* r, const uint8_t* mask, void* dx, void* dr,
+MDTF_EXPORT int mdtf_bn_bwd_dual_ep(const void* dy, const void* x, const void* r, const uint8_t* mask, void* dx, void* dr,
                                  long long M, int C, const float* gamma, const float* mean, const float* invstd,
                                  float* dgamma, float* dbeta, float* psum, float* psq, int P, const float* gamma2,
                                  const float* mean2, const float* invstd2, float* dgamma2, float* dbeta2, float* ws,
-                                 hipStream_t st) {
+                                 float* psq2, hipStream_t st) {
   if (C % 8 || !mask) return MDTF_EINVAL;
+  if (psq2 && P <= 0) return MDTF_EINVAL;
   Geo g = make_geo(M, C);
   const long long half = 2LL * g.gx * C + 4LL * C;
   float* q0 = ws;
@@ -1392,6 +1407,12 @@
     hipLaunchKernelGGL(bn_finalize_bwd, dim3(ceil_div(C, kFinCh)), dim3(kFinCh * kFinGroups), 0, st, p0, p1, g.gx, M,
                        C, gamma, mean, invstd, dgamma, dbeta, kk, kk + C, kk + 2 * C, 0);
   }
+  if (psq2) {
+    hipLaunchKernelGGL(bn_finalize_bwd_shared, dim3(ceil_div(C, kFinCh)), dim3(kFinCh * kFinGroups), 0, st,
+                       FinBwd{psum, psq, P, gamma, mean, invstd, dgamma, dbeta, kk, kk + C, kk + 2 * C, 0},
+                       FinBwd{psum, psq2, P, gamma2, mean2, invstd2, dgamma2, dbeta2, kk2, kk2 + C, kk2 + 2 * C, 0},
+                       M, C);
+  } else {
   hipLaunchKernelGGL((bn_reduce_kernel<true, true>), dim3(g.gx, g.gy), dim3(kThreads), lds, st, (const bf16_t*)dy,
                      (const bf16_t*)r, mask, M, C, g.tpr, g.rg, q0, q1);
   const FinBwd sc{q0, q1, g.gx, gamma2, mean2, invstd2, dgamma2, dbeta2, kk2, kk2 + C, kk2 + 2 * C, 0};
@@ -1401,6 +1422,7 @@
   else
     hipLaunchKernelGGL(bn_finalize_bwd2, dim3(ceil_div(C, kFinCh), 1), dim3(kFinCh * kFinGroups), 0, st, sc, sc, M,
                        C);
+  }
   const long long n8 = M * C / 8;
   hipLaunchKernelGGL((bn_nt() ? bn_dx_dual_kernel<true> : bn_dx_dual_kernel<false>), dim3(ew_grid(n8)),
                      dim3(kThreads), 0, st, (const bf16_t*)dy,
@@ -1408,3 +1430,12 @@
   MDTF_LAUNCH_CHECK();
   return 0;
 }
+
+MDTF_EXPORT int mdtf_bn_bwd_dual(const void* dy, const void* x, const void* r, const uint8_t* mask, void* dx, void* dr,
+                                 long long M, int C, const float* gamma, const float* mean, const float* invstd,
+                                 float* dgamma, float* dbeta, float* psum, float* psq, int P, const float* gamma2,
+                                 const float* mean2, const float* invstd2, float* dgamma2, float* dbeta2, float* ws,
+                                 hipStream_t st) {
+  return mdtf_bn_bwd_dual_ep(dy, x, r, mask, dx, dr, M, C, gamma, mean, invstd, dgamma, dbeta, psum, psq, P, gamma2,
+                             mean2, invstd2, dgamma2, dbeta2, ws, nullptr, st);
+}
diff --git a/mdtf/csrc/conv_igemm.hip b/mdtf/csrc/conv_igemm.hip
--- a/mdtf/csrc/conv_igemm.hip
+++ b/mdtf/csrc/conv_igemm.hip
@@ -45,6 +45,8 @@
   float* bsum;
   float* bsq;
   int bslots;
+  const bf16_t* bx2;
+  float* bsq2;
   float* dbias;
   float* slab;
   int slab_cap;
@@ -61,6 +63,7 @@
   long long m_base;
   int fin_blocks, fin_first;
   int co_remap;
+  int epi_early;
   const float* fin_psum;
   const float* fin_psq;
   int fin_P, fin_C;
@@ -618,6 +621,25 @@
   const bf16_t* wbase = MODE == 3 ? a.wseg[seg] : a.wgt;
   const int nl0 = MODE == 3 ? n0 - seg * a.seg_cols : n0;
 
+  constexpr int ITER = BM * (BN / 8) / NT;
+  static_assert(ITER * NT == BM * (BN / 8), "copy-out rows per thread");
+  auto copyout_off = [&](long long m, int n) -> long long {
+    if (m >= a.M || n >= a.Ncol) return -1;
+    long long pix = m;
+    if (MODE == 2) {
+      const unsigned mu = static_cast<unsigned>(m);
+      const unsigned t = fdiv31(mu, a.mg_rw, a.sh_rw);
+      const int j = static_cast<int>(mu - t * static_cast<unsigned>(a.cls_Wc));
+      const unsigned nb = fdiv31(t, a.mg_rh, a.sh_rh);
+      const int i = static_cast<int>(t - nb * static_cast<unsigned>(a.cls_Hc));
+      pix = (static_cast<long long>(nb) * a.H + a.cls_h0 + a.SH * i) * a.W + a.cls_w0 + a.SW * j;
+    }
+    return pix * a.Ncol + n;
+  };
+  constexpr bool EPI_EARLY = (MODE == 1 || MODE == 2) && NW == 4 && ITER <= 8 && STAGES >= 2 &&
+                             !(BM == 128 && BN == 128 && STAGES >= 10);
+  constexpr bool BX2_OK = EPI_EARLY && ITER <= 4;
+  constexpr int EI = EPI_EARLY ? ITER : 1;
   unsigned a_off[RA], a_mask[RA];
 #pragma unroll
   for (int i = 0; i < RA; ++i) {
@@ -710,6 +732,45 @@
     }
   }
 
+  constexpr int ER = BX2_OK ? ITER : 1;
+  uint4 e_old[EI], e_x[EI], e_r[ER];
+  uint8_t e_am[EI], e_mb[EI];
+#pragma unroll
+  for (int it = 0; it < EI; ++it) {
+    e_old[it] = e_x[it] = make_uint4(0, 0, 0, 0);
+    e_am[it] = e_mb[it] = 0xffu;
+  }
+#pragma unroll
+  for (int it = 0; it < ER; ++it) e_r[it] = make_uint4(0, 0, 0, 0);
+  bool early = false;
+  if constexpr (EPI_EARLY) {
+    early = a.epi_early && a.K <= 256 && (a.accumulate || a.bsum != nullptr);
+#pragma unroll
+    for (int i = 0; i < RA; ++i) asm volatile("" ::"v"(a_off[i]), "v"(a_mask[i]));
+#pragma unroll
+    for (int i = 0; i < RB; ++i) asm volatile("" ::"v"(b_off[i]));
+    if (early) {
+      const bool st_on = a.bsum != nullptr;
+      const bf16_t* osrc = a.accumulate ? (a.acc_src ? a.acc_src : a.out) : a.bx;
+      const bf16_t* xsrc = st_on ? a.bx : osrc;
+      const bf16_t* rsrc = st_on && a.bx2 ? a.bx2 : xsrc;
+      const uint8_t* amsrc = a.acc_mask ? a.acc_mask : reinterpret_cast<const uint8_t*>(osrc);
+      const uint8_t* bmsrc = st_on && a.bmask ? a.bmask : reinterpret_cast<const uint8_t*>(xsrc);
+#pragma unroll
+      for (int it = 0; it < EI; ++it) {
+        int row, c8;
+        copyout_rc<BN>(tid + it * NT, row, c8, a.co_remap != 0);
+        const long long o = copyout_off(m0 + row, n0 + c8 * 8);
+        const long long oo = (o >= 0 && a.accumulate) ? o : 0, ox = (o >= 0 && st_on) ? o : 0;
+        e_old[it] = *reinterpret_cast<const uint4*>(osrc + oo);
+        e_am[it] = amsrc[(a.acc_mask ? oo : 0) >> 3];
+        e_x[it] = *reinterpret_cast<const uint4*>(xsrc + ox);
+        e_mb[it] = bmsrc[(st_on && a.bmask ? ox : 0) >> 3];
+        if constexpr (BX2_OK) e_r[it] = *reinterpret_cast<const uint4*>(rsrc + (a.bx2 ? ox : 0));
+      }
+    }
+  }
+
   const int KT = a.K / 64;
   const int fr = lane & 15, fq = lane >> 4;
   if constexpr (SPLIT) {
@@ -893,38 +954,35 @@
   }
   __syncthreads();
   const bool bstat = (MODE == 1 || MODE == 2) && a.bsum != nullptr;
-  float bs0[8], bs1[8];
-#pragma unroll
-  for (int k = 0; k < 8; ++k) bs0[k] = bs1[k] = 0.f;
-  constexpr int ITER = BM * (BN / 8) / NT;
-  static_assert(ITER * NT == BM * (BN / 8), "copy-out rows per thread");
+  const bool bstat2 = BX2_OK && bstat && a.bx2 != nullptr;
+  float bs0[8], bs1[8], bs2[8];
+#pragma unroll
+  for (int k = 0; k < 8; ++k) bs0[k] = bs1[k] = bs2[k] = 0.f;
   constexpr int PF = (FD_PF16 && (MODE == 1 || MODE == 2) && ITER <= 16) ? ITER
                                                                         : (ITER < 4 ? ITER : (ITER % 4 == 0 ? 4 : 2));
   static_assert(ITER % PF == 0, "prefetch groups");
 #pragma unroll
   for (int g0 = 0; g0 < ITER; g0 += PF) {
   long long off[PF];
-  uint4 old4[PF], x4[PF];
+  uint4 old4[PF], x4[PF], r4[BX2_OK ? PF : 1];
   uint32_t mb[PF];
 #pragma unroll
   for (int it = 0; it < PF; ++it) {
     const int idx = tid + (g0 + it) * NT;
     int row, c8;
     copyout_rc<BN>(idx, row, c8, a.co_remap != 0);
-    const long long m = m0 + row;
-    const int n = n0 + c8 * 8;
-    off[it] = -1;
-    if (m < a.M && n < a.Ncol) {
-      long long pix = m;
-      if (MODE == 2) {
-        const unsigned mu = static_cast<unsigned>(m);
-        const unsigned t = fdiv31(mu, a.mg_rw, a.sh_rw);
-        const int j = static_cast<int>(mu - t * static_cast<unsigned>(a.cls_Wc));
-        const unsigned nb = fdiv31(t, a.mg_rh, a.sh_rh);
-        const int i = static_cast<int>(t - nb * static_cast<unsigned>(a.cls_Hc));
-        pix = (static_cast<long long>(nb) * a.H + a.cls_h0 + a.SH * i) * a.W + a.cls_w0 + a.SW * j;
-      }
-      off[it] = pix * a.Ncol + n;
+    if constexpr (EPI_EARLY) {
+      if (early) {
+        off[it] = copyout_off(m0 + row, n0 + c8 * 8);
+        old4[it] = a.acc_mask ? mask_bf8(e_old[g0 + it], e_am[g0 + it]) : e_old[g0 + it];
+        x4[it] = e_x[g0 + it];
+        mb[it] = a.bmask ? e_mb[g0 + it] : 0xffu;
+        if constexpr (BX2_OK) r4[it] = e_r[g0 + it];
+        continue;
+      }
+    }
+    off[it] = copyout_off(m0 + row, n0 + c8 * 8);
+    if (off[it] >= 0) {
       if (a.accumulate) {
         old4[it] = *reinterpret_cast<const uint4*>((a.acc_src ? a.acc_src : a.out) + off[it]);
         if (a.acc_mask) old4[it] = mask_bf8(old4[it], a.acc_mask[off[it] >> 3]);
@@ -932,6 +990,9 @@
       if (bstat) {
         x4[it] = *reinterpret_cast<const uint4*>(a.bx + off[it]);
         mb[it] = a.bmask ? a.bmask[off[it] >> 3] : 0xffu;
+        if constexpr (BX2_OK) {
+          if (bstat2) r4[it] = *reinterpret_cast<const uint4*>(a.bx2 + off[it]);
+        }
       }
     }
   }
@@ -995,6 +1056,16 @@
           bs0[k] += gk;
           bs1[k] += gk * xk;
         }
+        if constexpr (BX2_OK) {
+          if (bstat2) {
+            const uint32_t rw[4] = {r4[it].x, r4[it].y, r4[it].z, r4[it].w};
+#pragma unroll
+            for (int k = 0; k < 8; ++k) {
+              const float rk = (k & 1) ? __uint_as_float(rw[k >> 1] & 0xffff0000u) : __uint_as_float(rw[k >> 1] << 16);
+              bs2[k] += (((mb[it] >> k) & 1u) ? c[k] : 0.f) * rk;
+            }
+          }
+        }
       }
     } else {
       *reinterpret_cast<uint4*>(dst) = v;
@@ -1016,6 +1087,10 @@
     for (int k = 0; k < 8; ++k) {
       red[k * LDR + slot] = bs0[k];
       red[(8 + k) * LDR + slot] = bs1[k];
+    }
+    if (bstat2) {
+#pragma unroll
+      for (int k = 0; k < 8; ++k) red[(16 + k) * LDR + slot] = bs2[k];
     }
     __syncthreads();
     for (int nl = tid; nl < BN; nl += NT) {
@@ -1029,6 +1104,11 @@
         const long long slot = (long long)(mt % a.bslots) * a.Ncol + n;
         atomicAdd(a.bsum + slot, sv);
         atomicAdd(a.bsq + slot, q);
+        if (bstat2) {
+          float q2 = 0.f;
+          for (int t2 = c8; t2 < NT; t2 += BN / 8) q2 += red[(16 + k) * LDR + t2];
+          atomicAdd(a.bsq2 + slot, q2);
+        }
       }
     }
   }
@@ -1571,7 +1651,10 @@
                                           : STAGES * (size_t)(BM + BN) * 128;
   const size_t ctile = (size_t)BM * (BN * 2 + 16);
   size_t lds = stage_bytes > ctile ? stage_bytes : ctile;
-  if (lds < (size_t)(NT + 8) * 16 * sizeof(float)) lds = (size_t)(NT + 8) * 16 * sizeof(float);
+  if (a.bx2 && !((MODE == 1 || MODE == 2) && NW == 4 && BM * (BN / 8) / NT <= 4 && STAGES >= 2))
+    return MDTF_EUNSUPPORTED;
+  const size_t red_rows = a.bx2 ? 24 : 16;
+  if (lds < (size_t)(NT + 8) * red_rows * sizeof(float)) lds = (size_t)(NT + 8) * red_rows * sizeof(float);
   if (STAGES == 1 && a.K > 64) return MDTF_EINVAL;
   if (lds > 160 * 1024) return MDTF_EUNSUPPORTED;
   if (a.M >= (1LL << 31)) return MDTF_EUNSUPPORTED;
@@ -1583,7 +1666,7 @@
     magic31(static_cast<unsigned>(RW), &a.mg_rw, &a.sh_rw);
     magic31(static_cast<unsigned>(RH), &a.mg_rh, &a.sh_rh);
   }
-  if (MODE <= 2 && STAGES >= 2 && conv_persist_mode() && a.K >= 64) {
+  if (MODE <= 2 && STAGES >= 2 && conv_persist_mode() && a.K >= 64 && !a.bx2) {
     const int rc = launch_fd_p<BM, BN, MODE, STATS, STAGES, NW>(a, st);
     if (rc != MDTF_EUNSUPPORTED) return rc;
   }
@@ -1593,6 +1676,8 @@
       return (e && e[0] == '1') ? 1 : 0;
     }();
     a.co_remap = remap;
+    const char* ee = getenv("MDTF_FD_EPI_EARLY");
+    a.epi_early = (ee && ee[0] == '0') ? 0 : 1;
   }
   hipLaunchKernelGGL((conv_fd_v2<BM, BN, MODE, STATS, STAGES, NW>), dim3((unsigned)nblk), dim3(NT), lds, st, a);
   MDTF_LAUNCH_CHECK();
@@ -2289,9 +2374,9 @@
   const int ppb = 256 / C8;
   const int c8 = tid % C8, pl = tid / C8;
   const unsigned P = (unsigned)a.N * a.H * a.W;
-  float s0[8], s1[8];
-#pragma unroll
-  for (int k = 0; k < 8; ++k) s0[k] = s1[k] = 0.f;
+  float s0[8], s1[8], s2[8];
+#pragma unroll
+  for (int k = 0; k < 8; ++k) s0[k] = s1[k] = s2[k] = 0.f;
   for (unsigned p = blockIdx.x * (unsigned)ppb + pl; p < P; p += gridDim.x * (unsigned)ppb) {
     const unsigned q = fdiv31(p, a.mg_rw, a.sh_rw);
     const int w = static_cast<int>(p - q * (unsigned)a.W);
@@ -2317,6 +2402,16 @@
         s0[k] += gm;
         s1[k] += gm * xk;
       }
+      if (a.bx2) {
+        const uint4 r4 = *reinterpret_cast<const uint4*>(a.bx2 + off);
+        const uint32_t rw4[4] = {r4.x, r4.y, r4.z, r4.w};
+#pragma unroll
+        for (int k = 0; k < 8; ++k) {
+          const float g = (k & 1) ? __uint_as_float(vw[k >> 1] & 0xffff0000u) : __uint_as_float(vw[k >> 1] << 16);
+          const float rk = (k & 1) ? __uint_as_float(rw4[k >> 1] & 0xffff0000u) : __uint_as_float(rw4[k >> 1] << 16);
+          s2[k] += (((mb >> k) & 1u) ? g : 0.f) * rk;
+        }
+      }
     }
   }
   if constexpr (BSTAT) {
@@ -2337,6 +2432,18 @@
       }
       atomicAdd(a.bsum + slot + ch, sv);
       atomicAdd(a.bsq + slot + ch, q);
+    }
+    if (a.bx2) {
+      __syncthreads();
+#pragma unroll
+      for (int k = 0; k < 8; ++k) red[0][k][tid] = s2[k];
+      __syncthreads();
+      for (int ch = tid; ch < a.Ncol; ch += 256) {
+        const int cc = ch >> 3, k = ch & 7;
+        float q2 = 0.f;
+        for (int t = cc; t < 256; t += C8) q2 += red[0][k][t];
+        atomicAdd(a.bsq2 + slot + ch, q2);
+      }
     }
   }
 }
@@ -2456,13 +2563,14 @@
   return rc;
 }
 
-MDTF_EXPORT int mdtf_conv_dgrad_v2(const void* dy, const void* w, void* dx, int N, int H, int W, int Cin, int OH,
+MDTF_EXPORT int mdtf_conv_dgrad_v2_ep(const void* dy, const void* w, void* dx, int N, int H, int W, int Cin, int OH,
                                    int OW, int Cout, int KH, int KW, int SH, int SW, int PH, int PW, int DH, int DW,
                                    int bm, int bn, int accumulate, const void* bx, const void* bmask,
                                    float* bsum, float* bsq, int bslots, const void* acc_src, const void* acc_mask,
-                                   hipStream_t st) {
+                                   const void* bx2, float* bsq2, hipStream_t st) {
   if (Cout % 64 || Cin % 8) return MDTF_EINVAL;
   if ((acc_src || acc_mask) && !accumulate) return MDTF_EINVAL;
+  if ((bx2 != nullptr) != (bsq2 != nullptr) || (bx2 && !bsum)) return MDTF_EINVAL;
   if ((long long)N * OH * OW * Cout * 2 > 0x7fffffffLL) return MDTF_EUNSUPPORTED;
   if ((SH != 1 || SW != 1) && (DH != 1 || DW != 1)) return MDTF_EUNSUPPORTED;
   if (ceil_div(KH, SH) * ceil_div(KW, SW) > 32) return MDTF_EUNSUPPORTED;
@@ -2478,6 +2586,8 @@
   a.bsum = bsum;
   a.bsq = bsq;
   a.bslots = bslots > 0 ? bslots : 1;
+  a.bx2 = (const bf16_t*)bx2;
+  a.bsq2 = bsq2;
   a.Ncol = Cin;
   int stages;
   decode_tile(&bm, &stages);
@@ -2528,6 +2638,15 @@
   return 0;
 }
 
+MDTF_EXPORT int mdtf_conv_dgrad_v2(const void* dy, const void* w, void* dx, int N, int H, int W, int Cin, int OH,
+                                   int OW, int Cout, int KH, int KW, int SH, int SW, int PH, int PW, int DH, int DW,
+                                   int bm, int bn, int accumulate, const void* bx, const void* bmask,
+                                   float* bsum, float* bsq, int bslots, const void* acc_src, const void* acc_mask,
+                                   hipStream_t st) {
+  return mdtf_conv_dgrad_v2_ep(dy, w, dx, N, H, W, Cin, OH, OW, Cout, KH, KW, SH, SW, PH, PW, DH, DW, bm, bn, accumulate,
+                               bx, bmask, bsum, bsq, bslots, acc_src, acc_mask, nullptr, nullptr, st);
+}
+
 MDTF_EXPORT int mdtf_set_wgrad_fin(const float* psum, const float* psq, int P, const float* gamma, const float* mean,
                                    const float* invstd, float* ws, long long M, int C) {
   if (C < 0 || (C > 0 && (!psum || !psq || !mean || !invstd || !ws || P <= 0 || M <= 0))) return MDTF_EINVAL;
diff --git a/mdtf/ops/bn.py b/mdtf/ops/bn.py
--- a/mdtf/ops/bn.py
+++ b/mdtf/ops/bn.py
@@ -19,6 +19,7 @@
            + [N.P, N.P])
 N.register("mdtf_maxpool_bn_bwd", [N.P] * 4 + [N.I] * 12 + [N.P] * 8 + [N.P])
 N.register("mdtf_bn_bwd_dual", [N.P] * 6 + [N.L, N.I] + [N.P] * 7 + [N.I] + [N.P] * 6 + [N.P])
+N.register("mdtf_bn_bwd_dual_ep", [N.P] * 6 + [N.L, N.I] + [N.P] * 7 + [N.I] + [N.P] * 7 + [N.P])
 N.register("mdtf_bn_bwd_finalize_ws", [N.L, N.I, N.P, N.P, N.P, N.P, N.P, N.I, N.P, N.P])
 N.register("mdtf_bn_dx_ws", [N.P, N.P, N.P, N.P, N.P, N.L, N.I, N.P, N.P, N.P, N.I, N.I, N.P])
 N.register("mdtf_bn_fwd_coeffs", [N.L, N.I, N.P, N.P, N.P, N.P, N.F, N.F, N.P, N.P, N.P, N.P, N.I, N.P, N.P])
@@ -97,6 +98,7 @@
 DUAL_DZ = os.environ.get("MDTF_DUAL_DZ", "0") == "1"
 DUAL_FUSED = os.environ.get("MDTF_DUAL_BWD_FUSED", "1") != "0"
 DUAL_BWD = [0]
+DUAL_BWD_NOREDUCE = [0]
 
 
 class _BNTrain(torch.autograd.Function):
@@ -287,7 +289,7 @@
         ctx.like = (gamma, beta, gamma2, beta2)
         ctx.out_sink = actsink.attach(y)
         if ctx.out_sink is not None:
-            ctx.out_sink.stat_req = (x, mask)
+            ctx.out_sink.stat_req = (x, mask, None, None, r if DUAL_FUSED and not DUAL_DZ else None)
         return y
 
     @staticmethod
@@ -314,12 +316,14 @@
             dr = torch.empty_like(r)
             ws = torch.empty(2 * int(N.fn("mdtf_bn_workspace_floats")(M, C)), dtype=torch.float32, device=x.device)
             ps, pq, P = (pstats[0], pstats[1], int(pstats.shape[1])) if pstats is not None else (None, None, 0)
-            N.check(N.fn("mdtf_bn_bwd_dual")(N.ptr(dy), N.ptr(x), N.ptr(r), N.ptr(mask), N.ptr(dx), N.ptr(dr), M, C,
-                                             N.ptr(g), N.ptr(mean), N.ptr(invstd), N.ptr(grads[0]), N.ptr(grads[1]),
-                                             N.ptr(ps), N.ptr(pq), P, N.ptr(g2), N.ptr(mean2), N.ptr(invstd2),
-                                             N.ptr(grads[2]), N.ptr(grads[3]), N.ptr(ws), N.stream_ptr()),
-                    "bn_bwd_dual")
+            pq2 = pstats[2] if pstats is not None and pstats.shape[0] == 3 else None
+            N.check(N.fn("mdtf_bn_bwd_dual_ep")(N.ptr(dy), N.ptr(x), N.ptr(r), N.ptr(mask), N.ptr(dx), N.ptr(dr), M,
+                                                C, N.ptr(g), N.ptr(mean), N.ptr(invstd), N.ptr(grads[0]),
+                                                N.ptr(grads[1]), N.ptr(ps), N.ptr(pq), P, N.ptr(g2), N.ptr(mean2),
+                                                N.ptr(invstd2), N.ptr(grads[2]), N.ptr(grads[3]), N.ptr(ws),
+                                                N.ptr(pq2), N.stream_ptr()), "bn_bwd_dual")
             DUAL_BWD[0] += 1
+            DUAL_BWD_NOREDUCE[0] += pq2 is not None
             if pstats is not None:
                 from . import conv as _conv
                 _conv.bwd_stats_release(pstats, True)
diff --git a/mdtf/ops/conv.py b/mdtf/ops/conv.py
--- a/mdtf/ops/conv.py
+++ b/mdtf/ops/conv.py
@@ -15,6 +15,7 @@
 N.register("mdtf_conv_wgrad", [N.P, N.P, N.P] + [N.I] * 18 + [N.P])
 N.register("mdtf_conv_fwd_v2", [N.P, N.P, N.P, N.P, N.P] + [N.I] * 18 + [N.P, N.P])
 N.register("mdtf_conv_dgrad_v2", [N.P, N.P, N.P] + [N.I] * 18 + [N.P, N.P, N.P, N.P, N.I, N.P, N.P, N.P])
+N.register("mdtf_conv_dgrad_v2_ep", [N.P, N.P, N.P] + [N.I] * 18 + [N.P, N.P, N.P, N.P, N.I, N.P, N.P, N.P, N.P, N.P])
 N.register("mdtf_conv_wgrad_v2", [N.P, N.P, N.P] + [N.I] * 18 + [N.P, N.I, N.P])
 N.register("mdtf_set_slab_stream", [N.P])
 N.register("mdtf_set_wgrad_store", [N.I])
@@ -232,7 +233,15 @@
 
 
 def _bn_args(bn_stats):
-    return bn_stats if bn_stats is not None else (None, None, None, None, 0)
+    return bn_stats[:5] if bn_stats is not None else (None, None, None, None, 0)
+
+
+def _bn2_args(bn_stats):
+    return bn_stats[5:7] if bn_stats is not None and len(bn_stats) > 5 else (None, None)
+
+
+def dgrad_bx2_ok(cd):
+    return (cd.backend == "mdtf" and cd.ver == 2 and cd.bm * cd.bn <= 64 * 128 and cd.stages >= 2)
 
 
 def _acc_args(acc_src):
@@ -358,11 +367,15 @@
     geo = _geo(x_shape, w.shape, dy.shape[1:3], stride, pads, dil)
     if ver in (2, 3):
         bx, bmask, bsum, bsq, bslots = _bn_args(bn_stats)
+        bx2, bsq2 = _bn2_args(bn_stats)
         ag, am = _acc_args(acc_src)
-        N.check(N.fn("mdtf_conv_dgrad_v2")(N.ptr(dy), N.ptr(w), N.ptr(dx), *geo, _v2_code(bm, stages, ver), bn,
-                                           int(bool(accumulate) or acc_src is not None), N.ptr(bx), N.ptr(bmask),
-                                           N.ptr(bsum), N.ptr(bsq), int(bslots), N.ptr(ag), N.ptr(am),
-                                           N.stream_ptr()), "conv_dgrad_v2")
+        args = (N.ptr(dy), N.ptr(w), N.ptr(dx), *geo, _v2_code(bm, stages, ver), bn,
+                int(bool(accumulate) or acc_src is not None), N.ptr(bx), N.ptr(bmask), N.ptr(bsum), N.ptr(bsq),
+                int(bslots), N.ptr(ag), N.ptr(am))
+        if bx2 is not None:
+            N.check(N.fn("mdtf_conv_dgrad_v2_ep")(*args, N.ptr(bx2), N.ptr(bsq2), N.stream_ptr()), "conv_dgrad_v2")
+        else:
+            N.check(N.fn("mdtf_conv_dgrad_v2")(*args, N.stream_ptr()), "conv_dgrad_v2")
         return dx
     if acc_src is not None:
         raise ValueError("a masked accumulate source needs the v2 kernel")
@@ -659,6 +672,7 @@
 
 
 BWD_STATS = os.environ.get("MDTF_BN_BWD_STATS", "1") != "0"
+BWD_STATS2 = os.environ.get("MDTF_BN_BWD_STATS2", "1") != "0"
 STAT_SLOTS = 64
 MAX_STAT_SLOTS = int(os.environ.get("MDTF_BN_MAX_SLOTS", "128"))
 _STATS = {}
@@ -736,9 +750,9 @@
 _BSTATS = {}
 
 
-def bwd_stats_acquire(device, C, slots):
-    pool = _BSTATS.setdefault((device, C, slots), [])
-    return pool.pop() if pool else torch.zeros((2, slots, C), dtype=torch.float32, device=device)
+def bwd_stats_acquire(device, C, slots, rows=2):
+    pool = _BSTATS.setdefault((device, C, slots, rows), [])
+    return pool.pop() if pool else torch.zeros((rows, slots, C), dtype=torch.float32, device=device)
 
 
 def _early_finalize(xs, sbuf):
@@ -754,7 +768,7 @@
 def bwd_stats_release(buf, zeroed):
     if not zeroed:
         buf.zero_()
-    _BSTATS.setdefault((buf.device, buf.shape[2], buf.shape[1]), []).append(buf)
+    _BSTATS.setdefault((buf.device, buf.shape[2], buf.shape[1], buf.shape[0]), []).append(buf)
 
 
 def _fwd_stats(ch, want_stats, rows, co, device):
@@ -766,12 +780,17 @@
     return buf[0], buf[1]
 
 
-def _bwd_stats(xs, stat_rows, x):
+def _bwd_stats(xs, stat_rows, x, cd=None):
     if xs.stat_req is None or not xs.completing() or not BWD_STATS or N.deterministic():
         return None, None
     bx, bmask = xs.stat_req[:2]
+    bx2 = xs.stat_req[4] if len(xs.stat_req) > 4 and cd is not None and BWD_STATS2 and dgrad_bx2_ok(cd) else None
+    if bx2 is not None and not bx2.is_contiguous():
+        bx2 = None
     slots = STAT_SLOTS if stat_rows is None else stat_slots(-(-(x.numel() // x.shape[3]) // stat_rows))
-    sbuf = bwd_stats_acquire(x.device, x.shape[3], slots)
+    sbuf = bwd_stats_acquire(x.device, x.shape[3], slots, 3 if bx2 is not None else 2)
+    if bx2 is not None:
+        return (bx, bmask, sbuf[0], sbuf[1], sbuf.shape[1], bx2, sbuf[2]), sbuf
     return (bx, bmask, sbuf[0], sbuf[1], sbuf.shape[1]), sbuf
 
 
@@ -808,7 +827,7 @@
 def _dgrad_into_sink(xs, cd, dy, w, x, stride, pads, dil, pconv=None):
     if pconv is None:
         buf, acc, pend = xs.target_ex()
-        bst, sbuf = _bwd_stats(xs, cd.stat_rows, x)
+        bst, sbuf = _bwd_stats(xs, cd.stat_rows, x, cd)
         dx = _launch_dgrad(cd, dy, w, x.shape, stride, pads, dil, out=buf, accumulate=acc, bn_stats=bst,
                            acc_src=pend)
     else:
```

Result: no change. 13040 images/sec, median of 4 (+0.1%).
